# fixstars/cuda-bundle-adjustment

Measured on AMD Instinct MI355X. Metric: edges/sec (edge-iterations/s = E x LM iterations / wall, graph resident in HBM, every timed 10-iteration run from its own perturbed start) + 10-iter LM wall-clock (contract_wall: initialize()+optimize(10) after warm-up, C++ API) on KITTI-00-shaped graph; per-iter chi2 vs g2o-faithful oracle, higher is better.
Workload: dtype f64

## Files before the change

cuda-bundle-adjustment_amd/csrc/ba_device.hpp:

```cpp
#pragma once

#include "ba_kernels.hpp"

#include <type_traits>

namespace cubahip
{


#ifdef CUBA_HIP_TRACE
static __device__ unsigned long long cuba_trace_buf[3][8192 * 8];
#define TRACE_DECL unsigned long long tr_[8] = { 0, 0, 0, 0, 0, 0, 0, 0 }; int trn_ = 0; \
	{ unsigned long long t0_; asm volatile("s_memrealtime %0\n\ts_waitcnt lgkmcnt(0)" : "=s"(t0_)); tr_[7] = t0_; }
#define TRACE_MARK() do { asm volatile("s_waitcnt vmcnt(0) lgkmcnt(0)" ::: "memory"); tr_[trn_++] = wall_clock64(); } while (0)
#define TRACE_FLUSH(kid, wave) do { if ((threadIdx.x & 63) == 0 && (wave) < 8192) for (int t_ = 0; t_ < 8; t_++) cuba_trace_buf[kid][(wave) * 8 + t_] = tr_[t_]; } while (0)
#else
#define TRACE_DECL
#define TRACE_MARK() do { } while (0)
#define TRACE_FLUSH(kid, wave) do { } while (0)
#endif

__device__ __forceinline__ void atomic_max_nonneg(unsigned long long* p, Scalar v)
{
	if (v > 0) atomicMax(p, (unsigned long long)__double_as_longlong((double)v));
// ... 109 lines not shown
	int i = threadIdx.x;
	for (; i + 3072 < n; i += 4096)
	{
		const Scalar a = parts[i], b = parts[i + 1024], c = parts[i + 2048], d = parts[i + 3072];
		v0 += a; v1 += b; v2 += c; v3 += d;
	}
	for (; i < n; i += 1024) v0 += parts[i];
	return (v0 + v1) + (v2 + v3);
}

__device__ __forceinline__ Scalar block_sum_1024(Scalar v, Scalar* sh16)
{
	v = wave_sum(v);
	if ((threadIdx.x & 63) == 0) sh16[threadIdx.x >> 6] = v;
	__syncthreads();
	Scalar t = threadIdx.x < 16 ? sh16[threadIdx.x] : Scalar(0);
	if (threadIdx.x < 64) t = wave_sum(t);
	return t;
}

__device__ __forceinline__ void store_slot_group(Scalar* out, Scalar total)
{
	if (threadIdx.x < NSLOT) out[threadIdx.x] = threadIdx.x == 0 ? total : Scalar(0);
}

static __global__ __launch_bounds__(1024) void reduce_parts_kernel(const Scalar* __restrict__ parts, int n, Scalar* out)
{
	__shared__ Scalar sh[16];
	store_slot_group(out, block_sum_1024(parts_thread_sum(parts, n), sh));
}

static void launch_reduce_parts(const Scalar* parts, int n, Scalar* out, hipStream_t s)
{
	hipLaunchKernelGGL(reduce_parts_kernel, dim3(1), dim3(1024), 0, s, parts, n, out);
}

struct LaneEdge
{
	int ip, il;
	bool stereo;
	Scalar wr;
	EdgeLin lin;
};

__device__ __forceinline__ void load_pose(const DeviceGraph& g, int ip, Scalar q[4], Scalar t[3], Scalar cam[5])
{
#pragma unroll
	for (int i = 0; i < 4; i++) q[i] = g.q[4 * (size_t)ip + i];
#pragma unroll
	for (int i = 0; i < 3; i++) t[i] = g.t[3 * (size_t)ip + i];
#pragma unroll
	for (int i = 0; i < 5; i++) cam[i] = g.cam[5 * (size_t)ip + i];
}

__device__ __forceinline__ void linearize_edge(const DeviceGraph& g, int e, LaneEdge& out)
{
	const int pe = g.e_pose[e];
	out.stereo = (pe & STEREO_BIT) != 0;
	out.ip = pe & ~STEREO_BIT;
	out.il = g.e_lm[e];
	Scalar q[4], t[3], cam[5], Xw[3], meas[3], Xc[3];
	load_pose(g, out.ip, q, t, cam);
#pragma unroll
	for (int i = 0; i < 3; i++) Xw[i] = g.Xw[3 * (size_t)out.il + i];
	meas[0] = g.e_mu[e]; meas[1] = g.e_mv[e]; meas[2] = g.e_mr[e];
	const Scalar w = g.e_w[e];
	const Scalar s = edge_residual(q, t, cam, Xw, meas, out.stereo, out.lin.r, Xc);
	const int kind = out.stereo ? g.rk[1].kind : g.rk[0].kind;
	const Scalar delta = out.stereo ? g.rk[1].delta : g.rk[0].delta;
	out.wr = w * robust_weight(kind, delta, w * s);
	const Rot3 R = quat_to_rot(q[0], q[1], q[2], q[3]);
	edge_jacobians(Xc, R, cam, out.stereo, out.lin);
}

__device__ __forceinline__ void publish_report(const DeviceSystem& sys)
{
	sys.host_flags[0] = *sys.fail; sys.host_flags[1] = *sys.iters; sys.host_flags[2] = *sys.done;
	__threadfence_system();
	asm volatile("s_waitcnt vmcnt(0) lgkmcnt(0)" ::: "memory");
	const int t = ++(*sys.ticket);
	__hip_atomic_store(&sys.host_flags[3], t, __ATOMIC_RELAXED, __HIP_MEMORY_SCOPE_SYSTEM);
}

}
```

cuda-bundle-adjustment_amd/csrc/ba_edge.hip:

```cpp

#include "ba_device.hpp"

namespace cubahip
{

__device__ __forceinline__ void residual_chi2_body(const DeviceGraph& g, Scalar* parts, Scalar* per_edge, int bid, int nb)
{
	Scalar acc = 0;
	for (int e = g.e_begin + bid * 256 + threadIdx.x; e < g.e_end; e += nb * 256)
	{
		const int pe = g.e_pose[e];
		const bool stereo = (pe & STEREO_BIT) != 0;
		const int ip = pe & ~STEREO_BIT;
		const int il = g.e_lm[e];
		Scalar q[4], t[3], cam[5], Xw[3], meas[3], r[3], Xc[3];
		load_pose(g, ip, q, t, cam);
#pragma unroll
		for (int i = 0; i < 3; i++) Xw[i] = g.Xw[3 * (size_t)il + i];
		meas[0] = g.e_mu[e]; meas[1] = g.e_mv[e]; meas[2] = g.e_mr[e];
		const Scalar ee = g.e_w[e] * edge_residual(q, t, cam, Xw, meas, stereo, r, Xc);
		const int kind = stereo ? g.rk[1].kind : g.rk[0].kind;
		const Scalar delta = stereo ? g.rk[1].delta : g.rk[0].delta;
		acc += robust_rho(kind, delta, ee);
		if (per_edge) per_edge[e] = ee;
// ... 517 lines not shown
	{
		Scalar xl[3] = { 0, 0, 0 }, sc = 0;
		if (lmFree)
		{
			Scalar cs[3];
#pragma unroll
			for (int k = 0; k < 3; k++) cs[k] = red[0][k] + red[1][k] + red[2][k] + red[3][k];
			sc = finish_landmark_x(sys, il, cs, lambda, xl);
#pragma unroll
			for (int k = 0; k < 3; k++) g.Xw[3 * (size_t)il + k] = go.Xw[3 * (size_t)il + k] + xl[k];
		}
		scParts[blockIdx.x] = sc;
#pragma unroll
		for (int k = 0; k < 3; k++) xsh[k] = xl[k];
	}
	__syncthreads();
	Scalar Xn[3];
#pragma unroll
	for (int k = 0; k < 3; k++) Xn[k] = go.Xw[3 * (size_t)il + k] + xsh[k];
	Scalar rho = 0;
	for (int e = e0 + threadIdx.x; e < e1; e += 256)
	{
		const int pe = g.e_pose[e];
		const bool stereo = (pe & STEREO_BIT) != 0;
		const int ip = pe & ~STEREO_BIT;
		Scalar q[4], t[3], cam[5], meas[3], xp[6];
		load_pose(go, ip, q, t, cam);
		meas[0] = g.e_mu[e]; meas[1] = g.e_mv[e]; meas[2] = g.e_mr[e];
		const bool poseFree = ip < g.Pf;
#pragma unroll
		for (int r = 0; r < 6; r++) xp[r] = poseFree ? sys.xp[6 * (size_t)ip + r] : Scalar(0);
		rho += updated_edge_rho(g, q, t, cam, xp, poseFree, Xn, meas, g.e_w[e], stereo);
	}
	rho = wave_sum(rho);
	if ((threadIdx.x & 63) == 0) rsh[threadIdx.x >> 6] = rho;
	__syncthreads();
	if (threadIdx.x == 0) chiParts[blockIdx.x] = (rsh[0] + rsh[1]) + (rsh[2] + rsh[3]);
}

size_t trial_tail_parts(const DeviceGraph& g, const DeviceStructure& st, int priorParts)
{
	const size_t a = (size_t)(st.nWaves + LIN_BLOCK / WAVE - 1) / (LIN_BLOCK / WAVE) + st.nBig;
	const size_t nA = (a + 63) / 64 * 64;
	return nA + (a + priorParts + 63) / 64 * 64 + 4 * 256 + 64;
}

void launch_trial_tail_fused(const DeviceGraph& g, const DeviceStructure& st, const DeviceSystem& sys, Scalar lambda, const Scalar* old, hipStream_t s,
	const LmDevice* decide, const DevicePriors* pr, const DeviceRelPoses* rp)
{
	const int nLm = (st.nWaves + LIN_BLOCK / WAVE - 1) / (LIN_BLOCK / WAVE);
	const int nA = nLm + st.nBig;
	const int nRp = relpose_chi2_parts(rp);
	const int nPr = prior_chi2_parts(pr) + nRp;
	Scalar* scParts = sys.parts;
	Scalar* chiParts = sys.parts + (size_t)(nA + 63) / 64 * 64;
	Scalar* scaleParts = chiParts + (size_t)(nA + nPr + 63) / 64 * 64;
	const int poseBlocks = (g.Pf + LIN_BLOCK - 1) / LIN_BLOCK;
	const int nScale = g.Pf > 0 ? min((g.Pf * 6 + 255) / 256, 256) : 0;
	if (nLm + poseBlocks + nScale > 0)
		hipLaunchKernelGGL(trial_tail_kernel, dim3(nLm + poseBlocks + nScale), dim3(LIN_BLOCK), 0, s, g, st, sys, lambda, old, scParts, chiParts, nLm, poseBlocks, scaleParts, nScale);
	if (st.nBig > 0) hipLaunchKernelGGL(big_trial_tail_kernel, dim3(st.nBig), dim3(256), 0, s, g, st, sys, lambda, old, scParts + nLm, chiParts + nLm);
	if (nPr > nRp) launch_prior_chi2(g, *pr, chiParts + nA, s);
	if (nRp > 0) launch_relpose_chi2(g, *rp, chiParts + nA + (nPr - nRp), s);
	hipLaunchKernelGGL(reduce_report_kernel, dim3(1), dim3(1024), 0, s, sys, scParts, nA, sys.slots + NSLOT, chiParts, nA + nPr, sys.slots, scaleParts, 4 * nScale, sys.slots + 3 * NSLOT,
		decide ? decide->state : (double*)nullptr, decide ? decide->lam : (Scalar*)nullptr, decide ? decide->ring : (double*)nullptr);
}

void batch_fill_tail(const DeviceGraph& g, const DeviceStructure& st, const DeviceSystem& sys, const Scalar* old, const LmDevice& lm, Scalar* state, size_t stateCount, BatchTrial& t)
{
	const int nLm = (st.nWaves + LIN_BLOCK / WAVE - 1) / (LIN_BLOCK / WAVE);
	const int nA = nLm + st.nBig;
	t.scParts = sys.parts;
	t.chiParts = sys.parts + (size_t)(nA + 63) / 64 * 64;
	t.scaleParts = t.chiParts + (size_t)(nA + 63) / 64 * 64;
	t.poseBlocks = (g.Pf + LIN_BLOCK - 1) / LIN_BLOCK;
	t.nScale = g.Pf > 0 ? min((g.Pf * 6 + 255) / 256, 256) : 0;
	t.nLm = nLm; t.nA = nA; t.old = old;
	t.tailGrid = (unsigned)(nLm + t.poseBlocks + t.nScale);
	t.lmState = lm.state; t.lmLam = lm.lam; t.lmRing = lm.ring; t.reportOn = 1;
	t.state = state; t.stateCount = stateCount;
	t.restoreGrid = (unsigned)std::min<size_t>(512, (stateCount + 255) / 256);
}

__global__ void lm_decide_failed_kernel(DeviceSystem sys, double* lmState, Scalar* lmLam, double* lmRing)
{
	if (threadIdx.x != 0) return;
	lm_decide(lmState, lmLam, lmRing, 0, 0.0, 0.0, 0.0);
	__threadfence_system();
	if (sys.host_flags) publish_report(sys);
}

void launch_lm_decide_failed(const DeviceSystem& sys, const LmDevice& lm, hipStream_t s)
{
	hipLaunchKernelGGL(lm_decide_failed_kernel, dim3(1), dim3(64), 0, s, sys, lm.state, lm.lam, lm.ring);
}

__global__ __launch_bounds__(256) void restore_if_rejected_batch_kernel(const BatchEntry* __restrict__ tab)
{
	const BatchTrial& t = tab[blockIdx.y].t;
	if (blockIdx.x >= t.restoreGrid || t.lmState[5] != 0.0) return;
	const size_t stride = (size_t)t.restoreGrid * 256;
	const Scalar* __restrict__ backup = t.backupDst;
	Scalar* __restrict__ state = t.state;
	for (size_t i = (size_t)blockIdx.x * 256 + threadIdx.x; i < t.stateCount; i += stride) state[i] = backup[i];
}

__global__ __launch_bounds__(256) void restore_if_rejected_kernel(Scalar* __restrict__ state, const Scalar* __restrict__ backup, size_t count, const double* lmState)
{
	if (lmState[5] != 0.0) return;
	const size_t stride = (size_t)gridDim.x * 256;
	for (size_t i = (size_t)blockIdx.x * 256 + threadIdx.x; i < count; i += stride) state[i] = backup[i];
}

void launch_restore_if_rejected(Scalar* state, const Scalar* backup, size_t count, const LmDevice& lm, hipStream_t s)
{
	const unsigned grid = (unsigned)std::min<size_t>(512, (count + 255) / 256);
	if (grid) hipLaunchKernelGGL(restore_if_rejected_kernel, dim3(grid), dim3(256), 0, s, state, backup, count, lm.state);
}

void launch_batch_tail(const BatchEntry* tab, int n, unsigned tailGridMax, unsigned restoreGridMax, hipStream_t s)
{
	if (tailGridMax) hipLaunchKernelGGL(trial_tail_batch_kernel, dim3(tailGridMax, n), dim3(LIN_BLOCK), 0, s, tab);
	hipLaunchKernelGGL(reduce_report_batch_kernel, dim3(n), dim3(1024), 0, s, tab);
	if (restoreGridMax) hipLaunchKernelGGL(restore_if_rejected_batch_kernel, dim3(restoreGridMax, n), dim3(256), 0, s, tab);
}

}
```

cuda-bundle-adjustment_amd/csrc/ba_kernels.hpp:

```cpp
#pragma once

#include <hip/hip_runtime.h>
#include <cstdint>
#include <vector>

#include "ba_math.hpp"

namespace cubahip
{

constexpr int PCG_SETUP_POSES = 64;
constexpr int NSLOT = 16;
constexpr int WAVE = 64;
constexpr int LIN_BLOCK = 256;
constexpr int STEREO_BIT = 0x40000000;

struct DeviceGraph
{
	int Pt = 0, Pf = 0, Lt = 0, Lf = 0, E = 0;
	int e_begin = 0, e_end = 0;
	Scalar *q = nullptr, *t = nullptr, *cam = nullptr, *Xw = nullptr;
	int *e_pose = nullptr, *e_lm = nullptr;
	Scalar *e_mu = nullptr, *e_mv = nullptr, *e_mr = nullptr, *e_w = nullptr;
	int* lm_ptr = nullptr;
	RobustKernel rk[2] = { { 0, 0 }, { 0, 0 } };
};

constexpr int BP_HEAVY = 64;

struct DeviceStructure
{
	int nWaves = 0;
	int* wave_lm = nullptr;
	int nBig = 0;
	int* big_lm = nullptr;
	int nblk = 0;
	int *hsc_rowptr = nullptr, *hsc_colind = nullptr;
	int *adj_ptr = nullptr, *adj_blk = nullptr, *adj_col = nullptr;
	int2* ell = nullptr;
	int ell_m = 0, ell_over = 0;
	int* hsc_blkrow = nullptr;
	int nOd = 0;
	int nDiagProd = 0;
	int* od_blocks = nullptr;
	int inv_rows8 = 1;
	int nHeavy = 0;
	int *prod_ea = nullptr, *prod_eb = nullptr;
	const int *prod_beg = nullptr, *prod_end = nullptr, *pe_beg = nullptr, *pe_end = nullptr;
	int* prod_lm = nullptr;
	int* pe_edge = nullptr;
	int nCb = 0;
	int *cb_I = nullptr, *cb_J = nullptr, *cb_ptr = nullptr, *cb_blk = nullptr;
	Scalar *cb_wi = nullptr, *cb_wj = nullptr;
	Scalar* e_rec = nullptr;
	int mixed = 0;
};

int spmv_rows_for(int Pf);

struct DeviceSystem
{
	Scalar* hsc = nullptr;
	Scalar* bsc = nullptr;
	Scalar* bp = nullptr;
	Scalar* lm_sys = nullptr;
	Scalar* lm_inv = nullptr;
	Scalar* xp = nullptr;
	Scalar* xl = nullptr;
	Scalar* parts = nullptr;
	Scalar* slots = nullptr;
	unsigned long long* maxdiag = nullptr;
	int* fail = nullptr;
	Scalar *minv = nullptr, *r = nullptr, *z = nullptr, *p0 = nullptr, *p1 = nullptr, *ap = nullptr;
	Scalar *rz = nullptr, *pq = nullptr;
	int rzStride = 0, pqStride = 0;
	int nrz0 = 0, nrz = 0, npq = 0;
	int* done = nullptr;
	int* iters = nullptr;
	int* host_flags = nullptr;
	int* ticket = nullptr;
	int* kbase = nullptr;
	int agg = 0;
	int nc = 0;
	Scalar inv_agg = 0;
	int cl = 1;
	Scalar* acinv = nullptr;
	float* acinv32 = nullptr;
	Scalar* gj_pivots = nullptr;
	Scalar* rc = nullptr;
	Scalar* hrow = nullptr;
	int spmv_rows = 2;
	Scalar* qpart = nullptr;
	Scalar* r2 = nullptr;
	const Scalar* lam_dev = nullptr;
	int upper = 0;
	Scalar* tq = nullptr;
	int* lowpos = nullptr;
};

struct DevicePriors
{
	int n = 0;
	int nPoses = 0;
	const int* pose_ptr = nullptr;
	const int* pose_id = nullptr;
	const int* pose = nullptr;
	const Scalar *qbar = nullptr, *tbar = nullptr;
	const Scalar* info = nullptr;
	Scalar* chi = nullptr;
};
void launch_prior_linearize(const DeviceGraph& g, const DeviceStructure& st, const DeviceSystem& sys, const DevicePriors& pr, int mode, hipStream_t s);
void launch_prior_chi2(const DeviceGraph& g, const DevicePriors& pr, Scalar* parts, hipStream_t s);
int prior_chi2_parts(const DevicePriors* pr);

constexpr int REL_REC = 90;
struct DeviceRelPoses
{
	int n = 0;
	int nActive = 0;
	int nBlocks = 0;
	int nPoses = 0;
	const int *pose_i = nullptr, *pose_j = nullptr;
	const int* blk_ptr = nullptr;
	const int* blk_id = nullptr;
	const int* pose_ptr = nullptr;
	const int* pose_id = nullptr;
	const int* pose_item = nullptr;
	const Scalar *q = nullptr, *t = nullptr;
	const Scalar* info = nullptr;
	Scalar* rec = nullptr;
	Scalar* chi = nullptr;
};
void launch_relpose_linearize(const DeviceGraph& g, const DeviceStructure& st, const DeviceSystem& sys, const DeviceRelPoses& rp, int mode, hipStream_t s);
void launch_relpose_chi2(const DeviceGraph& g, const DeviceRelPoses& rp, Scalar* parts, hipStream_t s);
int relpose_chi2_parts(const DeviceRelPoses* rp);

void launch_residual_chi2(const DeviceGraph& g, Scalar* parts, Scalar* slots, Scalar* per_edge, hipStream_t st, const DevicePriors* pr = nullptr,
	const DeviceRelPoses* rp = nullptr);

struct BlockPassRange { int begin, end, heavy; };
void launch_linearize_dm(const DeviceGraph& g, const DeviceStructure& st, const DeviceSystem& sys, int mode, Scalar lambda, hipStream_t s,
	const Scalar* backupSrc = nullptr, Scalar* backupDst = nullptr, size_t backupCount = 0, const BlockPassRange* range = nullptr);
void launch_block_pass(const DeviceGraph& g, const DeviceStructure& st, const DeviceSystem& sys, const BlockPassRange& range, hipStream_t s);

void launch_pose_maxdiag(const DeviceGraph& g, const DeviceStructure& st, const DeviceSystem& sys, hipStream_t s);

void launch_back_substitute(const DeviceGraph& g, const DeviceStructure& st, const DeviceSystem& sys, Scalar lambda, hipStream_t s);

void launch_pose_scale(const DeviceGraph& g, const DeviceSystem& sys, Scalar lambda, Scalar* slots, hipStream_t s);
struct LmDevice;
void launch_trial_tail_fused(const DeviceGraph& g, const DeviceStructure& st, const DeviceSystem& sys, Scalar lambda, const Scalar* old, hipStream_t s,
	const LmDevice* decide = nullptr, const DevicePriors* pr = nullptr, const DeviceRelPoses* rp = nullptr);
size_t trial_tail_parts(const DeviceGraph& g, const DeviceStructure& st, int priorParts = 0);
constexpr int LM_REC = 8, LM_RING = 64;
struct LmDevice { double* state = nullptr; Scalar* lam = nullptr; double* ring = nullptr; };
void launch_lm_decide_failed(const DeviceSystem& sys, const LmDevice& lm, hipStream_t s);
void launch_restore_if_rejected(Scalar* state, const Scalar* backup, size_t count, const LmDevice& lm, hipStream_t s);
void launch_landmark_scale(const DeviceGraph& g, const DeviceSystem& sys, Scalar lambda, Scalar* slots, hipStream_t s);

void launch_update_state(const DeviceGraph& g, const DeviceSystem& sys, hipStream_t s);

void launch_pcg_setup(const DeviceGraph& g, const DeviceStructure& st, const DeviceSystem& sys, Scalar lambda, hipStream_t s);
void launch_pcg_spmv(const DeviceGraph& g, const DeviceStructure& st, const DeviceSystem& sys, int k, int maxIter, Scalar tol2, hipStream_t s);
void launch_pcg_update(const DeviceGraph& g, const DeviceStructure& st, const DeviceSystem& sys, int k, int maxIter, Scalar tol2, hipStream_t s);
Scalar* launch_coarse_setup(const DeviceGraph& g, const DeviceStructure& st, const DeviceSystem& sys, Scalar* work0, Scalar* work1, hipStream_t s, hipEvent_t assembled = nullptr);
Scalar* launch_dense_inverse(Scalar* work0, Scalar* work1, int n, Scalar* pivots, hipStream_t s);
void launch_coarse_finish(const Scalar* swept, Scalar* dst, int n, hipStream_t s);
struct GjJob { Scalar* buf[2]; Scalar* piv[2]; int n, tiles; };
void launch_coarse_assemble(const DeviceGraph& g, const DeviceStructure& st, const DeviceSystem& sys, Scalar* work0, hipStream_t s);
void launch_dense_inverse_batch(const GjJob* jobs, int m, int nMax, hipStream_t s);
void launch_pcg2_fused(const DeviceGraph& g, const DeviceSystem& sys, int k, int kOut, int maxIter, Scalar tol2, int doUpdate, hipStream_t s);
int spmv_upper_grid(int Pf);
int pcg_rows_max_aggregate();
int pcg_rows_entries_per_thread(const DeviceSystem& sys);
void launch_build_lowpos(const DeviceGraph& g, const DeviceStructure& st, int* lowpos, hipStream_t s);
void launch_pcg_upper_iteration(const DeviceGraph& g, const DeviceStructure& st, const DeviceSystem& sys, int k, int maxIter, Scalar tol2, hipStream_t s, int which = 7);
void launch_pcg_advance(const DeviceSystem& sys, int n, hipStream_t s, Scalar tol2 = Scalar(-1));
void launch_coarse_to_fp32(const Scalar* swept, float* dst, int n, hipStream_t s);
void launch_pcg_iteration(const DeviceGraph& g, const DeviceStructure& st, const DeviceSystem& sys, int k, int maxIter, Scalar tol2, hipStream_t s);

struct LmDevice;
struct BatchTrial
{
	unsigned lmGroups = 0, lmGrid = 0; const Scalar* backupSrc = nullptr; Scalar* backupDst = nullptr; size_t backupCount = 0;
	int poseGroups = 0; unsigned schurGrid = 0;
	int nSetup = 0; size_t expandTotal = 0; unsigned nExpand = 0; const Scalar* copySrc = nullptr; Scalar* copyDst = nullptr; size_t copyPairs = 0; unsigned setupGrid = 0;
	int fusedOn = 0;
	const Scalar* old = nullptr; Scalar *scParts = nullptr, *chiParts = nullptr, *scaleParts = nullptr; int nLm = 0, poseBlocks = 0, nScale = 0; unsigned tailGrid = 0; int nA = 0;
	double* lmState = nullptr; Scalar* lmLam = nullptr; double* lmRing = nullptr; int reportOn = 0;
	Scalar* state = nullptr; size_t stateCount = 0; unsigned restoreGrid = 0;
};
struct BatchEntry
{
	DeviceGraph g; DeviceStructure st; DeviceSystem sys;
	int maxIter = 0;
	int gridSpmv = 0;
	BatchTrial t;
};
void batch_fill_linearize(const DeviceGraph& g, const DeviceStructure& st, const Scalar* backupSrc, Scalar* backupDst, size_t backupCount, BatchTrial& t);
void launch_batch_linearize(const BatchEntry* tab, int n, unsigned lmGridMax, unsigned schurGridMax, bool mixed, hipStream_t s);
void batch_fill_setup(const DeviceGraph& g, const DeviceStructure& st, const DeviceSystem& sys, const Scalar* copySrc, Scalar* copyDst, size_t copyCount, BatchTrial& t);
void launch_batch_setup(const BatchEntry* tab, int n, unsigned gridMax, hipStream_t s);
void launch_batch_first_precond(const BatchEntry* tab, int n, const DeviceSystem& sys0, int ncMax, size_t ldsMax, Scalar tol2, hipStream_t s);
void batch_fill_tail(const DeviceGraph& g, const DeviceStructure& st, const DeviceSystem& sys, const Scalar* old, const LmDevice& lm, Scalar* state, size_t stateCount, BatchTrial& t);
void launch_batch_tail(const BatchEntry* tab, int n, unsigned tailGridMax, unsigned restoreGridMax, hipStream_t s);
int batch_kernel_class(const DeviceGraph& g, const DeviceSystem& sys);
size_t batch_pcg2_lds_bytes(const DeviceSystem& sys);
void launch_pcg_batch_iteration(const BatchEntry* tab, int n, const DeviceGraph& g0, const DeviceSystem& sys0, int gridSpmvMax, int ncMax, size_t ldsMax, int k, Scalar tol2, hipStream_t s);
void launch_pcg_batch_advance(const BatchEntry* tab, int n, int iters, hipStream_t s, Scalar tol2);

hipError_t graph_add_pcg_chunk(hipGraph_t graph, const DeviceGraph& g, const DeviceStructure& st, const DeviceSystem& sys, int chunk, int maxIter, Scalar tol2, int report);

void launch_hsc_expand(const DeviceGraph& g, const DeviceStructure& st, const DeviceSystem& sys, hipStream_t s);
void launch_pcg_setup_expand(const DeviceGraph& g, const DeviceStructure& st, const DeviceSystem& sys, Scalar lambda, hipStream_t s,
	const Scalar* copySrc = nullptr, Scalar* copyDst = nullptr, size_t copyCount = 0);

constexpr int SC_T = 32;
constexpr int SC_TP = 5;
constexpr int SC_TT = SC_T * SC_T;

struct SparseCholPlan
{
	int Pf = 0, T = 0, nTiles = 0, nLevels = 0, slack = 0;
	std::vector<int> posOfSeg, segOfPos;
	std::vector<int> colPtr;
	std::vector<int> rowIdx, colOfTile;
	std::vector<int> gPtr;
	std::vector<int> gather;
	std::vector<int> wgRec;
	std::vector<int> lvlPtr, lvlTiles;
	std::vector<int> lvlColPtr, lvlCols;
	std::vector<int> blkTile;
	long long entries = 0;
	size_t tileBytes() const { return sizeof(Scalar) * (size_t)SC_TT * ((size_t)2 * nTiles + 1); }
	double secondsEstimate() const;
};
bool sparse_chol_plan(int Pf, const int* rowptr, const int* colind, int slack, size_t maxTiles, SparseCholPlan& out);

struct SparseChol
{
	Scalar* tiles = nullptr;
	Scalar* tilesT = nullptr;
	Scalar* y = nullptr;
	Scalar* rinv = nullptr;
	const int *colPtr = nullptr, *rowIdx = nullptr, *colOfTile = nullptr, *gPtr = nullptr, *gather = nullptr;
	const int *wgRec = nullptr, *lvlCols = nullptr, *blkTile = nullptr, *posOfSeg = nullptr;
	int* fail = nullptr;
	int T = 0, Pf = 0, nTiles = 0;
};
void launch_sparse_chol_fill(const DeviceStructure& st, const DeviceSystem& sys, const SparseChol& d, hipStream_t s);
void launch_sparse_chol_solve(const SparseChol& d, const SparseCholPlan& plan, Scalar* x, hipStream_t s);
void launch_sparse_chol_factor(const SparseChol& d, const SparseCholPlan& plan, hipStream_t s);

struct SelInvPlan
{
	int nLevels = 0;
	std::vector<int> stepPtr;
	std::vector<int> offRec;
	std::vector<int> colStepPtr, cols;
	std::vector<int> gather;
// ... 58 lines not shown
```

cuda-bundle-adjustment_amd/csrc/ba_lm.hip:

```cpp
#include "ba_solver.hpp"

using namespace cubahip;

void cuba_hip_solver::graphWorker()
{
	(void)hipSetDevice(device);
	std::unique_lock<std::mutex> lk(gb.m);
	for (;;)
	{
		gb.cv.wait(lk, [&] { return gb.stop || !gb.jobs.empty() || !gb.trash.empty(); });
		if (gb.stop) return;
		if (gb.jobs.empty())
		{
			std::vector<hipGraphExec_t> t; t.swap(gb.trash);
			gb.busy = true;
			lk.unlock();
			for (hipGraphExec_t e : t) (void)hipGraphExecDestroy(e);
			lk.lock();
			gb.busy = false;
			gb.cv.notify_all();
			continue;
		}
		GraphJob j = gb.jobs.front(); gb.jobs.pop_front();
		gb.busy = true;
		lk.unlock();
		const auto t0 = Clock::now();
		hipGraph_t graph = nullptr; hipGraphExec_t exec = nullptr;
		bool ok = hipGraphCreate(&graph, 0) == hipSuccess && graph_add_pcg_chunk(graph, j.g, j.st, j.sys, j.chunk, j.maxIter, j.tol2, 1) == hipSuccess &&
			hipGraphInstantiate(&exec, graph, nullptr, nullptr, 0) == hipSuccess;
		if (graph) (void)hipGraphDestroy(graph);
		if (!ok) (void)hipGetLastError();
		const double dt = std::chrono::duration<double>(Clock::now() - t0).count();
		lk.lock();
		gb.busy = false;
		if (ok && j.gen == gb.gen) { gb.ready[std::make_pair(j.chunk, j.acinv)] = exec; gb.builds++; gb.seconds.store(gb.seconds.load() + dt); }
		else if (exec) (void)hipGraphExecDestroy(exec);
		gb.cv.notify_all();
	}
}

hipGraphExec_t cuba_hip_solver::pcgGraphIfReady(int chunk, int maxIter, Scalar tol2)
{
	if (pcgGraphTol2 != tol2 || pcgGraphMaxIter != maxIter) { dropPcgGraph(); pcgGraphTol2 = tol2; pcgGraphMaxIter = maxIter; }
	const auto key = std::make_pair(chunk, (const Scalar*)sys.acinv);
	auto it = pcgGraphs.find(key);
	if (it != pcgGraphs.end()) return it->second;
	std::lock_guard<std::mutex> lk(gb.m);
	for (auto& kv : gb.ready) pcgGraphs[kv.first] = kv.second;
	gb.ready.clear();
	it = pcgGraphs.find(key);
	if (it != pcgGraphs.end()) return it->second;
	if (!gb.requested.count(key))
	{
		gb.requested[key] = 1;
		gb.jobs.push_back(GraphJob{ chunk, (const Scalar*)sys.acinv, g, st, sys, maxIter, tol2, gb.gen });
		if (!gb.th.joinable()) gb.th = std::thread([this] { graphWorker(); });
		gb.cv.notify_all();
	}
	return nullptr;
}

void cuba_hip_solver::dropPcgGraph()
{
	{
		std::lock_guard<std::mutex> lk(gb.m);
		gb.gen++;
		gb.jobs.clear(); gb.requested.clear();
		const bool offload = gb.th.joinable() && !gb.stop;
		for (auto& kv : gb.ready) { if (offload) gb.trash.push_back(kv.second); else (void)hipGraphExecDestroy(kv.second); }
		gb.ready.clear();
		for (auto& kv : pcgGraphs) { if (offload) gb.trash.push_back(kv.second); else (void)hipGraphExecDestroy(kv.second); }
		if (offload && !gb.trash.empty()) gb.cv.notify_all();
	}
	pcgGraphs.clear();
	batchRequests.clear();
	graphsOrderedFor = nullptr;
}

void cuba_hip_solver::ensureOverlapObjects()
{
	if (gjStream) return;
	int prioLow = 0, prioHigh = 0;
	HIP_TRY(hipDeviceGetStreamPriorityRange(&prioLow, &prioHigh));
	HIP_TRY(hipStreamCreateWithPriority(&gjStream, hipStreamNonBlocking, prioLow));
	HIP_TRY(hipEventCreateWithFlags(&evSetup, hipEventDisableTiming));
	HIP_TRY(hipEventCreateWithFlags(&evAssembled, hipEventDisableTiming));
	HIP_TRY(hipEventCreateWithFlags(&evInverse, hipEventDisableTiming));
	HIP_TRY(hipEventCreateWithFlags(&evFirstInv, hipEventDisableTiming));
	HIP_TRY(hipEventRecord(evFirstInv, gjStream));
}

void cuba_hip_solver::waitReport()
{
	volatile int* flags = (volatile int*)((char*)h_pinned + 1024);
	{
		const auto t0 = Clock::now();
		for (long spins = 0; flags[3] != expectedTicket; spins++)
			if ((spins & 0xfff) == 0xfff && std::chrono::duration<double>(Clock::now() - t0).count() > 2.0) break;
		if (flags[3] == expectedTicket)
		{
			std::atomic_thread_fence(std::memory_order_acquire);
			return;
		}
	}
	sync();
	std::atomic_thread_fence(std::memory_order_acquire);
	expectedTicket = flags[3];
}

void cuba_hip_solver::downloadAsDouble(const Scalar* dsrc, double* hdst, size_t n)
{
	if (!n) return;
	if (sizeof(Scalar) == sizeof(double))
	{
		HIP_TRY(hipMemcpyAsync(hdst, dsrc, n * sizeof(double), hipMemcpyDeviceToHost, stream));
		sync();
		return;
	}
	std::vector<Scalar> tmp(n);
	HIP_TRY(hipMemcpyAsync(tmp.data(), dsrc, n * sizeof(Scalar), hipMemcpyDeviceToHost, stream));
	sync();
	for (size_t i = 0; i < n; i++) hdst[i] = (double)tmp[i];
}

void cuba_hip_solver::uploadFromDouble(Scalar* ddst, const double* hsrc, size_t n)
{
	if (!n) return;
	std::vector<Scalar> tmp(hsrc, hsrc + n);
	HIP_TRY(hipMemcpyAsync(ddst, tmp.data(), n * sizeof(Scalar), hipMemcpyHostToDevice, stream));
	sync();
}

double cuba_hip_solver::computeErrors()
{
	need();
	StageTimer tm(this, 2);
	launch_residual_chi2(g, d_parts.data(), slotsDev, nullptr, stream, priors(), relPoses());
	return readSlots(0);
}

void cuba_hip_solver::linearize(int mode, double lam, bool withBackup)
{
	waitAssembled();
	const bool parts = mode == 1 && !redParts.empty();
	launch_linearize_dm(g, st, sys, mode, lam, stream, withBackup ? d_state.data() : nullptr, d_backup.data(), d_state.size(), parts ? &redParts[0].od : nullptr);
	if (parts && !partsByCaller)
		for (size_t c = 1; c < redParts.size(); c++) launch_block_pass(g, st, sys, redParts[c].od, stream);
	if (priors()) launch_prior_linearize(g, st, sys, pri, mode, stream);
	if (relPoses()) launch_relpose_linearize(g, st, sys, rel, mode, stream);
}

void cuba_hip_solver::schurPart(int part, size_t ranges[4])
{
	need();
	if (part < 0 || part >= schurParts()) throw ArgError{ "cuba_hip_schur_part: no such part" };
	if (part == 0)
	{
		StageTimer tm(this, 4);
		zeroReduced();
		partsByCaller = true;
		try { linearize(1, lambda, false); } catch (...) { partsByCaller = false; throw; }
		partsByCaller = false;
	}
	else
	{
		StageTimer tm(this, 4);
		launch_block_pass(g, st, sys, redParts[part].od, stream);
	}
	const size_t nblk = (size_t)st.nblk;
	ranges[0] = redParts.empty() ? 0 : 36 * redParts[part].blkBegin;
	ranges[1] = redParts.empty() ? 36 * nblk : 36 * (redParts[part].blkEnd - redParts[part].blkBegin);
	ranges[2] = part == 0 ? 36 * nblk : 0;
	ranges[3] = part == 0 ? d_red.size() - 36 * nblk : 0;
}

void cuba_hip_solver::assemble()
{
	need();
	StageTimer tm(this, 3);
	zeroReduced(true);
	d_maxdiag.zero(stream);
	linearize(0, 0.0);
}

void cuba_hip_solver::maxDiagonalParts(double* posePart, double* lmPart)
{
	need();
// ... 67 lines not shown
	return ok2;
}

int cuba_hip_solver::pcgBudget(int maxIter) const
{
	const int it = directAfter > 0 ? directAfter : std::min(384, std::max(128, Pf / 4));
	return std::min(maxIter, std::max(4, it / 4 * 4));
}

bool cuba_hip_solver::ensureDirectPlan()
{
	if (directPlanValid) return !directRefused;
	const auto t0 = Clock::now();
	ensureHostPattern();
	if (!sparse_chol_plan(Pf, h_rowptr.data(), h_colind.data(), directSlack, (size_t)std::max(1, directMaxTiles), directPlan))
	{
		directPlanValid = true; directRefused = true;
		char buf[200];
		std::snprintf(buf, sizeof buf, "exact reduced solve unavailable: the factor of the %d-pose reduced matrix needs more than direct_max_tiles = %d tiles", Pf, directMaxTiles);
		lastError = buf;
		return false;
	}
	const SparseCholPlan& p = directPlan;
	{
		size_t freeB = 0, totalB = 0;
		const size_t have = sizeof(Scalar) * (d_scTiles.size() + d_scTilesT.size());
		if (hipMemGetInfo(&freeB, &totalB) == hipSuccess && p.tileBytes() > have && p.tileBytes() - have > freeB)
		{
			directPlanValid = true; directRefused = true;
			char buf[200];
			std::snprintf(buf, sizeof buf, "exact reduced solve unavailable: the factor of the %d-pose reduced matrix needs %.1f MB, %.1f MB of device memory are free",
				Pf, p.tileBytes() / 1e6, freeB / 1e6);
			lastError = buf;
			return false;
		}
		(void)hipGetLastError();
	}
	std::vector<int> ints;
	auto put = [&](const std::vector<int>& v) { const size_t o = ints.size(); ints.insert(ints.end(), v.begin(), v.end()); while (ints.size() % 4) ints.push_back(0); return o; };
	const size_t oColPtr = put(p.colPtr), oRowIdx = put(p.rowIdx), oColOf = put(p.colOfTile), oGPtr = put(p.gPtr), oGather = put(p.gather),
		oWgRec = put(p.wgRec), oLvlCols = put(p.lvlCols), oBlkTile = put(p.blkTile), oPos = put(p.posOfSeg);
	d_scInts.upload(ints, stream);
	d_scTiles.resize((size_t)SC_TT * ((size_t)p.nTiles + 1)); d_scTilesT.resize((size_t)SC_TT * std::max(1, p.nTiles));
	d_scY.resize((size_t)SC_T * p.T); d_scRinv.resize((size_t)SC_T * p.T); d_scFail.resize(1);
	sync();
	SparseChol& d = directDev;
	d.tiles = d_scTiles.data(); d.tilesT = d_scTilesT.data(); d.y = d_scY.data(); d.rinv = d_scRinv.data(); d.fail = d_scFail.data();
	const int* base = d_scInts.data();
	d.colPtr = base + oColPtr; d.rowIdx = base + oRowIdx; d.colOfTile = base + oColOf; d.gPtr = base + oGPtr; d.gather = base + oGather;
	d.wgRec = base + oWgRec; d.lvlCols = base + oLvlCols; d.blkTile = base + oBlkTile; d.posOfSeg = base + oPos;
	d.T = p.T; d.Pf = Pf; d.nTiles = p.nTiles;
	directPlanValid = true;
	directPlanBuilds++;
	directPlanSeconds = std::chrono::duration<double>(Clock::now() - t0).count();
	if (std::getenv("CUBA_HIP_DEBUG"))
		std::fprintf(stderr, "[cuba_hip] exact reduced solve, symbolic phase: %d poses -> %d tile columns, %d tiles (%.1f MB), %d levels, %lld tile products, slack %d, %.2f ms\n",
			Pf, p.T, p.nTiles, p.tileBytes() / 1e6, p.nLevels, p.entries, p.slack, 1e3 * directPlanSeconds);
	return true;
}

bool cuba_hip_solver::solveDirect()
{
	if (!ensureDirectPlan()) return false;
	const auto t0 = Clock::now();
	launch_sparse_chol_fill(st, sys, directDev, stream);
	launch_sparse_chol_solve(directDev, directPlan, sys.xp, stream);
	int* hflag = (int*)hostStage();
	HIP_TRY(hipMemcpyAsync(hflag, directDev.fail, sizeof(int), hipMemcpyDeviceToHost, stream));
	sync();
	directSeconds = std::chrono::duration<double>(Clock::now() - t0).count();
	cntDirect++;
	directSticky = true;
	coarseValid = false;
	if (std::getenv("CUBA_HIP_DEBUG"))
		std::fprintf(stderr, "[cuba_hip] exact reduced solve: %d unknowns, %.3f ms, lambda %.3e%s\n", 6 * Pf, 1e3 * directSeconds, lambda, *hflag ? " -- NON-POSITIVE PIVOT" : "");
	if (*hflag)
	{
		cntDirectFailed++;
		lastError = "exact reduced solve: non-positive pivot (the damped reduced matrix is not positive definite)";
		return false;
	}
	return true;
}

bool cuba_hip_solver::solveBegin(SolveCtx& sc)
{
	lastSolveBrokeDown = false;
	need();
	if (Pf == 0) { sc.result = true; return true; }
	const int maxIter = sc.maxIter = maxIterAlloc;
	const Scalar tol2 = sc.tol2 = pcgTol * pcgTol;
	if (failDirty) { d_fail.zero(stream); failDirty = false; }
	const bool twoLevel = sc.twoLevel = sys.agg > 0;
	const bool direct = sc.direct = directUsable();
	if (direct && (directSticky || directAlways))
	{
		launch_pcg_setup(g, st, sys, lambda, stream);
		failDirty = true;
		coarseValid = false;
		if (pcgHistory.size() >= 65536) pcgHistory.erase(pcgHistory.begin(), pcgHistory.begin() + 32768);
		pcgHistory.push_back(0);
		sc.result = solveDirect();
		return true;
	}
	sc.budget = direct && !acceptUnconverged ? pcgBudget(maxIter) : maxIter;
	const size_t invCount = (size_t)36 * sys.cl * sys.cl * sys.nc * sys.nc;
	bool takeInverse = false;
	if (twoLevel && coarseValid && pendingInv >= 0)
	{
		HIP_TRY(hipStreamWaitEvent(stream, evInverse, 0));
		takeInverse = true; pendingInv = -1;
	}
	const bool deferred = sc.deferLaunch && twoLevel && coarseValid;
	{
		const bool f32 = fp32Inverse();
		const Scalar* cpSrc = !takeInverse ? nullptr : f32 ? reinterpret_cast<const Scalar*>(d_coarse32[1].data()) : d_coarse[0].data();
		Scalar* cpDst = f32 ? reinterpret_cast<Scalar*>(d_coarse32[0].data()) : d_coarse[2].data();
		const size_t cpCount = f32 ? inv32Count() / 2 : invCount;
		if (deferred) { sc.deferred = true; sc.copySrc = cpSrc; sc.copyDst = cpDst; sc.copyCount = cpCount; }
		else launch_pcg_setup_expand(g, st, sys, lambda, stream, cpSrc, cpDst, cpCount);
	}
	if (twoLevel)
	{
		const int gjSteps = (6 * sys.cl * sys.nc + 31) / 32, first = gjSteps & 1;
		{
			ensureOverlapObjects();
			const size_t invBytes = sizeof(Scalar) * (size_t)36 * sys.cl * sys.cl * sys.nc * sys.nc;
			if (!coarseValid && heuristics && firstInvValid)
			{
				HIP_TRY(hipStreamWaitEvent(stream, evFirstInv, 0));
				if (fp32Inverse()) HIP_TRY(hipMemcpyAsync(d_coarse32[0].data(), d_firstInv32.data(), inv32Count() * sizeof(float), hipMemcpyDeviceToDevice, stream));
				else HIP_TRY(hipMemcpyAsync(d_coarse[2].data(), d_firstInv.data(), invBytes, hipMemcpyDeviceToDevice, stream));
				pendingInv = -1;
				coarseValid = true; sideAge = overlapPeriod(); firstInvPending = true;
			}
			else if (!coarseValid)
			{
				drainInversion();
				(void)launch_coarse_setup(g, st, sys, d_coarse[first].data(), d_coarse[1 - first].data(), stream);
				if (fp32Inverse()) launch_coarse_to_fp32(d_coarse[0].data(), d_coarse32[0].data(), 6 * sys.cl * sys.nc, stream);
				else launch_coarse_finish(d_coarse[0].data(), d_coarse[2].data(), 6 * sys.cl * sys.nc, stream);
				coarseValid = true; cntCoarseRefresh++; cntCoarseInline++; sideAge = 0;
				if (heuristics)
				{
					if (fp32Inverse()) d_firstInv32.resize(inv32Count()); else d_firstInv.resize(invCount);
					sideAge = overlapPeriod(); firstInvPending = true;
				}
			}
			sys.acinv = d_coarse[2].data();
			const bool regular = ++sideAge >= overlapPeriod();
			if (regular) sideAge = 0;
			if (regular)
			{
				if (!deferred) HIP_TRY(hipEventRecord(evSetup, stream));
				if (sc.deferCoarse)
				{
					sc.deferCoarse->push_back(CoarseJob{ this, first, firstInvPending, !deferred });
					if (firstInvPending) { firstInvPending = false; firstInvValid = true; }
				}
				else
				{
					HIP_TRY(hipStreamWaitEvent(gjStream, evSetup, 0));
					(void)launch_coarse_setup(g, st, sys, d_coarse[first].data(), d_coarse[1 - first].data(), gjStream, evAssembled);
					if (fp32Inverse()) launch_coarse_to_fp32(d_coarse[0].data(), d_coarse32[1].data(), 6 * sys.cl * sys.nc, gjStream);
					else launch_coarse_finish(d_coarse[0].data(), d_coarse[0].data(), 6 * sys.cl * sys.nc, gjStream);
					if (firstInvPending)
					{
						if (fp32Inverse()) HIP_TRY(hipMemcpyAsync(d_firstInv32.data(), d_coarse32[1].data(), inv32Count() * sizeof(float), hipMemcpyDeviceToDevice, gjStream));
						else HIP_TRY(hipMemcpyAsync(d_firstInv.data(), d_coarse[0].data(), invBytes, hipMemcpyDeviceToDevice, gjStream));
						HIP_TRY(hipEventRecord(evFirstInv, gjStream));
						firstInvPending = false; firstInvValid = true;
					}
					HIP_TRY(hipEventRecord(evInverse, gjStream));
				}
				pendingInv = 0;
				assemblePending = true; cntCoarseRefresh++;
			}
		}
		if (!deferred) launch_pcg2_fused(g, sys, 0, 0, maxIter, tol2, 0, stream);
	}
	const bool graphs = sc.graphs = useGraph && !sc.batched && g_liveHandles.load(std::memory_order_relaxed) <= 1;
	if (useGraph && !graphs && (!pcgGraphs.empty() || graphsOrderedFor)) dropPcgGraph();
	if (graphs && pcgGraphs.empty() && graphsOrderedFor != (const void*)sys.acinv)
	{
		for (int c = 64; c >= 4; c /= 2) (void)pcgGraphIfReady(c, maxIter, tol2);
		graphsOrderedFor = (const void*)sys.acinv;
	}
	sc.hInts = (volatile int*)((char*)h_pinned + 1024);
	sc.tSolve0 = Clock::now();
	int predicted = 32;
	if (runIters.size() >= 2)
	{
		const double a = runIters[runIters.size() - 2], b = runIters.back();
		const double lin = b + std::max(0.0, b - a), geo = b * std::min(1.35, std::max(1.0, b / std::max(1.0, a)));
		predicted = (int)std::max(lin, geo) + 1;
	}
	else if (runIters.size() == 1) predicted = (int)(1.35 * runIters[0]) + 2;
	else if (firstSolveIters > 0) predicted = firstSolveIters + 1;
	{
		const size_t k = runIters.size();
		if (heuristics && k < prevRunIters.size() && std::equal(runIters.begin(), runIters.end(), prevRunIters.begin())) predicted = prevRunIters[k];
	}
	sc.predicted = predicted;
	return false;
}

bool cuba_hip_solver::solveBrokeDown(SolveCtx& sc)
{
	lastSolveBrokeDown = true; lastFailCode = sc.hInts[0];
	cntPcgIters += sc.hInts[1]; coarseValid = false; firstInvValid = false; firstInvPending = false; failDirty = true;
	if (sc.direct && lastFailCode != 1 && !(lastFailCode == 2 && fp32Inverse() && sc.twoLevel))
	{
		if (pcgHistory.size() >= 65536) pcgHistory.erase(pcgHistory.begin(), pcgHistory.begin() + 32768);
		pcgHistory.push_back(-sc.hInts[1]);
		d_fail.zero(stream); failDirty = false;
		return solveDirect();
	}
	return false;
}

bool cuba_hip_solver::solveReducedOnce()
{
	StageTimer tm(this, 6);
	SolveCtx sc;
	if (solveBegin(sc)) return sc.result;
	const int maxIter = sc.maxIter; const Scalar tol2 = sc.tol2; const bool graphs = sc.graphs; const int predicted = sc.predicted;
	bool converged = false;
	int k0 = 0, looks = 0, eagerIters = 0;
	int target = (predicted + 3) / 4 * 4;
	while (k0 < sc.budget && !converged)
	{
		int todo = std::max(4, std::min(target, sc.budget) - k0);
		while (todo > 0)
		{
			int c = graphs ? 256 : todo;
			for (; graphs && c > 4 && c > todo; c >>= 1) {}
			if (graphs && todo > c && todo % 4 == 0 && todo <= 128 && pcgGraphMaxIter == maxIter && pcgGraphTol2 == tol2)
			{
				if ((pcgGraphs.count(std::make_pair(todo, (const Scalar*)sys.acinv)) || ++batchRequests[todo] >= 2) && pcgGraphIfReady(todo, maxIter, tol2)) c = todo;
			}
			hipGraphExec_t exec = graphs ? pcgGraphIfReady(c, maxIter, tol2) : nullptr;
			if (exec) { HIP_TRY(hipGraphLaunch(exec, stream)); noteReport(); }
			else
			{
				for (int k = 0; k < c; k++) enqueuePcgIteration(k, maxIter, tol2, stream);
				launch_pcg_advance(sys, c, stream, tol2); noteReport();
				if (graphs) { eagerIters += c; cntPcgPlain += c; }
			}
			k0 += c; todo -= c;
		}
		waitReport();
		if (sc.hInts[0] != 0) return solveBrokeDown(sc);
		if (sc.hInts[2] != 0 || sc.hInts[1] < std::min(k0, maxIter)) converged = true;
		target = k0 + ((looks == 0 && k0 <= 96) ? 4 : std::max(8, k0 / 8 / 4 * 4));
		looks++; cntPcgLooks++; cntHostLooks++;
	}
	sc.converged = converged; sc.k0 = k0; sc.looks = looks; sc.eagerIters = eagerIters;
	return solveEnd(sc);
}

bool cuba_hip_solver::solveEnd(SolveCtx& sc)
{
	const int maxIter = sc.maxIter; const bool direct = sc.direct; const bool converged = sc.converged;
	const int k0 = sc.k0, looks = sc.looks, eagerIters = sc.eagerIters, predicted = sc.predicted;
	const auto tSolve1 = Clock::now();
	if (std::getenv("CUBA_HIP_DEBUG"))
	{
		std::vector<Scalar> part((size_t)std::max(1, sys.nrz0));
		HIP_TRY(hipMemcpyAsync(part.data(), sys.rz, sizeof(Scalar) * part.size(), hipMemcpyDeviceToHost, stream));
		sync();
		double rz0 = 0; for (Scalar v : part) rz0 += (double)v;
		std::fprintf(stderr, "[cuba_hip] PCG: %d iterations, %d enqueued (%d as plain launches), %d host looks (prediction %d), lambda %.3e, r0.z0 %.6e, solve %.3f ms, graphs built so far %lld\n",
			sc.hInts[1], k0, eagerIters, looks, predicted, lambda, rz0, 1e3 * std::chrono::duration<double>(tSolve1 - sc.tSolve0).count(), (long long)gb.builds.load());
	}
	const int itersDone = sc.itersDone >= 0 ? sc.itersDone : sc.hInts[1];
	cntPcgIters += itersDone; cntPcgEnqueued += k0;
	if (runIters.empty()) firstSolveIters = itersDone;
	runIters.push_back(itersDone);
	if (pcgHistory.size() >= 65536) pcgHistory.erase(pcgHistory.begin(), pcgHistory.begin() + 32768);
	pcgHistory.push_back(converged ? itersDone : -itersDone);
	if (!converged)
	{
		cntPcgUnconverged++;
		coarseValid = false;
		if (direct && !acceptUnconverged) return solveDirect();
		char buf[160];
		std::snprintf(buf, sizeof buf, "PCG stopped at max_iter = %d without reaching pcg_tol = %g", maxIter, pcgTol);
		lastError = buf;
		return acceptUnconverged;
	}
	return true;
}

void cuba_hip_solver::backSubstitute()
{
	need();
	StageTimer tm(this, 4);
	launch_back_substitute(g, st, sys, lambda, stream);
}

bool cuba_hip_solver::solve()
{
	schur();
	if (!solveReduced()) return false;
	backSubstitute();
	return true;
}

void cuba_hip_solver::update()
{
	need();
	StageTimer tm(this, 7);
	launch_update_state(g, sys, stream);
}

double cuba_hip_solver::computeScale(double lam)
{
	need();
	double a = 0, b = 0;
	scaleParts(lam, &a, &b);
	return a + b;
}

void cuba_hip_solver::lmRunBegin(LmRun& r, int niter, double* chi2Out)
{
	const double tau = 1e-5;
	if (!h_lmRing)
	{
		HIP_TRY(hipHostMalloc((void**)&h_lmRing, sizeof(double) * LM_RING * LM_REC, hipHostMallocMapped | hipHostMallocCoherent));
		HIP_TRY(hipHostGetDevicePointer((void**)&lmRingDev, h_lmRing, 0));
	}
	coarseValid = false;
	startRunHistory();
	r = LmRun();
	r.niter = niter; r.chi2Out = chi2Out; r.stop = niter <= 0;
	r.F = computeErrors();
	r.lam = tau * maxDiagonal();
	{
		double* st8 = reinterpret_cast<double*>(hostStage());
		st8[0] = r.F; st8[1] = r.lam; st8[2] = 2.0; st8[3] = 0.0; st8[4] = 0.0; st8[5] = 1.0; st8[6] = 0.0; st8[7] = (double)LmRun::maxq;
		r.tagBase = 65536.0 * (double)(++lmRunNonce); st8[8] = r.tagBase;
		Scalar* l1 = reinterpret_cast<Scalar*>(st8 + 12);
		l1[0] = (Scalar)r.lam;
		HIP_TRY(hipMemcpyAsync(d_lmState.data(), st8, sizeof(double) * 9, hipMemcpyHostToDevice, stream));
		HIP_TRY(hipMemcpyAsync(d_lamS.data(), l1, sizeof(Scalar), hipMemcpyHostToDevice, stream));
	}
	r.lm.state = d_lmState.data(); r.lm.lam = d_lamS.data(); r.lm.ring = lmRingDev;
}

void cuba_hip_solver::lmAbsorb(LmRun& r, int upto)
{
	std::atomic_thread_fence(std::memory_order_acquire);
	for (; r.seen < upto && !r.stop; r.seen++)
	{
		const volatile double* rec = h_lmRing + (size_t)(r.seen % LM_RING) * LM_REC;
		const double tag = r.tagBase + (double)(r.seen + 1);
		if (rec[7] != tag)
		{
			cntLateRecords++;
			sync();
			std::atomic_thread_fence(std::memory_order_acquire);
			if (rec[7] != tag) throw StateError{ "the device's decision record of an LM trial never arrived" };
		}
		const bool acc = rec[5] != 0.0;
		const double rho = rec[2];
		r.lam = rec[3]; r.F = rec[4];
		if (acc) r.rejRun = 0; else r.rejRun++;
		const bool iterationEnds = acc || r.rejRun == LmRun::maxq || !(rho < 0);
		if (!iterationEnds) continue;
		if (r.chi2Out) r.chi2Out[r.done] = r.F;
		r.done++;
		if (r.done == r.niter || r.rejRun == LmRun::maxq || rho <= 0 || !std::isfinite(r.lam)) r.stop = true;
		r.rejRun = 0;
	}
}

bool cuba_hip_solver::lmBeforeTrial(LmRun& r)
{
	if (r.stop) return false;
	if (r.enq > r.seen)
	{
		const bool safe = r.done + 1 < r.niter && r.rejRun + 1 < LmRun::maxq;
		if (!safe) { waitReport(); cntHostLooks++; lmAbsorb(r, r.enq); if (r.stop) return false; }
	}
	cntTrials++;
	lambda = -1.0;
	return true;
}

bool cuba_hip_solver::lmAfterSolveHost(LmRun& r)
{
	lmAbsorb(r, r.enq);
	if (r.stop) { cntTrials--; return false; }
	return true;
}

bool cuba_hip_solver::lmAfterSolve(LmRun& r, bool ok)
{
	if (!lmAfterSolveHost(r)) return false;
	if (ok) launch_trial_tail_fused(g, st, sys, (Scalar)-1, d_backup.data(), stream, &r.lm, priors(), relPoses());
	else launch_lm_decide_failed(sys, r.lm, stream);
	noteReport();
	launch_restore_if_rejected(d_state.data(), d_backup.data(), d_state.size(), r.lm, stream);
	r.enq++;
	(void)hipStreamQuery(stream);
	return true;
}

int cuba_hip_solver::lmRunEnd(LmRun& r)
{
	if (r.seen < r.enq) { waitReport(); cntHostLooks++; lmAbsorb(r, r.enq); }
	lambda = r.lam;
	return r.done;
}

int cuba_hip_solver::optimizeDeviceDecision(int niter, double* chi2Out)
{
	LmRun r;
	lmRunBegin(r, niter, chi2Out);
	while (lmBeforeTrial(r))
	{
		schur(true);
		const bool ok = solveReduced();
		if (!lmAfterSolve(r, ok)) break;
	}
	return lmRunEnd(r);
}

bool cuba_hip_solver::fullyBatchable() const
{
	return batchable() && st.nBig == 0 && st.nDiagProd == 0 && st.nOd > 0 && st.nWaves > 0 && redParts.empty() && h_priorPose.empty() && h_relI.empty();
}

bool cuba_hip_solver::batchable() const
{
	return !profile && partHi < 0 && Pf > 0 && Lf > 0 && E > 0 && trial_tail_parts(g, st, extraChiParts()) <= d_parts.size() && batch_kernel_class(g, sys) >= 0;
}

void cuba_hip_solver::launchCoarseJobs(std::vector<CoarseJob>& jobs, hipEvent_t common)
{
	if (jobs.empty()) return;
	ensureOverlapObjects();
	hipStream_t side = gjStream;
	const int m = (int)jobs.size();
	if (!h_gjTab) { HIP_TRY(hipHostMalloc((void**)&h_gjTab, sizeof(GjJob) * CUBA_HIP_BATCH_MAX, hipHostMallocDefault)); HIP_TRY(hipEventCreateWithFlags(&evGjTab, hipEventDisableTiming)); HIP_TRY(hipEventRecord(evGjTab, side)); }
	d_gjTab.resize(sizeof(GjJob) * CUBA_HIP_BATCH_MAX);
	HIP_TRY(hipEventSynchronize(evGjTab));
	int nMax = 0;
	for (int a = 0; a < m; a++)
	{
		cuba_hip_solver* h = jobs[a].h;
		const int Nc = 6 * h->sys.cl * h->sys.nc;
		HIP_TRY(hipStreamWaitEvent(side, jobs[a].ownEvent || !common ? h->evSetup : common, 0));
		launch_coarse_assemble(h->g, h->st, h->sys, h->d_coarse[jobs[a].first].data(), side);
		GjJob& j = h_gjTab[a];
		j.buf[0] = h->d_coarse[jobs[a].first].data(); j.buf[1] = h->d_coarse[1 - jobs[a].first].data();
		j.piv[0] = h->sys.gj_pivots; j.piv[1] = h->sys.gj_pivots + 32 * 32;
		j.n = Nc; j.tiles = (Nc + 31) / 32;
		nMax = std::max(nMax, Nc);
	}
	for (int a = 0; a < m; a++) HIP_TRY(hipEventRecord(jobs[a].h->evAssembled, side));
	HIP_TRY(hipMemcpyAsync(d_gjTab.data(), h_gjTab, sizeof(GjJob) * m, hipMemcpyHostToDevice, side));
	HIP_TRY(hipEventRecord(evGjTab, side));
	launch_dense_inverse_batch(reinterpret_cast<const GjJob*>(d_gjTab.data()), m, nMax, side);
	for (int a = 0; a < m; a++)
	{
		cuba_hip_solver* h = jobs[a].h;
		const int Nc = 6 * h->sys.cl * h->sys.nc;
		const size_t invBytes = sizeof(Scalar) * (size_t)Nc * Nc;
		if (h->fp32Inverse()) launch_coarse_to_fp32(h->d_coarse[0].data(), h->d_coarse32[1].data(), Nc, side);
		else launch_coarse_finish(h->d_coarse[0].data(), h->d_coarse[0].data(), Nc, side);
		if (jobs[a].firstInvCopy)
		{
			if (h->fp32Inverse()) HIP_TRY(hipMemcpyAsync(h->d_firstInv32.data(), h->d_coarse32[1].data(), h->inv32Count() * sizeof(float), hipMemcpyDeviceToDevice, side));
			else HIP_TRY(hipMemcpyAsync(h->d_firstInv.data(), h->d_coarse[0].data(), invBytes, hipMemcpyDeviceToDevice, side));
			HIP_TRY(hipEventRecord(h->evFirstInv, side));
		}
		HIP_TRY(hipEventRecord(h->evInverse, side));
	}
	jobs.clear();
}

static int cuba_hip_optimize_batch_full(cuba_hip_solver** hs, int n, int niter, double* chi2, int* nDone)
{
	cuba_hip_solver* lead = hs[0];
	hipStream_t bs = lead->stream;
	struct StreamGuard
	{
		cuba_hip_solver** hs; int n; std::vector<hipStream_t> own;
		StreamGuard(cuba_hip_solver** h, int m, hipStream_t s) : hs(h), n(m), own((size_t)m)
		{
			for (int i = 0; i < n; i++) { own[i] = hs[i]->stream; (void)hipStreamSynchronize(own[i]); hs[i]->stream = s; }
		}
		~StreamGuard() { if (n > 0) (void)hipStreamSynchronize(hs[0]->stream); for (int i = 0; i < n; i++) hs[i]->stream = own[i]; }
	} streamGuard(hs, n, bs);
	std::vector<cuba_hip_solver::LmRun> runs((size_t)n);
	std::vector<cuba_hip_solver::SolveCtx> ctx((size_t)n);
	lead->ensureOverlapObjects();
	std::vector<cuba_hip_solver::CoarseJob> coarseJobs;
	if (lead->h_batchTab && lead->batchTabEntries < 3 * CUBA_HIP_BATCH_MAX) { (void)hipHostFree(lead->h_batchTab); lead->h_batchTab = nullptr; }
	if (!lead->h_batchTab) { HIP_TRY(hipHostMalloc((void**)&lead->h_batchTab, sizeof(BatchEntry) * CUBA_HIP_BATCH_MAX * 3, hipHostMallocDefault)); lead->batchTabEntries = 3 * CUBA_HIP_BATCH_MAX; }
	lead->d_batchTab.resize(sizeof(BatchEntry) * CUBA_HIP_BATCH_MAX * 3);
// ... 404 lines not shown
```

cuda-bundle-adjustment_amd/csrc/ba_pcg.hip:

```cpp

#include "ba_device.hpp"

namespace cubahip
{

template <bool ROWCOPY>
__device__ __forceinline__ void pcg_setup_body(const DeviceGraph& g, const DeviceStructure& st, const DeviceSystem& sys, Scalar lambda, int bid, int nb)
{
	const int i = threadIdx.x < PCG_SETUP_POSES ? bid * PCG_SETUP_POSES + (int)threadIdx.x : g.Pf;
	lambda = launch_lambda(sys, lambda);
	Scalar rz = 0;
	if (i < g.Pf)
	{
		Scalar* blk = sys.hsc + 36 * (size_t)st.hsc_rowptr[i];
		Scalar A[36], Ai[36];
#pragma unroll
		for (int c = 0; c < 6; c++)
#pragma unroll
			for (int r = 0; r <= c; r++)
			{
				Scalar v = blk[c * 6 + r];
				if (r == c) v += lambda;
				A[c * 6 + r] = v;
				A[r * 6 + c] = v;
			}
#pragma unroll
		for (int k = 0; k < 36; k++) blk[k] = A[k];
		if (ROWCOPY && !sys.upper)
		{
			const int pos = (st.adj_ptr[i + 1] - st.adj_ptr[i]) - (st.hsc_rowptr[i + 1] - st.hsc_rowptr[i]);
			if (pos < 20 * st.ell_m)
			{
				Scalar* dst = sys.hrow + 36 * ((size_t)i * st.ell_m * 20 + pos);
#pragma unroll
				for (int k = 0; k < 36; k++) dst[k] = A[k];
			}
		}
		if (!spd6_inverse(A, Ai)) *sys.fail = 1;
#pragma unroll
		for (int k = 0; k < 36; k++) sys.minv[36 * (size_t)i + k] = Ai[k];
		Scalar rr[6];
#pragma unroll
		for (int k = 0; k < 6; k++) rr[k] = sys.bsc[6 * (size_t)i + k];
#pragma unroll
		for (int r = 0; r < 6; r++)
		{
			Scalar z = 0;
#pragma unroll
			for (int c = 0; c < 6; c++) z += Ai[c * 6 + r] * rr[c];
			sys.r[6 * (size_t)i + r] = rr[r];
			sys.z[6 * (size_t)i + r] = z;
			sys.xp[6 * (size_t)i + r] = 0;
			sys.p0[6 * (size_t)i + r] = 0;
			sys.p1[6 * (size_t)i + r] = 0;
			rz += rr[r] * z;
		}
	}
	rz = wave_sum(rz);
	if (sys.agg == 0)
	{
		if (threadIdx.x == 0)
		{
			const Scalar s2 = rz;
			sys.rz[bid] = s2;
			sys.rz[sys.rzStride + bid] = s2;
		}
		for (int t = nb + bid * 256 + threadIdx.x; t < sys.nrz; t += nb * 256) sys.rz[sys.rzStride + t] = 0;
	}
	if (bid == 0 && threadIdx.x == 0) { *sys.iters = 0; *sys.done = 0; *sys.kbase = 0; }
}

__global__ __launch_bounds__(256) void pcg_setup_kernel(DeviceGraph g, DeviceStructure st, DeviceSystem sys, Scalar lambda)
{
	pcg_setup_body<false>(g, st, sys, lambda, blockIdx.x, gridDim.x);
}

void launch_pcg_setup(const DeviceGraph& g, const DeviceStructure& st, const DeviceSystem& sys, Scalar lambda, hipStream_t s)
{
	if (g.Pf > 0) hipLaunchKernelGGL(pcg_setup_kernel, dim3((g.Pf + PCG_SETUP_POSES - 1) / PCG_SETUP_POSES), dim3(256), 0, s, g, st, sys, lambda);
}

__device__ __forceinline__ bool pcg_active(const DeviceSystem& sys, int k, int maxIter, Scalar tol2, int lane, Scalar& rzk)
{
	if (*sys.done) return false;
	rzk = wave_sum(load_parts(rz_slot(sys, k), rz_count(sys, k), lane));
	const Scalar rz0 = wave_sum(load_parts(sys.rz, sys.nrz0, lane));
	const bool on = k < maxIter && *sys.fail == 0 && rzk > tol2 * rz0 && rzk == rzk;
	if (!on && blockIdx.x == 0 && threadIdx.x == 0) { *sys.done = 1; if (!(rzk == rzk)) *sys.fail = 3; }
	return on;
}

__device__ __forceinline__ void spmv_entry(const DeviceStructure& st, const DeviceSystem& sys, const Scalar* pold, int a, int rr,
	Scalar& accz, Scalar& accp)
{
	const int bi = st.adj_blk[a];
	const int j = st.adj_col[a];
	const Scalar* B = sys.hsc + 36 * (size_t)(bi & 0x7fffffff);
	const int sr = bi < 0 ? 6 : 1, sc = bi < 0 ? 1 : 6;
	Scalar av[6], zv[6], pv[6];
#pragma unroll
	for (int c = 0; c < 6; c++)
	{
		av[c] = B[rr * sr + c * sc];
		zv[c] = sys.z[6 * (size_t)j + c];
		pv[c] = pold[6 * (size_t)j + c];
	}
#pragma unroll
	for (int c = 0; c < 6; c++) { accz += av[c] * zv[c]; accp += av[c] * pv[c]; }
}

typedef Scalar Scalar2 __attribute__((ext_vector_type(2)));

template <bool FUSED>
__device__ __forceinline__ void hsc_expand_body(const DeviceStructure& st, const DeviceSystem& sys, size_t total, size_t bid)
{
	const size_t t = bid * 256 + threadIdx.x;
	if (t >= total) return;
	const size_t slot = t / 36;
	const int e = (int)(t - 36 * slot);
	const int2 en = st.ell[slot];
	if (en.y < 0) return;
	const int rr = e / 6, c = e - 6 * rr;
	const Scalar* B = sys.hsc + 36 * (size_t)(en.x & 0x7fffffff);
	if (FUSED && en.y == (int)(slot / ((size_t)st.ell_m * 20))) return;
	sys.hrow[t] = B[en.x < 0 ? rr * 6 + c : c * 6 + rr];
}

__global__ __launch_bounds__(256) void hsc_expand_kernel(DeviceStructure st, DeviceSystem sys, size_t total)
{
	hsc_expand_body<false>(st, sys, total, blockIdx.x);
}

__global__ __launch_bounds__(256) void pcg_setup_expand_kernel(DeviceGraph g, DeviceStructure st, DeviceSystem sys, Scalar lambda, int nSetup, size_t total,
	unsigned nExpand, const Scalar2* __restrict__ copySrc, Scalar2* __restrict__ copyDst, size_t copyPairs)
{
	if ((int)blockIdx.x < nSetup) pcg_setup_body<true>(g, st, sys, lambda, blockIdx.x, nSetup);
	else if (blockIdx.x < nSetup + nExpand) hsc_expand_body<true>(st, sys, total, blockIdx.x - nSetup);
	else
	{
		const size_t stride = (size_t)(gridDim.x - nSetup - nExpand) * 256;
		for (size_t i = (size_t)(blockIdx.x - nSetup - nExpand) * 256 + threadIdx.x; i < copyPairs; i += stride) copyDst[i] = copySrc[i];
	}
}

__global__ __launch_bounds__(256) void pcg_setup_expand_batch_kernel(const BatchEntry* __restrict__ tab)
{
	const BatchEntry& e = tab[blockIdx.y];
	const BatchTrial& t = e.t;
	if (blockIdx.x >= t.setupGrid) return;
	if ((int)blockIdx.x < t.nSetup) pcg_setup_body<true>(e.g, e.st, e.sys, Scalar(-1), blockIdx.x, t.nSetup);
	else if (blockIdx.x < t.nSetup + t.nExpand) hsc_expand_body<true>(e.st, e.sys, t.expandTotal, blockIdx.x - t.nSetup);
	else
	{
		const Scalar2* __restrict__ src = reinterpret_cast<const Scalar2*>(t.copySrc);
		Scalar2* __restrict__ dst = reinterpret_cast<Scalar2*>(t.copyDst);
		const size_t stride = (size_t)(t.setupGrid - t.nSetup - t.nExpand) * 256;
		for (size_t i = (size_t)(blockIdx.x - t.nSetup - t.nExpand) * 256 + threadIdx.x; i < t.copyPairs; i += stride) dst[i] = src[i];
	}
}

void launch_hsc_expand(const DeviceGraph& g, const DeviceStructure& st, const DeviceSystem& sys, hipStream_t s)
{
	const size_t total = (size_t)g.Pf * st.ell_m * 20 * 36;
	if (total) hipLaunchKernelGGL(hsc_expand_kernel, dim3((unsigned)((total + 255) / 256)), dim3(256), 0, s, st, sys, total);
}

void launch_pcg_setup_expand(const DeviceGraph& g, const DeviceStructure& st, const DeviceSystem& sys, Scalar lambda, hipStream_t s,
	const Scalar* copySrc, Scalar* copyDst, size_t copyCount)
{
	if (g.Pf <= 0) return;
	const size_t total = sys.upper ? 0 : (size_t)g.Pf * st.ell_m * 20 * 36;
// ... 5 lines not shown
		reinterpret_cast<const Scalar2*>(copySrc), reinterpret_cast<Scalar2*>(copyDst), pairs);
}

void batch_fill_setup(const DeviceGraph& g, const DeviceStructure& st, const DeviceSystem& sys, const Scalar* copySrc, Scalar* copyDst, size_t copyCount, BatchTrial& t)
{
	t.expandTotal = sys.upper ? 0 : (size_t)g.Pf * st.ell_m * 20 * 36;
	t.nSetup = (g.Pf + PCG_SETUP_POSES - 1) / PCG_SETUP_POSES;
	t.nExpand = (unsigned)((t.expandTotal + 255) / 256);
	t.copyPairs = copySrc ? copyCount / 2 : 0;
	const unsigned nCopy = t.copyPairs ? (unsigned)std::min<size_t>(1024, (t.copyPairs + 255) / 256) : 0;
	t.copySrc = copySrc; t.copyDst = copyDst;
	t.setupGrid = t.nSetup + t.nExpand + nCopy;
}

void launch_batch_setup(const BatchEntry* tab, int n, unsigned gridMax, hipStream_t s)
{
	if (gridMax) hipLaunchKernelGGL(pcg_setup_expand_batch_kernel, dim3(gridMax, n), dim3(256), 0, s, tab);
}

template <int N>
__device__ __forceinline__ void spmv_batch(const DeviceSystem& sys, const Scalar* pold, const int2 (&e)[3], const Scalar* Arow, int rr, Scalar& accz, Scalar& accp)
{
	Scalar2 av[N][3], zv[N][3], pv[N][3];
#pragma unroll
	for (int n = 0; n < N; n++)
	{
		const size_t j = e[n].y >= 0 ? e[n].y : 0;
		const Scalar2* A2 = reinterpret_cast<const Scalar2*>(Arow + (size_t)n * (20 * 36) + 6 * rr);
		const Scalar2* z2 = reinterpret_cast<const Scalar2*>(sys.z + 6 * j);
		const Scalar2* p2 = reinterpret_cast<const Scalar2*>(pold + 6 * j);
		const bool on = e[n].y >= 0;
#pragma unroll
		for (int c = 0; c < 3; c++) { av[n][c] = on ? A2[c] : Scalar2{ 0, 0 }; zv[n][c] = z2[c]; pv[n][c] = p2[c]; }
	}
#pragma unroll
	for (int n = 0; n < N; n++)
	{
#pragma unroll
		for (int c = 0; c < 3; c++)
		{
			const Scalar a0 = av[n][c].x, a1 = av[n][c].y;
			accz += a0 * zv[n][c].x; accp += a0 * pv[n][c].x;
			accz += a1 * zv[n][c].y; accp += a1 * pv[n][c].y;
		}
	}
}

template <int ROWS>
__device__ __forceinline__ void pcg_spmv_body(const DeviceGraph& g, const DeviceStructure& st, const DeviceSystem& sys, int k, int maxIter, Scalar tol2)
{
	const int lane = threadIdx.x & 63, wv = threadIdx.x >> 6;
	const int half = wv & 1, lr = wv >> 1;
	const Scalar* pold = (k & 1) ? sys.p1 : sys.p0;
	Scalar* pnew = (k & 1) ? sys.p0 : sys.p1;
	const int row = blockIdx.x * ROWS + lr;
	TRACE_DECL
	TRACE_MARK();
	const int kb_v = vector_load_flag(sys.kbase);
	const int failed_v = vector_load_flag(sys.fail) | vector_load_flag(sys.done);
	const Scalar s_k = load_parts(rz_slot(sys, k), sys.nrz, lane);
	const Scalar s_0 = load_parts(sys.rz, sys.nrz0, lane);
	const Scalar s_m = load_parts(rz_slot(sys, k - 1), sys.nrz, lane);

	const bool rowOn = row < g.Pf;
	const int slot = half * 10 + lane / 6, rr = lane % 6;
	int2 e[3];
	int a0 = 0, a1 = 0;
#pragma unroll
	for (int m = 0; m < 3; m++)
		e[m] = (rowOn && lane < 60 && m < st.ell_m) ? st.ell[((size_t)row * st.ell_m + m) * 20 + slot] : int2{ 0, -1 };
	if (rowOn && st.ell_over && lane < 60) { a0 = st.adj_ptr[row] + 20 * st.ell_m + slot; a1 = st.adj_ptr[row + 1]; }
	Scalar accz = 0, accp = 0, zi = 0, pi_old = 0;
	if (rowOn && half == 0 && lane < 6)
	{
		zi = sys.z[6 * (size_t)row + lane];
		pi_old = pold[6 * (size_t)row + lane];
	}
	TRACE_MARK();
	k += __builtin_amdgcn_readfirstlane(kb_v);
	const int failed = __builtin_amdgcn_readfirstlane(failed_v);
	const Scalar rzk = to_uniform(wave_sum(s_k)), rz0 = to_uniform(wave_sum(s_0)), rzm = to_uniform(wave_sum(s_m));
	if (!(k < maxIter && failed == 0 && rzk > tol2 * rz0 && rzk == rzk))
	{
		if (blockIdx.x == 0 && threadIdx.x == 0) { *sys.done = 1; if (!(rzk == rzk)) *sys.fail = 3; }
		return;
	}
	const Scalar beta = k > 0 ? rzk / rzm : Scalar(0);
	if (rowOn)
	{
		int cnt = 0;
#pragma unroll
		for (int m = 0; m < 3; m++) cnt += __any(e[m].y >= 0) ? 1 : 0;
		const Scalar* Arow = sys.hrow + 36 * ((size_t)row * st.ell_m * 20 + slot);
		if (cnt == 3) spmv_batch<3>(sys, pold, e, Arow, rr, accz, accp);
		else if (cnt == 2) spmv_batch<2>(sys, pold, e, Arow, rr, accz, accp);
		else if (cnt == 1) spmv_batch<1>(sys, pold, e, Arow, rr, accz, accp);
		for (int a = a0; a < a1; a += 20) spmv_entry(st, sys, pold, a, rr, accz, accp);
	}
	TRACE_MARK();
	accz += __shfl_down(accz, 30); accp += __shfl_down(accp, 30);
	Scalar tz = accz, tp = accp;
	tz += __shfl_down(accz, 6);  tp += __shfl_down(accp, 6);
	tz += __shfl_down(accz, 12); tp += __shfl_down(accp, 12);
	tz += __shfl_down(accz, 18); tp += __shfl_down(accp, 18);
	tz += __shfl_down(accz, 24); tp += __shfl_down(accp, 24);
	__shared__ Scalar other[ROWS][12];
	__shared__ Scalar qrow[ROWS][6];
	__shared__ Scalar part[ROWS];
	if (half == 1 && lane < 6) { other[lr][lane] = tz; other[lr][6 + lane] = tp; }
	__syncthreads();
	TRACE_MARK();
	Scalar dot = 0;
	if (half == 0)
	{
		Scalar q = 0;
		if (row < g.Pf && lane < 6)
		{
			tz += other[lr][lane]; tp += other[lr][6 + lane];
			const Scalar pi = zi + beta * pi_old;
			q = tz + beta * tp;
			pnew[6 * (size_t)row + lane] = pi;
			sys.ap[6 * (size_t)row + lane] = q;
			dot = pi * q;
		}
		if (lane < 6) qrow[lr][lane] = q;
		dot = wave_sum(dot);
		if (lane == 0) part[lr] = dot;
	}
	__syncthreads();
	if (threadIdx.x < 6 * sys.cl)
	{
		const int a = threadIdx.x / 6, c = threadIdx.x - 6 * a;
		Scalar s2 = 0;
#pragma unroll
		for (int w = 0; w < ROWS; w++)
			s2 += (a == 0 ? Scalar(1) : agg_weight(blockIdx.x * ROWS + w, sys.agg, g.Pf)) * qrow[w][c];
		if (sys.qpart && sys.agg > 0)
		{
			const int per = sys.agg / ROWS, J = blockIdx.x / per, m = blockIdx.x - J * per;
			sys.qpart[(size_t)m * (6 * sys.cl * sys.nc) + 6 * sys.cl * J + threadIdx.x] = s2;
		}
	}
	if (threadIdx.x == 64)
	{
		Scalar s2 = 0;
#pragma unroll
		for (int w = 0; w < ROWS; w++) s2 += part[w];
		pq_slot(sys, k)[blockIdx.x] = s2;
	}
	TRACE_MARK();
	TRACE_FLUSH(0, blockIdx.x * 2 * ROWS + wv);
}

template <int ROWS, int MIN_WAVES>
__global__ __launch_bounds__(128 * ROWS, MIN_WAVES) void pcg_spmv_kernel(DeviceGraph g, DeviceStructure st, DeviceSystem sys, int k, int maxIter, Scalar tol2)
{
	pcg_spmv_body<ROWS>(g, st, sys, k, maxIter, tol2);
}

template <int ROWS, int MIN_WAVES>
__global__ __launch_bounds__(128 * ROWS, MIN_WAVES) void pcg_spmv_batch_kernel(const BatchEntry* __restrict__ tab, int k, Scalar tol2)
{
	const BatchEntry& e = tab[blockIdx.y];
	if ((int)blockIdx.x >= e.gridSpmv) return;
	pcg_spmv_body<ROWS>(e.g, e.st, e.sys, k, e.maxIter, tol2);
}

__device__ __forceinline__ void spmv_level(const DeviceSystem& sys, const Scalar* pold, int2 e, const Scalar* Arow, int r2,
	Scalar& az0, Scalar& ap0, Scalar& az1, Scalar& ap1)
{
	Scalar2 a0v[3], a1v[3], zv[3], pv[3];
	const size_t j = e.y >= 0 ? e.y : 0;
	const Scalar2* A2 = reinterpret_cast<const Scalar2*>(Arow + 12 * r2);
	const Scalar2* z2 = reinterpret_cast<const Scalar2*>(sys.z + 6 * j);
	const Scalar2* p2 = reinterpret_cast<const Scalar2*>(pold + 6 * j);
	const bool on = e.y >= 0;
#pragma unroll
	for (int c = 0; c < 3; c++)
	{
		a0v[c] = on ? A2[c] : Scalar2{ 0, 0 }; a1v[c] = on ? A2[3 + c] : Scalar2{ 0, 0 };
		zv[c] = z2[c]; pv[c] = p2[c];
	}
#pragma unroll
	for (int c = 0; c < 3; c++)
	{
		az0 += a0v[c].x * zv[c].x; ap0 += a0v[c].x * pv[c].x;
		az0 += a0v[c].y * zv[c].y; ap0 += a0v[c].y * pv[c].y;
		az1 += a1v[c].x * zv[c].x; ap1 += a1v[c].x * pv[c].x;
		az1 += a1v[c].y * zv[c].y; ap1 += a1v[c].y * pv[c].y;
	}
}

template <int ROWS>
__global__ __launch_bounds__(64 * ROWS, 5) void pcg_spmv_row_kernel(DeviceGraph g, DeviceStructure st, DeviceSystem sys, int k, int maxIter, Scalar tol2)
{
	const int lane = threadIdx.x & 63, lr = threadIdx.x >> 6;
	const Scalar* pold = (k & 1) ? sys.p1 : sys.p0;
	Scalar* pnew = (k & 1) ? sys.p0 : sys.p1;
	const int row = blockIdx.x * ROWS + lr;
	const int kb_v = vector_load_flag(sys.kbase);
	const int failed_v = vector_load_flag(sys.fail) | vector_load_flag(sys.done);
	const Scalar s_k = load_parts(rz_slot(sys, k), sys.nrz, lane);
	const Scalar s_0 = load_parts(sys.rz, sys.nrz0, lane);
	const Scalar s_m = load_parts(rz_slot(sys, k - 1), sys.nrz, lane);
	const bool rowOn = row < g.Pf;
	const int slot = lane / 3, r2 = lane - 3 * slot;
	int2 e[3];
	int a0 = 0, a1 = 0;
#pragma unroll
	for (int m = 0; m < 3; m++)
		e[m] = (rowOn && lane < 60 && m < st.ell_m) ? st.ell[((size_t)row * st.ell_m + m) * 20 + slot] : int2{ 0, -1 };
	if (rowOn && st.ell_over && lane < 60) { a0 = st.adj_ptr[row] + 20 * st.ell_m + slot; a1 = st.adj_ptr[row + 1]; }
	Scalar zi = 0, pi_old = 0;
	if (rowOn && lane < 6)
	{
		zi = sys.z[6 * (size_t)row + lane];
		pi_old = pold[6 * (size_t)row + lane];
	}
	k += __builtin_amdgcn_readfirstlane(kb_v);
	const int failed = __builtin_amdgcn_readfirstlane(failed_v);
	const Scalar rzk = to_uniform(wave_sum(s_k)), rz0 = to_uniform(wave_sum(s_0)), rzm = to_uniform(wave_sum(s_m));
	if (!(k < maxIter && failed == 0 && rzk > tol2 * rz0 && rzk == rzk))
	{
		if (blockIdx.x == 0 && threadIdx.x == 0) { *sys.done = 1; if (!(rzk == rzk)) *sys.fail = 3; }
		return;
	}
	const Scalar beta = k > 0 ? rzk / rzm : Scalar(0);
	Scalar az0 = 0, ap0 = 0, az1 = 0, ap1 = 0;
	if (rowOn)
	{
		int cnt = 0;
#pragma unroll
		for (int m = 0; m < 3; m++) cnt += __any(e[m].y >= 0) ? 1 : 0;
		const Scalar* Arow = sys.hrow + 36 * ((size_t)row * st.ell_m * 20 + slot);
		if (cnt >= 1) spmv_level(sys, pold, e[0], Arow, r2, az0, ap0, az1, ap1);
		if (cnt >= 2) spmv_level(sys, pold, e[1], Arow + 20 * 36, r2, az0, ap0, az1, ap1);
		if (cnt == 3) spmv_level(sys, pold, e[2], Arow + 2 * (20 * 36), r2, az0, ap0, az1, ap1);
		for (int a = a0; a < a1; a += 20)
		{
			const int bi = st.adj_blk[a];
			const size_t j = st.adj_col[a];
			const Scalar* B = sys.hsc + 36 * (size_t)(bi & 0x7fffffff);
			const int sr = bi < 0 ? 6 : 1, sc = bi < 0 ? 1 : 6;
#pragma unroll
			for (int c = 0; c < 6; c++)
			{
				const Scalar zc = sys.z[6 * j + c], pc = pold[6 * j + c];
				const Scalar b0 = B[(2 * r2) * sr + c * sc], b1 = B[(2 * r2 + 1) * sr + c * sc];
				az0 += b0 * zc; ap0 += b0 * pc; az1 += b1 * zc; ap1 += b1 * pc;
			}
		}
	}
	az0 += __shfl_down(az0, 30); ap0 += __shfl_down(ap0, 30); az1 += __shfl_down(az1, 30); ap1 += __shfl_down(ap1, 30);
	az0 += __shfl_down(az0, 15); ap0 += __shfl_down(ap0, 15); az1 += __shfl_down(az1, 15); ap1 += __shfl_down(ap1, 15);
	Scalar t0 = az0, u0 = ap0, t1 = az1, u1 = ap1;
#pragma unroll
	for (int d = 3; d <= 12; d += 3) { t0 += __shfl_down(az0, d); u0 += __shfl_down(ap0, d); t1 += __shfl_down(az1, d); u1 += __shfl_down(ap1, d); }
	const Scalar tzA = __shfl(t0, lane >> 1), tzB = __shfl(t1, lane >> 1), tpA = __shfl(u0, lane >> 1), tpB = __shfl(u1, lane >> 1);
	const Scalar tz = (lane & 1) ? tzB : tzA, tp = (lane & 1) ? tpB : tpA;
	__shared__ Scalar qrow[ROWS][6];
	__shared__ Scalar part[ROWS];
	Scalar q = 0, dot = 0;
	if (rowOn && lane < 6)
	{
		const Scalar pi = zi + beta * pi_old;
		q = tz + beta * tp;
		pnew[6 * (size_t)row + lane] = pi;
		sys.ap[6 * (size_t)row + lane] = q;
		dot = pi * q;
	}
	if (lane < 6) qrow[lr][lane] = q;
	dot = wave_sum(dot);
	if (lane == 0) part[lr] = dot;
	__syncthreads();
	if (threadIdx.x < 6 * sys.cl)
	{
		const int a = threadIdx.x / 6, c = threadIdx.x - 6 * a;
		Scalar s2 = 0;
#pragma unroll
		for (int w = 0; w < ROWS; w++)
			s2 += (a == 0 ? Scalar(1) : agg_weight(blockIdx.x * ROWS + w, sys.agg, g.Pf)) * qrow[w][c];
		if (sys.qpart && sys.agg > 0)
		{
			const int per = sys.agg / ROWS, J = blockIdx.x / per, m = blockIdx.x - J * per;
			sys.qpart[(size_t)m * (6 * sys.cl * sys.nc) + 6 * sys.cl * J + threadIdx.x] = s2;
		}
	}
	if (threadIdx.x == 64)
	{
		Scalar s2 = 0;
#pragma unroll
		for (int w = 0; w < ROWS; w++) s2 += part[w];
		pq_slot(sys, k)[blockIdx.x] = s2;
	}
}

__global__ __launch_bounds__(256) void pcg_update_kernel(DeviceGraph g, DeviceStructure st, DeviceSystem sys, int k, int maxIter, Scalar tol2)
{
	const int lane = threadIdx.x & 63, wv = threadIdx.x >> 6;
	k += *sys.kbase;
	Scalar rzk;
	if (!pcg_active(sys, k, maxIter, tol2, lane, rzk)) return;
	const Scalar pqk = wave_sum(load_parts(pq_slot(sys, k), sys.npq, lane));
	if (!(pqk > 0))
	{
		if (blockIdx.x == 0 && threadIdx.x == 0) *sys.fail = 2;
		return;
// ... 120 lines not shown
	if (doUpdate)
	{
		for (int u = t + PCG2_T; u < sys.nrz; u += PCG2_T) a_k += rz_slot(sys, k)[u];
		for (int u = t + PCG2_T; u < sys.nrz0; u += PCG2_T) a_0 += sys.rz[u];
		if (!PRE) for (int u = t + 2 * PCG2_T; u < sys.npq; u += PCG2_T) a_q += pq_slot(sys, k)[u];
	}
	if (t < ownN) { rown[t] = pre_r; qown[t] = pre_q; }
	for (int w = t + PCG2_T; w < ownN; w += PCG2_T)
	{
		rown[w] = rin[own0 + w];
		qown[w] = doUpdate && !PRE ? sys.ap[own0 + w] : Scalar(0);
	}
	if (doUpdate)
	{
		for (int pj = t; 2 * pj < Nc; pj += PCG2_T)
		{
			Scalar2 s1, s2 = { 0, 0 };
			if (pj == t)
			{
				s1 = sr;
#pragma unroll
				for (int m = 0; m < QV; m++) s2 += qv[m];
			}
			else s1 = *reinterpret_cast<const Scalar2*>(rcin + 2 * pj);
			for (int m0 = pj == t ? QV : 0; !PRE && m0 < per; m0 += QV)
			{
				Scalar2 qx[QV];
				const Scalar* src = sys.qpart + (size_t)m0 * Nc + 2 * pj;
#pragma unroll
				for (int m = 0; m < QV; m++) qx[m] = m0 + m < per ? *reinterpret_cast<const Scalar2*>(src + (size_t)m * Nc) : Scalar2{ 0, 0 };
#pragma unroll
				for (int m = 0; m < QV; m++) s2 += qx[m];
			}
			*reinterpret_cast<Scalar2*>(sR + 2 * pj) = s1;
			*reinterpret_cast<Scalar2*>(sQ + 2 * pj) = s2;
		}
		if (t < NcP - Nc) { sR[Nc + t] = 0; sQ[Nc + t] = 0; }
	}
	else
	{
		for (int jc = t; jc < Nc; jc += PCG2_T)
		{
			const int Jj = jc / CD, rem = jc - CD * Jj;
			const int a = rem / 6, c = rem - 6 * a;
			const int i0 = Jj * sys.agg, i1 = min(g.Pf, i0 + sys.agg);
			Scalar s1 = 0;
			for (int i = i0; i < i1; i += 8)
			{
				Scalar rv[8];
#pragma unroll
				for (int m = 0; m < 8; m++) rv[m] = i + m < i1 ? rin[6 * (size_t)(i + m) + c] : Scalar(0);
#pragma unroll
				for (int m = 0; m < 8; m++) s1 += (a == 0 ? Scalar(1) : agg_weight_local(Jj, i + m - i0, sys, g.Pf)) * rv[m];
			}
			sR[jc] = s1; sQ[jc] = 0;
		}
		if (t < NcP - Nc) { sR[Nc + t] = 0; sQ[Nc + t] = 0; }
	}
	AV ainv2[AR][AC2 > 0 ? AC2 : 1];
	if (AC2 > 0 && Nc > 64 * W * AC)
	{
#pragma unroll
		for (int a = 0; a < AR; a++)
		{
			const PT* Arow = acinv + (size_t)(CD * I + min(wv + 8 * a, CD - 1)) * ld;
#pragma unroll
			for (int m = 0; m < AC2; m++) ainv2[a][m] = *reinterpret_cast<const AV*>(Arow + min(W * lane + 64 * W * (AC + m), ld - W));
		}
	}
	TRACE_MARK();
	a_k = wave_sum(a_k); a_0 = wave_sum(a_0); a_q = wave_sum(a_q);
	if (lane == 0) { wsum[wv] = a_k; wsum[8 + wv] = a_0; wsum[16 + wv] = a_q; }
	__syncthreads();
	Scalar alpha = 0;
	const int kabs = k + __builtin_amdgcn_readfirstlane(kb_v);
	const int failed = __builtin_amdgcn_readfirstlane(failed_v);
	if (doUpdate)
	{
		Scalar rzk = 0, rz0 = 0, pqk = 0;
#pragma unroll
		for (int w = 0; w < PCG2_T / 64; w++) { rzk += wsum[w]; rz0 += wsum[8 + w]; pqk += wsum[16 + w]; }
		if (!(kabs < maxIter && failed == 0 && rzk > tol2 * rz0 && rzk == rzk))
		{
			if (blockIdx.x == 0 && threadIdx.x == 0) { *sys.done = 1; if (!(rzk == rzk)) *sys.fail = 3; }
			return;
		}
		if (!PRE)
		{
			if (!(pqk > 0))
			{
				if (blockIdx.x == 0 && threadIdx.x == 0) *sys.fail = 2;
				return;
			}
			alpha = rzk / pqk;
		}
	}
	TRACE_MARK();
	const int ow = t;
	for (int w = ow; w < ownN; w += PCG2_T)
	{
		const Scalar r = rown[w] - alpha * qown[w];
		rown[w] = r;
		if (doUpdate && !PRE)
		{
			rout[own0 + w] = r;
			sys.xp[own0 + w] = (w == ow ? pre_x : sys.xp[own0 + w]) + alpha * (w == ow ? pre_p : p[own0 + w]);
		}
	}
#pragma unroll
	for (int a = 0; a < AR; a++)
	{
		const int row = wv + 8 * a;
		Scalar acc = 0;
#pragma unroll
		for (int m = 0; m < AC; m++)
		{
			const int j = W * lane + 64 * W * m;
			if (j < Nc)
			{
#pragma unroll
				for (int i = 0; i < W; i++) acc += (Scalar)ainv[a][m][i] * (PRE ? sR[j + i] : sR[j + i] - alpha * sQ[j + i]);
			}
		}
		if (AC2 > 0 && Nc > 64 * W * AC)
		{
#pragma unroll
			for (int m = 0; m < AC2; m++)
			{
				const int j = W * lane + 64 * W * (AC + m);
				if (j < Nc)
				{
#pragma unroll
					for (int i = 0; i < W; i++) acc += (Scalar)ainv2[a][m][i] * (PRE ? sR[j + i] : sR[j + i] - alpha * sQ[j + i]);
				}
			}
		}
		if (row < CD)
			for (int j = lane + 64 * W * (AC + AC2); j < Nc; j += 64) acc += (Scalar)acinv[(size_t)(CD * I + row) * ld + j] * (PRE ? sR[j] : sR[j] - alpha * sQ[j]);
		acc = wave_sum(acc);
		if (lane == 0 && row < CD) yc[row] = acc;
	}
	__syncthreads();
	TRACE_MARK();
	Scalar dot = 0;
	for (int w = ow; w < ownN; w += PCG2_T)
	{
		const int il = w / 6, comp = w - 6 * il;
		Scalar z = yc[comp];
		if (CL == 2) z += agg_weight_local(I, il, sys, g.Pf) * yc[6 + comp];
#pragma unroll
		for (int c = 0; c < 6; c++)
			z += (w == ow ? pre_m[c] : sys.minv[36 * ((size_t)I * sys.agg + il) + c * 6 + comp]) * rown[6 * il + c];
		sys.z[(size_t)own0 + w] = z;
		dot += rown[w] * z;
	}
	dot = wave_sum(dot);
	if (lane == 0) wsum[24 + wv] = dot;
	if (!PRE && t < 8 * CD)
	{
		const int u = t % CD, h = t / CD, a = u / 6, c = u - 6 * a;
		Scalar s3 = 0;
		for (int il = h; 6 * il + c < ownN; il += 8)
			s3 += (a == 0 ? Scalar(1) : agg_weight_local(I, il, sys, g.Pf)) * rown[6 * il + c];
		part[t] = s3;
	}
	__syncthreads();
	if (!PRE && t >= 64 && t < 64 + CD)
// ... 67 lines not shown
	v += dpp_shift<0x118, 0xf>(v);
	v += dpp_shift<0x142, 0xa>(v);
	union { Scalar s; int w[sizeof(Scalar) / 4]; } u, lo, hi;
	u.s = v;
#pragma unroll
	for (int i = 0; i < (int)(sizeof(Scalar) / 4); i++) { lo.w[i] = __builtin_amdgcn_readlane(u.w[i], 31); hi.w[i] = __builtin_amdgcn_readlane(u.w[i], 63); }
	return upperHalf ? hi.s : lo.s;
}

template <int NS>
__device__ __forceinline__ void upper_steps(const DeviceStructure& st, const DeviceSystem& sys, const Scalar* pold, int s0, int b0, int b1, int grp, int c,
	Scalar beta, const Scalar (&pi)[6], Scalar (&acc)[6], Scalar& dotT)
{
	int bb[NS], j[NS], lp[NS]; bool on[NS];
	Scalar2 v[NS][3]; Scalar zj[NS], pjo[NS];
#pragma unroll
	for (int s = 0; s < NS; s++)
	{
		const int b = s0 + 5 * s + grp;
		on[s] = grp < 5 && b < b1;
		bb[s] = on[s] ? b : b0;
	}
#pragma unroll
	for (int s = 0; s < NS; s++) { j[s] = st.hsc_colind[bb[s]]; lp[s] = sys.lowpos[bb[s]]; }
#pragma unroll
	for (int s = 0; s < NS; s++)
	{
		const Scalar2* B2 = reinterpret_cast<const Scalar2*>(sys.hsc + (36 * (size_t)bb[s] + 6 * c));
		v[s][0] = B2[0]; v[s][1] = B2[1]; v[s][2] = B2[2];
	}
#pragma unroll
	for (int s = 0; s < NS; s++) { zj[s] = sys.z[6 * (size_t)j[s] + c]; pjo[s] = pold[6 * (size_t)j[s] + c]; }
#pragma unroll
	for (int s = 0; s < NS; s++)
	{
		const Scalar pj = on[s] ? zj[s] + beta * pjo[s] : Scalar(0);
		const Scalar Bc[6] = { v[s][0].x, v[s][0].y, v[s][1].x, v[s][1].y, v[s][2].x, v[s][2].y };
		Scalar t = 0;
#pragma unroll
		for (int r = 0; r < 6; r++) { acc[r] += Bc[r] * pj; t += Bc[r] * pi[r]; }
		if (on[s] && bb[s] != b0)
		{
			sys.tq[6 * (size_t)lp[s] + c] = t;
			dotT += pj * t;
		}
	}
}

constexpr int UPPER_WAVES = 4;
constexpr int UPPER_ROWS = 2 * UPPER_WAVES;
__global__ __launch_bounds__(64 * UPPER_WAVES, 4) void pcg_spmv_upper_kernel(DeviceGraph g, DeviceStructure st, DeviceSystem sys, int k, int maxIter, Scalar tol2)
{
	const int lane = threadIdx.x & 63, wv = threadIdx.x >> 6;
	const bool hi = lane >= 32;
	const int hl = lane & 31;
	const Scalar* pold = (k & 1) ? sys.p1 : sys.p0;
	Scalar* pnew = (k & 1) ? sys.p0 : sys.p1;
	const int lr = 2 * wv + (hi ? 1 : 0);
	const int row = blockIdx.x * UPPER_ROWS + lr;
	const int kb_v = vector_load_flag(sys.kbase);
	const int failed_v = vector_load_flag(sys.fail) | vector_load_flag(sys.done);
	const Scalar s_k = load_parts(rz_slot(sys, k), sys.nrz, lane);
	const Scalar s_0 = load_parts(sys.rz, sys.nrz0, lane);
	const Scalar s_m = load_parts(rz_slot(sys, k - 1), sys.nrz, lane);
	const bool rowOn = row < g.Pf;
	const int grp = hl / 6, c = hl - 6 * grp;
	TRACE_DECL
	TRACE_MARK();
	int b0 = 0, b1 = 0;
	if (rowOn) { b0 = st.hsc_rowptr[row]; b1 = st.hsc_rowptr[row + 1]; }
	Scalar zi[6], pio[6];
#pragma unroll
	for (int r = 0; r < 6; r++)
	{
		zi[r] = rowOn ? sys.z[6 * (size_t)row + r] : Scalar(0);
		pio[r] = rowOn ? pold[6 * (size_t)row + r] : Scalar(0);
	}
	TRACE_MARK();
	k += __builtin_amdgcn_readfirstlane(kb_v);
	const int failed = __builtin_amdgcn_readfirstlane(failed_v);
	const Scalar rzk = to_uniform(wave_sum(s_k)), rz0 = to_uniform(wave_sum(s_0)), rzm = to_uniform(wave_sum(s_m));
	if (!(k < maxIter && failed == 0 && rzk > tol2 * rz0 && rzk == rzk))
	{
		if (blockIdx.x == 0 && threadIdx.x == 0) { *sys.done = 1; if (!(rzk == rzk)) *sys.fail = 3; }
		return;
	}
	const Scalar beta = k > 0 ? rzk / rzm : Scalar(0);
	Scalar pi[6];
#pragma unroll
	for (int r = 0; r < 6; r++) pi[r] = zi[r] + beta * pio[r];
	Scalar acc[6] = { 0, 0, 0, 0, 0, 0 };
	Scalar dotT = 0;
	const int nb = b1 - b0;
	const int nbMax = max(__builtin_amdgcn_readlane(nb, 0), __builtin_amdgcn_readlane(nb, 32));
	int done = 0;
	for (; done + 10 < nbMax; done += 20) upper_steps<4>(st, sys, pold, b0 + done, b0, b1, grp, c, beta, pi, acc, dotT);
	if (done + 5 < nbMax) upper_steps<2>(st, sys, pold, b0 + done, b0, b1, grp, c, beta, pi, acc, dotT);
	else if (done < nbMax) upper_steps<1>(st, sys, pold, b0 + done, b0, b1, grp, c, beta, pi, acc, dotT);
	TRACE_MARK();
	Scalar qv[6];
#pragma unroll
	for (int r = 0; r < 6; r++) qv[r] = half_wave_sum(acc[r], hi);
	Scalar dot = half_wave_sum(dotT, hi);
#pragma unroll
	for (int r = 0; r < 6; r++) dot += pi[r] * qv[r];
	if (rowOn && hl < 6)
	{
		Scalar q = qv[0], pr = pi[0];
#pragma unroll
		for (int r = 1; r < 6; r++) { q = hl == r ? qv[r] : q; pr = hl == r ? pi[r] : pr; }
		pnew[6 * (size_t)row + hl] = pr;
		sys.ap[6 * (size_t)row + hl] = q;
	}
	__shared__ Scalar part[UPPER_ROWS];
	if (hl == 0) part[lr] = rowOn ? dot : Scalar(0);
	__syncthreads();
	if (threadIdx.x == 0)
	{
		Scalar s2 = 0;
#pragma unroll
		for (int w = 0; w < UPPER_ROWS; w++) s2 += part[w];
		pq_slot(sys, k)[blockIdx.x] = s2;
	}
	TRACE_MARK();
	TRACE_FLUSH(0, blockIdx.x * UPPER_WAVES + wv);
}

constexpr int ROWS_T = 512;
constexpr int ROWS_MAX_AGG = 8 * ROWS_T / 6;
template <int EPT>
__global__ __launch_bounds__(ROWS_T) void pcg_rows_kernel(DeviceGraph g, DeviceStructure st, DeviceSystem sys, int k, int maxIter, Scalar tol2)
{
	extern __shared__ __align__(16) unsigned char rows_lds[];
	Scalar* rown = reinterpret_cast<Scalar*>(rows_lds);
	Scalar* part = rown + 6 * sys.agg;
	Scalar* wsum = part + 96;
	const int t = threadIdx.x, lane = t & 63, wv = t >> 6, I = blockIdx.x;
	const int CD = 6 * sys.cl, Nc = CD * sys.nc;
	const Scalar* p = (k & 1) ? sys.p0 : sys.p1;
	const Scalar* rin = (k & 1) ? sys.r2 : sys.r;
	Scalar* rout = (k & 1) ? sys.r : sys.r2;
	Scalar* rcout = sys.rc + ((k & 1) ? 0 : Nc);
	TRACE_DECL
	TRACE_MARK();
	const int kb_v = vector_load_flag(sys.kbase);
	const int failed_v = vector_load_flag(sys.fail) | vector_load_flag(sys.done);
	Scalar a_k = 0, a_0 = 0, a_q = 0;
	for (int u = t; u < sys.nrz; u += ROWS_T) a_k += rz_slot(sys, k)[u];
	for (int u = t; u < sys.nrz0; u += ROWS_T) a_0 += sys.rz[u];
	{
		const Scalar* pq = pq_slot(sys, k);
		int u = t;
		Scalar q0 = 0, q1 = 0, q2 = 0, q3 = 0;
		for (; u + 3 * ROWS_T < sys.npq; u += 4 * ROWS_T) { const Scalar x0 = pq[u], x1 = pq[u + ROWS_T], x2 = pq[u + 2 * ROWS_T], x3 = pq[u + 3 * ROWS_T]; q0 += x0; q1 += x1; q2 += x2; q3 += x3; }
		for (; u < sys.npq; u += ROWS_T) q0 += pq[u];
		a_q = (q0 + q1) + (q2 + q3);
	}
	const int own0 = 6 * I * sys.agg;
	const int ownN = min(6 * g.Pf, own0 + 6 * sys.agg) - own0;
	Scalar qrow[EPT], rrow[EPT], prow[EPT], xrow[EPT];
#pragma unroll
	for (int e = 0; e < EPT; e++) { qrow[e] = 0; rrow[e] = 0; prow[e] = 0; xrow[e] = 0; }
#pragma unroll
	for (int e = 0; e < EPT; e++)
	{
		const int w = t + e * ROWS_T;
		if (w >= ownN) break;
		const size_t gi = (size_t)own0 + w;
		const int pose = (int)(gi / 6), comp = (int)(gi - 6 * (size_t)pose);
		const int a0 = st.adj_ptr[pose];
		const int nlow = (st.adj_ptr[pose + 1] - a0) - (st.hsc_rowptr[pose + 1] - st.hsc_rowptr[pose]);
		Scalar q = sys.ap[gi];
		rrow[e] = rin[gi]; prow[e] = p[gi]; xrow[e] = sys.xp[gi];
		const Scalar* tin = sys.tq + 6 * (size_t)(a0 - st.hsc_rowptr[pose]) + comp;
		for (int a = 0; a < nlow; a += 16)
		{
			Scalar tv[16];
#pragma unroll
			for (int m = 0; m < 16; m++) tv[m] = tin[6 * (size_t)min(a + m, nlow - 1)];
#pragma unroll
			for (int m = 0; m < 16; m++) q += a + m < nlow ? tv[m] : Scalar(0);
		}
		qrow[e] = q;
	}
	TRACE_MARK();
	a_k = wave_sum(a_k); a_0 = wave_sum(a_0); a_q = wave_sum(a_q);
	if (lane == 0) { wsum[wv] = a_k; wsum[8 + wv] = a_0; wsum[16 + wv] = a_q; }
	__syncthreads();
	TRACE_MARK();
	const int kabs = k + __builtin_amdgcn_readfirstlane(kb_v);
	const int failed = __builtin_amdgcn_readfirstlane(failed_v);
	Scalar rzk = 0, rz0 = 0, pqk = 0;
#pragma unroll
	for (int w = 0; w < ROWS_T / 64; w++) { rzk += wsum[w]; rz0 += wsum[8 + w]; pqk += wsum[16 + w]; }
	if (!(kabs < maxIter && failed == 0 && rzk > tol2 * rz0 && rzk == rzk))
	{
		if (blockIdx.x == 0 && threadIdx.x == 0) { *sys.done = 1; if (!(rzk == rzk)) *sys.fail = 3; }
		return;
	}
	if (!(pqk > 0))
	{
		if (blockIdx.x == 0 && threadIdx.x == 0) *sys.fail = 2;
		return;
	}
	const Scalar alpha = rzk / pqk;
#pragma unroll
	for (int e = 0; e < EPT; e++)
	{
		const int w = t + e * ROWS_T;
		if (w >= ownN) break;
		const Scalar r = rrow[e] - alpha * qrow[e];
		rown[w] = r;
		rout[own0 + w] = r;
		sys.xp[own0 + w] = xrow[e] + alpha * prow[e];
	}
	__syncthreads();
	if (t < 8 * CD)
	{
		const int u = t % CD, h = t / CD, a = u / 6, c = u - 6 * a;
		Scalar s3 = 0;
		for (int il = h; 6 * il + c < ownN; il += 8)
			s3 += (a == 0 ? Scalar(1) : agg_weight_local(I, il, sys, g.Pf)) * rown[6 * il + c];
		part[t] = s3;
	}
	__syncthreads();
	if (t < CD)
	{
		Scalar s3 = 0;
#pragma unroll
		for (int h = 0; h < 8; h++) s3 += part[CD * h + t];
		rcout[CD * I + t] = s3;
	}
	TRACE_MARK();
	TRACE_FLUSH(2, blockIdx.x * (ROWS_T / 64) + wv);
}

typedef void (*PcgRowsKernel)(DeviceGraph, DeviceStructure, DeviceSystem, int, int, Scalar);
int pcg_rows_entries_per_thread(const DeviceSystem& sys)
{
	const int entries = 6 * sys.agg;
	return entries <= 2 * ROWS_T ? 2 : entries <= 4 * ROWS_T ? 4 : 8;
}
static PcgRowsKernel pcg_rows_kernel_for(const DeviceSystem& sys)
{
	const int ept = pcg_rows_entries_per_thread(sys);
	return ept == 2 ? pcg_rows_kernel<2> : ept == 4 ? pcg_rows_kernel<4> : pcg_rows_kernel<8>;
}
int pcg_rows_max_aggregate() { return ROWS_MAX_AGG; }

__global__ __launch_bounds__(256) void build_lowpos_kernel(DeviceStructure st, int Pf, int* __restrict__ lowpos)
{
	const int row = blockIdx.x * 256 + threadIdx.x;
	if (row >= Pf) return;
	const int a0 = st.adj_ptr[row];
	const int nlow = (st.adj_ptr[row + 1] - a0) - (st.hsc_rowptr[row + 1] - st.hsc_rowptr[row]);
	const int base = a0 - st.hsc_rowptr[row];
	for (int a = 0; a < nlow; a++) lowpos[st.adj_blk[a0 + a] & 0x7fffffff] = base + a;
}

void launch_build_lowpos(const DeviceGraph& g, const DeviceStructure& st, int* lowpos, hipStream_t s)
{
	if (g.Pf > 0) hipLaunchKernelGGL(build_lowpos_kernel, dim3((g.Pf + 255) / 256), dim3(256), 0, s, st, g.Pf, lowpos);
}

static void* spmv_upper_kernel_for(const DeviceSystem&) { return (void*)pcg_spmv_upper_kernel; }
int spmv_upper_grid(int Pf) { return (Pf + UPPER_ROWS - 1) / UPPER_ROWS; }
static size_t rows_lds_bytes(const DeviceSystem& sys) { return sizeof(Scalar) * (6 * (size_t)sys.agg + 96 + 24); }

void launch_pcg_upper_iteration(const DeviceGraph& g, const DeviceStructure& st, const DeviceSystem& sys, int k, int maxIter, Scalar tol2, hipStream_t s, int which)
{
	typedef void (*K3)(DeviceGraph, DeviceStructure, DeviceSystem, int, int, Scalar);
	if (which & 1) hipLaunchKernelGGL((K3)spmv_upper_kernel_for(sys), dim3(spmv_upper_grid(g.Pf)), dim3(64 * UPPER_WAVES), 0, s, g, st, sys, k, maxIter, tol2);
	if (which & 2) hipLaunchKernelGGL(pcg_rows_kernel_for(sys), dim3(sys.nc), dim3(ROWS_T), rows_lds_bytes(sys), s, g, st, sys, k, maxIter, tol2);
	if (which & 4)
		hipLaunchKernelGGL((void (*)(DeviceGraph, DeviceSystem, int, int, int, Scalar, int))pcg2_kernel_for(sys, true), dim3(sys.nc), dim3(PCG2_T), pcg2_lds_bytes(sys), s,
			g, sys, k, k + 1, maxIter, tol2, 1);
}

static bool spmv_wants_occupancy(const DeviceGraph& g) { return 2 * (long long)g.Pf > 3 * 1024; }
int spmv_rows_for(int Pf)
{
	return 2 * (long long)Pf > 3 * 1024 ? 4 : 2;
}
static bool spmv_row_per_wave(const DeviceSystem& sys) { return sys.spmv_rows >= 4; }
static void* spmv_kernel_for(const DeviceGraph&, const DeviceSystem& sys)
{
	return sys.spmv_rows == 4 ? (void*)pcg_spmv_row_kernel<4> : (void*)pcg_spmv_kernel<2, 1>;
}
static dim3 spmv_block_for(const DeviceSystem& sys) { return dim3((spmv_row_per_wave(sys) ? 64 : 128) * sys.spmv_rows); }

void launch_pcg_spmv(const DeviceGraph& g, const DeviceStructure& st, const DeviceSystem& sys, int k, int maxIter, Scalar tol2, hipStream_t s)
{
	const dim3 grid((g.Pf + sys.spmv_rows - 1) / sys.spmv_rows);
	hipLaunchKernelGGL((void (*)(DeviceGraph, DeviceStructure, DeviceSystem, int, int, Scalar))spmv_kernel_for(g, sys), grid, spmv_block_for(sys), 0, s, g, st, sys, k, maxIter, tol2);
}

void launch_pcg_update(const DeviceGraph& g, const DeviceStructure& st, const DeviceSystem& sys, int k, int maxIter, Scalar tol2, hipStream_t s)
{
	hipLaunchKernelGGL(pcg_update_kernel, dim3((g.Pf + 39) / 40), dim3(256), 0, s, g, st, sys, k, maxIter, tol2);
}

__device__ __forceinline__ void pcg_advance_body(const DeviceSystem& sys, int n, int report, Scalar tol2)
{
	if (tol2 >= 0 && n > 0)
	{
		const int lane = threadIdx.x;
		const Scalar rzk = wave_sum(load_parts(rz_slot(sys, 0), sys.nrz, lane)), rz0 = wave_sum(load_parts(sys.rz, sys.nrz0, lane));
		if (lane == 0 && *sys.done == 0 && *sys.fail == 0 && !(rzk > tol2 * rz0))
		{
			*sys.done = 1;
			if (!(rzk == rzk)) *sys.fail = 3;
		}
	}
	if (threadIdx.x != 0) return;
	*sys.kbase += n;
	if (report && sys.host_flags) publish_report(sys);
}

__global__ __launch_bounds__(64) void pcg_advance_kernel(DeviceSystem sys, int n, int report, Scalar tol2) { pcg_advance_body(sys, n, report, tol2); }

__global__ __launch_bounds__(64) void pcg_advance_batch_kernel(const BatchEntry* __restrict__ tab, int n, int report, Scalar tol2)
{
	if (tab[blockIdx.x].gridSpmv == 0) return;
	pcg_advance_body(tab[blockIdx.x].sys, n, report, tol2);
}

__global__ void collect_eval_kernel(const Scalar* slots, Scalar* out)
{
	if (threadIdx.x == 0) { out[0] = slots[0]; out[1] = slots[NSLOT]; out[2] = slots[3 * NSLOT]; }
}

void launch_collect_eval(const DeviceSystem& sys, Scalar* out3, hipStream_t s)
{
	hipLaunchKernelGGL(collect_eval_kernel, dim3(1), dim3(64), 0, s, sys.slots, out3);
}

void launch_pcg_report(const DeviceSystem& sys, hipStream_t s)
{
	hipLaunchKernelGGL(pcg_advance_kernel, dim3(1), dim3(64), 0, s, sys, 0, 1, Scalar(-1));
}

void launch_pcg_advance(const DeviceSystem& sys, int n, hipStream_t s, Scalar tol2)
{
	hipLaunchKernelGGL(pcg_advance_kernel, dim3(1), dim3(64), 0, s, sys, n, 1, tol2);
}

template <int CL, int AC, int AC2, int W>
static void* pcg2_batch_fn() { return (void*)pcg2_fused_batch_kernel<CL, AC, AC2, W>; }
static void* pcg2_batch_kernel_for(const DeviceSystem& sys)
{
	const int Nc = 6 * sys.cl * sys.nc;
	if (sys.acinv32 && sizeof(Scalar) == 8)
	{
		if (sys.cl == 2) return Nc <= 768 ? pcg2_batch_fn<2, 3, 0, 4>() : Nc <= 1536 ? pcg2_batch_fn<2, 6, 0, 4>() : pcg2_batch_fn<2, 6, 3, 4>();
		return Nc <= 768 ? pcg2_batch_fn<1, 3, 0, 4>() : Nc <= 1536 ? pcg2_batch_fn<1, 6, 0, 4>() : pcg2_batch_fn<1, 6, 3, 4>();
	}
	const bool small = Nc <= 768;
	if (sys.cl == 2) return small ? pcg2_batch_fn<2, 6, 0, 2>() : pcg2_batch_fn<2, 12, 6, 2>();
	return small ? pcg2_batch_fn<1, 6, 0, 2>() : pcg2_batch_fn<1, 12, 6, 2>();
}

int batch_kernel_class(const DeviceGraph& g, const DeviceSystem& sys)
{
	if (sys.agg <= 0 || sys.upper || sys.spmv_rows != 2) return -1;
	const int Nc = 6 * sys.cl * sys.nc;
	const int cls = (sys.acinv32 && sizeof(Scalar) == 8) ? (Nc <= 768 ? 0 : Nc <= 1536 ? 1 : 2) : (Nc <= 768 ? 3 : 4);
	return (cls * 2 + (sys.cl == 2 ? 1 : 0)) * 2 + (spmv_wants_occupancy(g) ? 1 : 0);
}

size_t batch_pcg2_lds_bytes(const DeviceSystem& sys) { return pcg2_lds_bytes(sys); }

void launch_pcg_batch_iteration(const BatchEntry* tab, int n, const DeviceGraph& g0, const DeviceSystem& sys0, int gridSpmvMax, int ncMax, size_t ldsMax, int k, Scalar tol2, hipStream_t s)
{
	void* spmv = 2LL * gridSpmvMax * n * 2 > 3 * 1024 || spmv_wants_occupancy(g0) ? (void*)pcg_spmv_batch_kernel<2, 4> : (void*)pcg_spmv_batch_kernel<2, 1>;
	hipLaunchKernelGGL((void (*)(const BatchEntry*, int, Scalar))spmv, dim3(gridSpmvMax, n), dim3(256), 0, s, tab, k, tol2);
	hipLaunchKernelGGL((void (*)(const BatchEntry*, int, int, Scalar, int))pcg2_batch_kernel_for(sys0), dim3(ncMax, n), dim3(PCG2_T), ldsMax, s, tab, k, k + 1, tol2, 1);
}

void launch_batch_first_precond(const BatchEntry* tab, int n, const DeviceSystem& sys0, int ncMax, size_t ldsMax, Scalar tol2, hipStream_t s)
{
	hipLaunchKernelGGL((void (*)(const BatchEntry*, int, int, Scalar, int))pcg2_batch_kernel_for(sys0), dim3(ncMax, n), dim3(PCG2_T), ldsMax, s, tab, 0, 0, tol2, 0);
}

void launch_pcg_batch_advance(const BatchEntry* tab, int n, int iters, hipStream_t s, Scalar tol2)
{
	hipLaunchKernelGGL(pcg_advance_batch_kernel, dim3(n), dim3(64), 0, s, tab, iters, 1, tol2);
}

void launch_pcg_iteration(const DeviceGraph& g, const DeviceStructure& st, const DeviceSystem& sys, int k, int maxIter, Scalar tol2, hipStream_t s)
{
	launch_pcg_spmv(g, st, sys, k, maxIter, tol2, s);
	launch_pcg_update(g, st, sys, k, maxIter, tol2, s);
}

template <typename... Args>
static hipError_t add_kernel_node(hipGraph_t graph, hipGraphNode_t& last, void* fn, dim3 grid, dim3 block, unsigned lds, Args... args)
{
	void* ptrs[] = { (void*)&args... };
	hipKernelNodeParams p = {};
	p.func = fn; p.gridDim = grid; p.blockDim = block; p.sharedMemBytes = lds; p.kernelParams = ptrs; p.extra = nullptr;
	hipGraphNode_t node = nullptr;
	const hipError_t e = hipGraphAddKernelNode(&node, graph, last ? &last : nullptr, last ? 1 : 0, &p);
	last = node;
	return e;
}

hipError_t graph_add_pcg_chunk(hipGraph_t graph, const DeviceGraph& g, const DeviceStructure& st, const DeviceSystem& sys, int chunk, int maxIter, Scalar tol2, int report)
{
	hipGraphNode_t last = nullptr;
	hipError_t e = hipSuccess;
	for (int k = 0; k < chunk && e == hipSuccess; k++)
	{
		if (sys.upper && sys.agg > 0)
		{
			e = add_kernel_node(graph, last, spmv_upper_kernel_for(sys), dim3(spmv_upper_grid(g.Pf)), dim3(64 * UPPER_WAVES), 0, g, st, sys, k, maxIter, tol2);
			if (e == hipSuccess) e = add_kernel_node(graph, last, (void*)pcg_rows_kernel_for(sys), dim3(sys.nc), dim3(ROWS_T), (unsigned)rows_lds_bytes(sys), g, st, sys, k, maxIter, tol2);
			if (e == hipSuccess) e = add_kernel_node(graph, last, pcg2_kernel_for(sys, true), dim3(sys.nc), dim3(PCG2_T), (unsigned)pcg2_lds_bytes(sys), g, sys, k, k + 1, maxIter, tol2, 1);
			continue;
		}
		e = add_kernel_node(graph, last, spmv_kernel_for(g, sys), dim3((g.Pf + sys.spmv_rows - 1) / sys.spmv_rows), spmv_block_for(sys), 0, g, st, sys, k, maxIter, tol2);
		if (e != hipSuccess) break;
		if (sys.agg > 0)
		{
			e = add_kernel_node(graph, last, pcg2_kernel_for(sys), dim3(sys.nc), dim3(PCG2_T),
				(unsigned)pcg2_lds_bytes(sys), g, sys, k, k + 1, maxIter, tol2, 1);
		}
		else e = add_kernel_node(graph, last, (void*)pcg_update_kernel, dim3((g.Pf + 39) / 40), dim3(256), 0, g, st, sys, k, maxIter, tol2);
	}
	if (e == hipSuccess) e = add_kernel_node(graph, last, (void*)pcg_advance_kernel, dim3(1), dim3(64), 0, sys, chunk, report, tol2);
	return e;
}


}


#ifdef CUBA_HIP_TRACE
extern "C" int cuba_hip_debug_read_trace(unsigned long long* out)
{
	return (int)hipMemcpyFromSymbol(out, HIP_SYMBOL(cubahip::cuba_trace_buf), sizeof(unsigned long long) * 3 * 8192 * 8);
}
#endif
```

cuda-bundle-adjustment_amd/csrc/ba_setup.hip:

```cpp
#include "ba_solver.hpp"

using namespace cubahip;

void cuba_hip_solver::finishValues()
{
	if (!valuesPending) return;
	valuesPending = false;
	HIP_TRY(hipStreamWaitEvent(stream, evValues, 0));
	topo::launch_gather_edges(d_perm.data(), d_rawEp.data(), d_rawEl.data(), d_rawDim.data(), d_rawMeas.data(), d_rawOmega.data(), E,
		nullptr, nullptr, d_mu.data(), d_mv.data(), d_mr.data(), d_w.data(), stream);
	sortedValuesValid = true;
}

void cuba_hip_solver::setGraph(int Pt_, int Pf_, int Lt_, int Lf_, const double* q, const double* t, const double* cam, const double* Xw,
	int E_, const int32_t* ep, const int32_t* el, const uint8_t* edim, const double* meas, const double* omega, bool deferValues, int ownLo, int ownHi)
{
	const bool ranged = ownHi >= 0;
	if (ranged && (ownLo < 0 || ownHi > Lt_ || ownLo > ownHi)) throw ArgError{ "bad landmark range" };
	if (ranged) deferValues = false;
	if (valuesPending) { HIP_TRY(hipStreamSynchronize(upStream)); valuesPending = false; sortedValuesValid = false; }
	deferredUpload = false;
	if (Pt_ < 0 || Lt_ < 0 || E_ < 0 || Pf_ < 0 || Pf_ > Pt_ || Lf_ < 0 || Lf_ > Lt_) throw ArgError{ "bad vertex counts" };
	if (Pt_ >= STEREO_BIT) throw ArgError{ "too many poses" };
	if (sizeof(Scalar) == 4 && Lt_ >= (1 << 23)) throw ArgError{ "fp32 build: at most 2^23 - 1 landmarks" };
// ... 95 lines not shown
		lap("set_graph: device sort + gather enqueued");
	}
	else
	{
	resetPoseOrder();
	if (!sameInput)
	{
	h_inEp.assign(ep, ep + E); h_inEl.assign(el, el + E); h_inDim.assign(edim, edim + E);
	h_lmptr.assign(Lt + 1, 0);
	for (int e = 0; e < E; e++) h_lmptr[el[e] + 1]++;
	for (int l = 0; l < Lt; l++) h_lmptr[l + 1] += h_lmptr[l];
	perm.assign(E, 0);
	{
		std::vector<int> cursor(h_lmptr.begin(), h_lmptr.end() - 1);
		for (int e = 0; e < E; e++) perm[cursor[el[e]]++] = e;
		std::vector<long long> byEdges(h_lmptr.begin(), h_lmptr.end());
		parallelRows(Lt, byEdges, [&](int l) {
			std::sort(perm.begin() + h_lmptr[l], perm.begin() + h_lmptr[l + 1],
				[&](int a, int b) { return ep[a] != ep[b] ? ep[a] < ep[b] : a < b; });
		});
	}
	}
	lap("set_graph: validate + sort edges");
	std::vector<int>& sPose = h_spose[sameInput ? topoSlot : topoSlot ^ 1];
	std::vector<int>& sLm = h_slm[sameInput ? topoSlot : topoSlot ^ 1];
	sPose.resize(E); sLm.resize(E);
	std::vector<Scalar>&mu = h_stage[0], &mv = h_stage[1], &mr = h_stage[2], &w = h_stage[3];
	mu.resize(E); mv.resize(E); mr.resize(E); w.resize(E);
	h_epose.resize(E);
	{
		parallelFor(E, [&](int i) {
			const int e = perm[i];
			if (!sameInput)
			{
				h_epose[i] = ep[e];
				sPose[i] = ep[e] | (edim[e] == 3 ? STEREO_BIT : 0);
				sLm[i] = el[e];
			}
			mu[i] = meas[3 * (size_t)e]; mv[i] = meas[3 * (size_t)e + 1];
			mr[i] = edim[e] == 3 ? meas[3 * (size_t)e + 2] : 0.0;
			w[i] = omega[e];
		});
	}
	sameTopology = sameCounts && hostTopoValid && (sameInput || (sPose == h_spose[topoSlot] && sLm == h_slm[topoSlot]));
	if (!sameInput) topoSlot ^= 1;
	lap("set_graph: gather sorted arrays");
	if (!sameInput || devTopology) { d_epose.upload(sPose, stream); d_elm.upload(sLm, stream); d_lmptr.upload(h_lmptr, stream); }
	d_mu.upload(mu, stream); d_mv.upload(mv, stream); d_mr.upload(mr, stream); d_w.upload(w, stream);
	cntValueBytes += (int64_t)E * 4 * (int64_t)sizeof(Scalar);
	devTopology = false; hostTopoValid = true;
	}
	const size_t nState = (size_t)7 * Pt + (size_t)3 * Lt;
	if (sizeof(Scalar) == sizeof(double) && !reorderActive)
	{
		d_state.resize(nState); d_cam.resize((size_t)5 * Pt);
		Scalar* ds = d_state.data();
		if (Pt)
		{
			HIP_TRY(hipMemcpyAsync(ds, q, sizeof(double) * 4 * (size_t)Pt, hipMemcpyHostToDevice, stream));
			HIP_TRY(hipMemcpyAsync(ds + 4 * (size_t)Pt, t, sizeof(double) * 3 * (size_t)Pt, hipMemcpyHostToDevice, stream));
			HIP_TRY(hipMemcpyAsync(d_cam.data(), cam, sizeof(double) * 5 * (size_t)Pt, hipMemcpyHostToDevice, stream));
		}
		if (Lt) HIP_TRY(hipMemcpyAsync(ds + 7 * (size_t)Pt, Xw, sizeof(double) * 3 * (size_t)Lt, hipMemcpyHostToDevice, stream));
	}
	else
	{
		if (!reorderActive) stageState();
		d_state.upload(state, stream);
		d_cam.upload(camv, stream);
	}
	if (!useDev && lmOrderActive) { lmOrderActive = false; }
	if (lmOrderActive) landmarkRowsInPlace(d_state.data() + 7 * (size_t)Pt, Lt, 3, true);
	d_backup.resize(nState);
	dropSnapshots();
	d_perEdge.resize(E);
	if (!h_pinned)
	{
		HIP_TRY(hipHostMalloc((void**)&h_pinned, 4096, hipHostMallocMapped | hipHostMallocCoherent));
		std::memset(h_pinned, 0, 4096);
		void* dev = nullptr;
		HIP_TRY(hipHostGetDevicePointer(&dev, h_pinned, 0));
		slotsDev = (Scalar*)dev; flagsDev = (int*)((char*)dev + 1024);
	}
	d_parts.resize(8192 + (size_t)E + 64); d_maxdiag.resize(64); d_fail.resize(1); d_iters.resize(1); d_kbase.resize(1); d_done.resize(1); d_ticket.resize(1);
	d_fail.zero(stream); d_iters.zero(stream); d_kbase.zero(stream); d_done.zero(stream); d_ticket.zero(stream);
	if (deferredUpload)
	{
		if (!upStream) { HIP_TRY(hipStreamCreateWithFlags(&upStream, hipStreamNonBlocking)); HIP_TRY(hipEventCreateWithFlags(&evValues, hipEventDisableTiming)); }
		HIP_TRY(hipEventRecord(evValues, stream)); HIP_TRY(hipStreamWaitEvent(upStream, evValues, 0));
		HIP_TRY(hipMemcpyAsync(d_rawMeas.data(), meas, sizeof(double) * 3 * (size_t)E, hipMemcpyHostToDevice, upStream));
		HIP_TRY(hipMemcpyAsync(d_rawOmega.data(), omega, sizeof(double) * (size_t)E, hipMemcpyHostToDevice, upStream));
		HIP_TRY(hipEventRecord(evValues, upStream));
		cntValueBytes += (int64_t)E * 32;
		deferredUpload = false;
	}
	sync(); expectedTicket = 0; ((volatile int*)((char*)h_pinned + 1024))[3] = 0;
	sync();

	lap("set_graph: alloc + upload + sync");
	g = DeviceGraph();
	g.Pt = Pt; g.Pf = Pf; g.Lt = Lt; g.Lf = Lf; g.E = E;
	g.q = d_state.data(); g.t = d_state.data() + 4 * (size_t)Pt; g.Xw = d_state.data() + 7 * (size_t)Pt;
	g.cam = d_cam.data();
	g.e_pose = d_epose.data(); g.e_lm = d_elm.data(); g.lm_ptr = d_lmptr.data();
	g.e_mu = d_mu.data(); g.e_mv = d_mv.data(); g.e_mr = d_mr.data(); g.e_w = d_w.data();
	g.rk[0] = rk[0]; g.rk[1] = rk[1];
	g.e_begin = 0; g.e_end = E;
	partLo = ranged ? ownLo : 0; partHi = ranged ? ownHi : -1;
	valuesPartial = ranged && useDev;
	if (sameTopology)
	{
		DeviceGraph a = gOld, b = g;
		a.rk[0] = a.rk[1] = b.rk[0] = b.rk[1] = RobustKernel();
		if (std::memcmp(&a, &b, sizeof(DeviceGraph)) != 0) dropPcgGraph();
		haveStructure = true;
	}
	coarseValid = false; startRunHistory();
	haveGraph = true;
	lambda = 0;
	for (double& v : prof) v = 0;
	cntPcgIters = cntTrials = cntCoarseRefresh = cntPcgLooks = cntPcgEnqueued = cntPcgUnconverged = 0;
	cntCoarseInline = cntFp32Fallbacks = 0;
	pcgHistory.clear();
	cntUploads++;
	prof[0] += std::chrono::duration<double>(Clock::now() - t0).count();
}

void cuba_hip_solver::buildStructure()
{
	if (!haveGraph) throw StateError{ "set_graph must be called first" };
	if (haveStructure) return;
	if (gjStream) { HIP_TRY(hipStreamSynchronize(gjStream)); pendingInv = -1; assemblePending = false; }
	if (devTopology && deviceSetup) { buildStructureDevice(); return; }
	localRanges = false;
	if (reorderActive) { std::vector<int> id(Pf); for (int i = 0; i < Pf; i++) id[i] = i; applyPoseOrder(id); }
	ensureHostTopology();
	const auto t0 = Clock::now();
	std::vector<int> nfree(Lf, 0);
	std::vector<long long> pairBase(Lf, 0);
	nmul = 0;
	long long npairs = 0;
	parallelFor(Lf, [&](int l) {
		int n = 0;
		for (int i = h_lmptr[l]; i < h_lmptr[l + 1]; i++) n += h_epose[i] < Pf;
		nfree[l] = n;
	});
	for (int l = 0; l < Lf; l++)
	{
		const int n = nfree[l];
		pairBase[l] = npairs;
		npairs += (long long)n * (n - 1) / 2;
		nmul += (long long)n * (n + 1) / 2;
	}
	if (npairs >= (1LL << 31)) throw ArgError{ "graph too dense: more than 2^31 Schur block products" };
	lap(nullptr);
	std::vector<int> peAllPtr(Pf + 1, 0);
	std::vector<int>& peAll = h_work[5];
	{
		const int T = (int)std::min<long long>(HostPool::instance().maxThreads(), E / 50000 + 1);
		std::vector<int> hist((size_t)T * Pf, 0);
		auto range = [&](int t) { return std::make_pair((int)((long long)E * t / T), (int)((long long)E * (t + 1) / T)); };
		HostPool::instance().run(T, [&](int t) {
			int* h = hist.data() + (size_t)t * Pf;
			for (int i = range(t).first; i < range(t).second; i++) if (h_epose[i] < Pf) h[h_epose[i]]++;
		});
		int run = 0;
		for (int ps = 0; ps < Pf; ps++)
		{
// ... 896 lines not shown
```

cuda-bundle-adjustment_amd/csrc/ba_solver.hip:

```cpp
#include "ba_solver.hpp"

using namespace cubahip;


namespace cubahip_host
{
std::atomic<int> g_liveHandles{ 0 };
}

namespace
{
std::string g_createError;

template <typename F>
int guarded(cuba_hip_solver* s, F&& f)
{
	if (!s) return CUBA_HIP_ERR_INVALID_ARGUMENT;
	try
	{
		if (hipSetDevice(s->device) != hipSuccess) { s->lastError = "hipSetDevice failed"; return CUBA_HIP_ERR_RUNTIME; }
		f();
		return CUBA_HIP_OK;
	}
	catch (const HipError& e)
// ... 41 lines not shown
	}
	std::free(p);
}

const char* cuba_hip_version(void) { return sizeof(Scalar) == 8 ? "cuba-hip 0.1 (gfx950, fp64)" : "cuba-hip 0.1 (gfx950, fp32)"; }
int cuba_hip_scalar_size(void) { return (int)sizeof(Scalar); }

int cuba_hip_create(int device, cuba_hip_solver** out)
{
	if (!out) return CUBA_HIP_ERR_INVALID_ARGUMENT;
	*out = nullptr;
	int n = 0;
	if (hipGetDeviceCount(&n) != hipSuccess || n <= 0) return CUBA_HIP_ERR_NO_DEVICE;
	if (device < 0 || device >= n) return CUBA_HIP_ERR_INVALID_ARGUMENT;
	if (hipSetDevice(device) != hipSuccess) return CUBA_HIP_ERR_RUNTIME;
	cuba_hip_solver* s = new (std::nothrow) cuba_hip_solver;
	if (!s) return CUBA_HIP_ERR_RUNTIME;
	s->device = device;
	if (hipStreamCreateWithFlags(&s->stream, hipStreamNonBlocking) != hipSuccess) { delete s; return CUBA_HIP_ERR_RUNTIME; }
	s->ownStream = true;
	g_liveHandles.fetch_add(1, std::memory_order_relaxed);
	*out = s;
	return CUBA_HIP_OK;
}

int cuba_hip_destroy(cuba_hip_solver* s)
{
	if (!s) return CUBA_HIP_ERR_INVALID_ARGUMENT;
	(void)hipSetDevice(s->device);
	(void)hipStreamSynchronize(s->stream);
	delete s;
	g_liveHandles.fetch_sub(1, std::memory_order_relaxed);
	return CUBA_HIP_OK;
}

const char* cuba_hip_last_error(const cuba_hip_solver* s) { return s ? s->lastError.c_str() : "null solver handle"; }

int cuba_hip_set_stream(cuba_hip_solver* s, void* hip_stream)
{
	return guarded(s, [&] {
		s->sync();
		if (s->ownStream && s->stream) { HIP_TRY(hipStreamDestroy(s->stream)); s->ownStream = false; }
		s->stream = (hipStream_t)hip_stream;
	});
}

int cuba_hip_set_option(cuba_hip_solver* s, const char* key, double value)
{
	return guarded(s, [&] {
		if (!key) throw ArgError{ "null key" };
		const std::string k(key);
		if (k == "pcg_tol") s->pcgTol = value;
		else if (k == "pcg_max_iter") { s->pcgMaxIter = (int)value; s->haveStructure = false; }
		else if (k == "heuristics") { s->heuristics = value != 0; s->firstInvValid = false; s->firstInvPending = false; }
		else if (k == "precond_fp32") { s->precondFp32 = value != 0; s->haveStructure = false; s->coarseValid = false; s->dropPcgGraph(); }
		else if (k == "pose_reorder") { s->poseReorder = value != 0; s->haveStructure = false; }
		else if (k == "device_setup") { s->deviceSetup = value != 0; s->haveStructure = false; }
		else if (k == "mixed_precision") s->mixedPrecision = value != 0 && sizeof(Scalar) == 8;
		else if (k == "pcg_accept_unconverged") s->acceptUnconverged = value != 0;
		else if (k == "direct_fallback") { s->directFallback = value != 0; s->directSticky = false; }
		else if (k == "direct_after") s->directAfter = (int)value;
		else if (k == "direct_max_tiles") { s->directMaxTiles = (int)value; s->directRefused = false; s->directPlanValid = false; }
		else if (k == "direct_slack") { s->directSlack = (int)value; s->directRefused = false; s->directPlanValid = false; }
		else if (k == "reduced_solver")
		{
			if (value != 0 && value != 1) throw ArgError{ "reduced_solver: 0 = block PCG with the exact solver as fallback, 1 = exact sparse Cholesky for every solve" };
			s->directAlways = value != 0;
		}
		else if (k == "pcg_aggregate") { s->pcgAggregate = (int)value; s->haveStructure = false; }
		else if (k == "coarse_linear") { s->coarseLinear = value != 0; s->haveStructure = false; }
		else if (k == "covariance_workspace_mb")
		{
			if (value < 0 || value > (double)(1 << 30)) throw ArgError{ "covariance_workspace_mb must lie in 0 .. 2^30 (0 = automatic)" };
			s->covWorkspaceMb = value;
		}
		else if (k == "landmark_reorder") s->lmReorder = value != 0;
		else if (k == "reduction_chunks")
		{
			if (value < 0 || value > 64) throw ArgError{ "reduction_chunks must lie in 0 .. 64" };
			s->redChunks = (int)value; s->haveStructure = false;
		}
		else if (k == "spmv_upper") { s->spmvUpper = (int)value; s->haveStructure = false; s->dropPcgGraph(); }
		else if (k == "pcg_graph") { s->useGraph = value != 0; s->dropPcgGraph(); }
		else if (k == "profile") s->profile = value != 0;
		else throw ArgError{ "unknown option: " + k };
	});
}


int cuba_hip_hint_unchanged(cuba_hip_solver* s, int same_edges, int same_values)
{
	return guarded(s, [&] { s->hintSameEdges = same_edges != 0; s->hintSameValues = same_edges != 0 && same_values != 0; });
}

int cuba_hip_set_graph(cuba_hip_solver* s, int Pt, int Pf, int Lt, int Lf, const double* q, const double* t, const double* cam,
	const double* Xw, int E, const int32_t* edge_pose, const int32_t* edge_landmark, const uint8_t* edge_dim,
	const double* meas, const double* omega)
{
	return guarded(s, [&] { s->setGraph(Pt, Pf, Lt, Lf, q, t, cam, Xw, E, edge_pose, edge_landmark, edge_dim, meas, omega); });
}

int cuba_hip_set_graph_begin(cuba_hip_solver* s, int Pt, int Pf, int Lt, int Lf, const double* q, const double* t, const double* cam,
	const double* Xw, int E, const int32_t* edge_pose, const int32_t* edge_landmark, const uint8_t* edge_dim,
	const double* meas, const double* omega)
{
	return guarded(s, [&] { s->setGraph(Pt, Pf, Lt, Lf, q, t, cam, Xw, E, edge_pose, edge_landmark, edge_dim, meas, omega, true); });
}

int cuba_hip_set_graph_partition(cuba_hip_solver* s, int Pt, int Pf, int Lt, int Lf,
	const double* q, const double* t, const double* cam, const double* Xw,
	int E, const int32_t* edge_pose, const int32_t* edge_landmark, const uint8_t* edge_dim,
	const double* meas, const double* omega, int landmark_begin, int landmark_end)
{
	return guarded(s, [&] {
		if (landmark_end < 0) throw ArgError{ "bad landmark range" };
		s->setGraph(Pt, Pf, Lt, Lf, q, t, cam, Xw, E, edge_pose, edge_landmark, edge_dim, meas, omega, false, landmark_begin, landmark_end);
	});
}

int cuba_hip_set_graph_end(cuba_hip_solver* s)
{
	return guarded(s, [&] {
		if (!s->haveGraph) throw StateError{ "set_graph_begin must be called first" };
		if (s->upStream) HIP_TRY(hipStreamSynchronize(s->upStream));
		s->finishValues();
	});
}

int cuba_hip_set_robust_kernel(cuba_hip_solver* s, int edge_type, int kind, double delta)
{
	return guarded(s, [&] {
		if (edge_type < 0 || edge_type > 1 || kind < 0 || kind > 2) throw ArgError{ "bad robust kernel" };
		s->rk[edge_type] = RobustKernel{ kind, (Scalar)delta };
	});
}

int cuba_hip_build_structure(cuba_hip_solver* s) { return guarded(s, [&] { s->buildStructure(); s->sync(); }); }

int cuba_hip_compute_errors(cuba_hip_solver* s, double* chi2)
{
	return guarded(s, [&] { if (!chi2) throw ArgError{ "null output" }; *chi2 = s->computeErrors(); });
}

int cuba_hip_build_system(cuba_hip_solver* s) { return guarded(s, [&] { s->need(); }); }

int cuba_hip_max_diagonal(cuba_hip_solver* s, double* v)
{
	return guarded(s, [&] { if (!v) throw ArgError{ "null output" }; *v = s->maxDiagonal(); });
}

int cuba_hip_set_lambda(cuba_hip_solver* s, double lambda) { return guarded(s, [&] { s->lambda = lambda; }); }
int cuba_hip_restore_diagonal(cuba_hip_solver* s) { return guarded(s, [&] { s->lambda = 0; }); }

int cuba_hip_schur(cuba_hip_solver* s) { return guarded(s, [&] { s->schur(); }); }

int cuba_hip_schur_parts(cuba_hip_solver* s, int* n_parts)
{
	return guarded(s, [&] { s->need(); if (n_parts) *n_parts = s->schurParts(); });
}

int cuba_hip_schur_part(cuba_hip_solver* s, int part, size_t ranges[4])
{
	return guarded(s, [&] { size_t r[4]; s->schurPart(part, r); if (ranges) std::copy(r, r + 4, ranges); });
}

int cuba_hip_solve_reduced(cuba_hip_solver* s, int* ok)
// ... 66 lines not shown
		if (niterations < 0) throw ArgError{ "negative iteration count" };
		const int b = cuba_hip_optimize_batch_impl(handles, n, niterations, chi2_per_iter, n_done);
		if (batched_solves) *batched_solves = b;
	});
}

int cuba_hip_get_solution(cuba_hip_solver* s, double* q, double* t, double* Xw)
{
	return guarded(s, [&] {
		if (!s->haveGraph) throw StateError{ "set_graph must be called first" };
		const Scalar* base = s->d_state.data();
		if (q) { s->downloadAsDouble(base, q, (size_t)4 * s->Pt); s->permutePoseArray(q, 4, false); }
		if (t) { s->downloadAsDouble(base + 4 * (size_t)s->Pt, t, (size_t)3 * s->Pt); s->permutePoseArray(t, 3, false); }
		if (Xw) s->downloadAsDouble(s->landmarkRowsForCaller(base + 7 * (size_t)s->Pt, s->Lt, 3), Xw, (size_t)3 * s->Lt);
	});
}

int cuba_hip_set_solution(cuba_hip_solver* s, const double* q, const double* t, const double* Xw)
{
	return guarded(s, [&] {
		if (!s->haveGraph) throw StateError{ "set_graph must be called first" };
		s->buildStructure();
		Scalar* base = s->d_state.data();
		if (q) { std::vector<double> v(q, q + (size_t)4 * s->Pt); s->permutePoseArray(v.data(), 4, true); s->uploadFromDouble(base, v.data(), v.size()); }
		if (t) { std::vector<double> v(t, t + (size_t)3 * s->Pt); s->permutePoseArray(v.data(), 3, true); s->uploadFromDouble(base + 4 * (size_t)s->Pt, v.data(), v.size()); }
		if (Xw)
		{
			s->uploadFromDouble(base + 7 * (size_t)s->Pt, Xw, (size_t)3 * s->Lt);
			if (s->lmOrderActive) s->landmarkRowsInPlace(base + 7 * (size_t)s->Pt, s->Lt, 3, true);
		}
	});
}

int cuba_hip_chi_squares(cuba_hip_solver* s, double* out)
{
	return guarded(s, [&] { if (!out && s->E) throw ArgError{ "null output" }; s->chiSquares(out); });
}

int cuba_hip_chi_squares_begin(cuba_hip_solver* s, double* out)
{
	return guarded(s, [&] { if (!out && s->E) throw ArgError{ "null output" }; s->chiSquares(out, false); });
}

int cuba_hip_chi_squares_end(cuba_hip_solver* s)
{
	return guarded(s, [&] { s->sync(); });
}

int cuba_hip_get_profile(cuba_hip_solver* s, double seconds[CUBA_HIP_PROFILE_ITEMS])
{
	return guarded(s, [&] { for (int i = 0; i < CUBA_HIP_PROFILE_ITEMS; i++) seconds[i] = s->prof[i]; });
}

int cuba_hip_get_counters(cuba_hip_solver* s, int64_t c[8])
{
	return guarded(s, [&] {
		c[0] = s->cntPcgIters; c[1] = s->cntTrials; c[2] = s->st.nblk; c[3] = s->nmul;
		c[4] = s->cntCoarseRefresh; c[5] = s->cntPcgLooks; c[6] = s->cntPcgEnqueued; c[7] = 6 * (int64_t)s->sys.cl * s->sys.nc;
	});
}

int cuba_hip_get_counter(cuba_hip_solver* s, const char* name, int64_t* value)
{
	return guarded(s, [&] {
		if (!name || !value) throw ArgError{ "null argument" };
		const std::string k(name);
		if (k == "pcg_iterations") *value = s->cntPcgIters;
		else if (k == "lm_trials") *value = s->cntTrials;
		else if (k == "coarse_refreshes") *value = s->cntCoarseRefresh;
		else if (k == "coarse_inline_inversions") *value = s->cntCoarseInline;
		else if (k == "pcg_host_looks") *value = s->cntPcgLooks;
		else if (k == "pcg_iterations_enqueued") *value = s->cntPcgEnqueued;
		else if (k == "pcg_unconverged_solves") *value = s->cntPcgUnconverged;
		else if (k == "pcg_graph_instantiations") *value = s->gb.builds.load();
		else if (k == "precond_fp32_fallbacks") *value = s->cntFp32Fallbacks;
		else if (k == "pcg_iterations_plain_launches") *value = s->cntPcgPlain;
		else if (k == "host_looks") *value = s->cntHostLooks;
		else if (k == "exact_solve_fallbacks") *value = s->cntDirect;
		else if (k == "exact_solve_failures") *value = s->cntDirectFailed;
		else if (k == "graph_uploads") *value = s->cntUploads;
		else if (k == "structure_builds") *value = s->cntStructureBuilds;
		else if (k == "value_bytes_uploaded") *value = s->cntValueBytes;
		else if (k == "late_decision_records") *value = s->cntLateRecords;
		else if (k == "covariance_ns") *value = (int64_t)(1e9 * s->covSeconds);
		else if (k == "covariance_pairs_ns") *value = (int64_t)(1e9 * s->covPairsSeconds);
		else if (k == "covariance_pairs_chunks") *value = s->covPairChunks;
		else throw ArgError{ "unknown counter: " + k };
	});
}

int cuba_hip_get_pcg_history(cuba_hip_solver* s, int32_t* iterations, int capacity, int* n_solves, int64_t* n_unconverged)
{
	return guarded(s, [&] {
		const int n = (int)s->pcgHistory.size();
		if (n_solves) *n_solves = n;
		if (n_unconverged) *n_unconverged = s->cntPcgUnconverged;
		if (iterations) for (int i = 0; i < std::min(n, capacity); i++) iterations[i] = s->pcgHistory[i];
	});
}

int cuba_hip_get_hsc_structure(cuba_hip_solver* s, int32_t* row_ptr, int32_t* col_ind, int* nblk)
{
	return guarded(s, [&] {
		s->need();
		s->ensureHostPattern();
		if (nblk) *nblk = (int)s->h_colind.size();
		if (!s->reorderActive)
		{
			if (row_ptr) std::memcpy(row_ptr, s->h_rowptr.data(), sizeof(int) * s->h_rowptr.size());
			if (col_ind) std::memcpy(col_ind, s->h_colind.data(), sizeof(int) * s->h_colind.size());
			return;
		}
		const auto blocks = s->callerBlocks();
		if (row_ptr)
		{
			for (int i = 0; i <= s->Pf; i++) row_ptr[i] = 0;
			for (const auto& b : blocks) row_ptr[(int)(b.key >> 32) + 1]++;
			for (int i = 0; i < s->Pf; i++) row_ptr[i + 1] += row_ptr[i];
		}
		if (col_ind) for (size_t k = 0; k < blocks.size(); k++) col_ind[k] = (int)(uint32_t)blocks[k].key;
	});
}

int cuba_hip_get_array(cuba_hip_solver* s, int which, double* out, size_t* count)
{
	return guarded(s, [&] {
		s->need();
		const Scalar* src = nullptr; size_t n = 0;
		switch (which)
		{
		case CUBA_HIP_ARRAY_BP: src = s->sys.bp; n = (size_t)6 * s->Pf; break;
		case CUBA_HIP_ARRAY_BSC: src = s->sys.bsc; n = (size_t)6 * s->Pf; break;
		case CUBA_HIP_ARRAY_XP: src = s->sys.xp; n = (size_t)6 * s->Pf; break;
		case CUBA_HIP_ARRAY_XL: src = s->sys.xl; n = (size_t)3 * s->Lf; break;
		case CUBA_HIP_ARRAY_LM_SYS: src = s->sys.lm_sys; n = (size_t)9 * s->Lf; break;
		case CUBA_HIP_ARRAY_HSC: src = s->sys.hsc; n = (size_t)36 * s->st.nblk; break;
		default: throw ArgError{ "unknown array id" };
		}
		if (count) *count = n;
		if (out && n)
		{
			if (which == CUBA_HIP_ARRAY_XL) src = s->landmarkRowsForCaller(src, s->Lf, 3);
			else if (which == CUBA_HIP_ARRAY_LM_SYS) src = s->landmarkRowsForCaller(src, s->Lf, 9);
			s->downloadAsDouble(src, out, n);
			if (s->reorderActive)
			{
				if (which == CUBA_HIP_ARRAY_BP || which == CUBA_HIP_ARRAY_BSC || which == CUBA_HIP_ARRAY_XP) s->permutePoseArray(out, 6, false);
				else if (which == CUBA_HIP_ARRAY_HSC)
				{
					const std::vector<double> v(out, out + n);
					const auto blocks = s->callerBlocks();
					for (size_t k = 0; k < blocks.size(); k++)
					{
						const double* src36 = v.data() + 36 * (size_t)blocks[k].src;
						double* dst = out + 36 * k;
						for (int c = 0; c < 6; c++)
							for (int r = 0; r < 6; r++) dst[c * 6 + r] = blocks[k].transposed ? src36[r * 6 + c] : src36[c * 6 + r];
					}
				}
			}
		}
	});
}

int cuba_hip_compute_covariance(cuba_hip_solver* s, double* pose_cov, double* landmark_cov, int* not_positive_definite)
{
// ... 474 lines not shown
```

cuda-bundle-adjustment_amd/csrc/ba_solver.hpp:

```cpp
#pragma once

#include <algorithm>
#include <chrono>
#include <cmath>
#include <cstdarg>
#include <cstdio>
#include <cstdlib>
#include <cstring>
#include <numeric>
#include <string>
#include <thread>
#include <atomic>
#include <functional>
#include <condition_variable>
#include <deque>
#include <map>
#include <mutex>
#include <vector>

#include "../../include/cuba_hip.h"
#include "ba_kernels.hpp"
#include "host_pool.hpp"
#include "ba_structure.hpp"

// ... 9 lines not shown
		hipError_t err__ = (expr);                                       \
		if (err__ != hipSuccess) throw HipError{ err__, #expr, __FILE__, __LINE__ }; \
	} while (0)

struct StateError { std::string msg; };
struct ArgError { std::string msg; };

template <typename T>
class DevBuf
{
public:
	DevBuf() = default;
	DevBuf(const DevBuf&) = delete;
	DevBuf& operator=(const DevBuf&) = delete;
	~DevBuf() { release(); }
	void release()
	{
		if (ptr_) (void)hipFree(ptr_);
		ptr_ = nullptr; size_ = cap_ = 0;
	}
	void resize(size_t n)
	{
		if (n > cap_)
		{
			release();
			if (n) HIP_TRY(hipMalloc((void**)&ptr_, n * sizeof(T)));
			static const int poison = std::getenv("CUBA_HIP_POISON") ? std::max(1, std::atoi(std::getenv("CUBA_HIP_POISON"))) : 0;
			static std::atomic<unsigned> poisonCount{ 0 };
			static const int pattern[4] = { 0x3f, 0x40, 0x3e, 0x41 };
			if (n && poison) { HIP_TRY(hipMemset(ptr_, poison >= 2 ? pattern[poisonCount++ & 3] : 0x7f, n * sizeof(T))); HIP_TRY(hipDeviceSynchronize()); }
			cap_ = n;
		}
		size_ = n;
	}
	void upload(const std::vector<T>& h, hipStream_t s)
	{
		resize(h.size());
		if (!h.empty()) HIP_TRY(hipMemcpyAsync(ptr_, h.data(), h.size() * sizeof(T), hipMemcpyHostToDevice, s));
	}
	void uploadRaw(const T* h, size_t n, hipStream_t s)
	{
		resize(n);
		if (n) HIP_TRY(hipMemcpyAsync(ptr_, h, n * sizeof(T), hipMemcpyHostToDevice, s));
	}
	void zero(hipStream_t s) { if (size_) HIP_TRY(hipMemsetAsync(ptr_, 0, size_ * sizeof(T), s)); }
	T* data() const { return ptr_; }
	size_t size() const { return size_; }
private:
	T* ptr_ = nullptr;
	size_t size_ = 0, cap_ = 0;
};

using Clock = std::chrono::steady_clock;

extern std::atomic<int> g_liveHandles;

constexpr int CUBA_HIP_BATCH_MAX = 64;

void upload_selinv_plan(const SelInvPlan& p, DevBuf<int>& ints, SelInv& view, hipStream_t s);

struct PairWork { DevBuf<Scalar> X; DevBuf<int> ints; };
int run_covariance_pairs(const SparseChol& d, const SparseCholPlan& plan, const DeviceGraph& g, const DeviceSystem& sys, const Scalar* W,
	const PairRequest& rq, size_t budgetBytes, PairWork& w, Scalar* out, hipStream_t s);

}
using namespace cubahip_host;

struct cuba_hip_solver;
int cuba_hip_optimize_batch_impl(cuba_hip_solver** hs, int n, int niter, double* chi2, int* nDone);

struct cuba_hip_solver
{
	int device = 0;
	hipStream_t stream = nullptr;
	bool ownStream = false;
	std::string lastError;

	double pcgTol = sizeof(Scalar) == 8 ? 1e-7 : 1e-4;
	int pcgMaxIter = 0;
	int coarseLinear = 1;
	int pcgAggregate = -1;
	int spmvUpper = -1;
	DevBuf<Scalar> d_tq; DevBuf<int> d_lowpos;
	bool deviceSetup = true;
	bool devTopology = false;
	bool hostTopoValid = false;
	static int bitsFor(long long n) { int b = 1; while ((1LL << b) < n + 1) b++; return b; }
	DevBuf<int> d_rawEp, d_rawEl, d_counters, d_tmpI0, d_tmpI1, d_adjRow, d_lowerPtr, d_chunk;
	DevBuf<uint8_t> d_rawDim;
	DevBuf<double> d_rawMeas, d_rawOmega, d_chiCaller;
	DevBuf<int> d_ownIds; DevBuf<double> d_ownVals;
	std::vector<int> h_ownIds; std::vector<double> h_ownVals;
	int64_t cntValueBytes = 0;
	bool valuesPartial = false;
	DevBuf<uint32_t> d_perm, d_k32a, d_k32b, d_v32a, d_v32b;
	DevBuf<uint64_t> d_k64a, d_k64b, d_v64a, d_v64b;
	DevBuf<unsigned char> d_topoTemp;
	DevBuf<long long> d_pairCount, d_freeCount, d_freeScan;
	bool poseReorder = true;
	bool reorderActive = false, reorderTried = false;
	std::vector<int> poseNewOfOld, poseOldOfNew;
	DevBuf<int> d_rawEpCaller, d_poseMap;
	bool lmReorder = true;
	bool lmOrderActive = false;
	DevBuf<int> d_lmMap, d_rawElCaller, d_lmFirst, d_lmLast;
	DevBuf<Scalar> d_rowTmp;
	bool landmarkOrderAllowed() const { return lmReorder && Lf > 1 && E > 0 && (partHi < 0 || (partLo <= 0 && partHi >= Lt)); }
	void switchLandmarkOrder(bool on);
	void computeLandmarkOrder();
	void resetLandmarkOrder();
	void landmarkRowsInPlace(Scalar* rows, int nrows, int width, bool toInternal);
	const Scalar* landmarkRowsForCaller(const Scalar* rows, int nrows, int width);
	bool mixedPrecision = false;
	bool profile = false;

	int Pt = 0, Pf = 0, Lt = 0, Lf = 0, E = 0;
	bool haveGraph = false, haveStructure = false;
	int partLo = 0, partHi = -1;
	struct RedPart { BlockPassRange od; size_t blkBegin, blkEnd; };
	int redChunks = 0;
	std::vector<RedPart> redParts;
	void cutReductionParts();
	int schurParts() const { return redParts.empty() ? 1 : (int)redParts.size(); }
	void schurPart(int part, size_t ranges[4]);
	bool partsByCaller = false;
	std::vector<int> perm;
	std::vector<int> h_lmptr, h_epose;
	RobustKernel rk[2] = { { 0, 0 }, { 0, 0 } };

	DevBuf<Scalar> d_state, d_backup, d_cam;
	std::map<int, DevBuf<Scalar>> d_snapshots;
	void dropSnapshots() { d_snapshots.clear(); }
	DevBuf<int> d_epose, d_elm, d_lmptr;
	DevBuf<Scalar> d_mu, d_mv, d_mr, d_w, d_perEdge;
	DevBuf<int> d_waveLm, d_bigLm, d_rowptr, d_colind, d_lmNfree, d_adjPtr, d_adjBlk, d_adjCol;
	DevBuf<int2> d_ell;
	DevBuf<long long> d_lmPairBase;
	DevBuf<Scalar> d_red;
	DevBuf<Scalar> d_parts, d_lmSys, d_lmInv, d_xp, d_xl, d_minv, d_r, d_z, d_p0, d_p1, d_ap, d_rz, d_pq;
	DevBuf<unsigned long long> d_maxdiag;
	DevBuf<int> d_fail, d_iters, d_kbase, d_done, d_ticket;
	DevBuf<Scalar> d_eval;
	DevBuf<Scalar> d_coarse[3], d_gjPivots, d_rc, d_r2, d_qpart, d_hrow;
	DevBuf<float> d_coarse32[2];
	DevBuf<Scalar> d_firstInv; DevBuf<float> d_firstInv32;
	bool firstInvValid = false, firstInvPending = false;
	bool heuristics = true;
	bool precondFp32 = sizeof(Scalar) == 8;
	bool fp32Inverse() const { return precondFp32 && sizeof(Scalar) == 8; }
	size_t inv32Count() const { const size_t n = (size_t)6 * sys.cl * sys.nc; return n * ((n + 3) & ~(size_t)3); }
	DevBuf<int> d_blkrow, d_odBlocks, d_prodPtr, d_prodEa, d_prodEb, d_prodLm, d_pePtr, d_peEdge;
	DevBuf<int> d_prodBeg, d_prodEnd, d_peBeg, d_peEnd;
	bool localRanges = false;
	DevBuf<Scalar> d_erec;
	DevBuf<int> d_cbI, d_cbJ, d_cbPtr, d_cbBlk;
	DevBuf<Scalar> d_cbWi, d_cbWj;
	std::vector<int> h_rowptr, h_colind;
	Scalar* h_pinned = nullptr;
	Scalar* slotsDev = nullptr;
	int* flagsDev = nullptr;
	Scalar* hostStage() const { return (Scalar*)((char*)h_pinned + 2048); }
	Scalar slot(int i) const { return ((const volatile Scalar*)h_pinned)[i]; }

	DeviceGraph g;
	DeviceStructure st;
	DeviceSystem sys;

	std::map<std::pair<int, const Scalar*>, hipGraphExec_t> pcgGraphs;
	bool useGraph = graphsByDefault();
	static bool graphsByDefault() { const char* e = std::getenv("CUBA_HIP_GRAPHS"); return e && e[0] == '1'; }
	hipStream_t captureStream = nullptr;
	hipStream_t capStream()
	{
		if (!captureStream) HIP_TRY(hipStreamCreateWithFlags(&captureStream, hipStreamNonBlocking));
		return captureStream;
	}

	struct GraphJob { int chunk; const Scalar* acinv; DeviceGraph g; DeviceStructure st; DeviceSystem sys; int maxIter; Scalar tol2; uint64_t gen; };
	struct GraphBuilder
	{
		std::thread th;
		std::mutex m;
		std::condition_variable cv;
		std::deque<GraphJob> jobs;
		std::map<std::pair<int, const Scalar*>, hipGraphExec_t> ready;
		std::map<std::pair<int, const Scalar*>, int> requested;
		std::vector<hipGraphExec_t> trash;
		uint64_t gen = 0;
		bool stop = false, busy = false;
		std::atomic<int64_t> builds{ 0 };
		std::atomic<double> seconds{ 0.0 };
	} gb;
	void graphWorker();
	hipGraphExec_t pcgGraphIfReady(int chunk, int maxIter, Scalar tol2);
	void dropPcgGraph();
	std::map<int, int> batchRequests;

	void enqueuePcgIteration(int k, int maxIter, Scalar tol2, hipStream_t s)
	{
		if (sys.agg > 0 && sys.upper) launch_pcg_upper_iteration(g, st, sys, k, maxIter, tol2, s);
		else if (sys.agg > 0)
		{
			launch_pcg_spmv(g, st, sys, k, maxIter, tol2, s);
			launch_pcg2_fused(g, sys, k, k + 1, maxIter, tol2, 1, s);
		}
		else launch_pcg_iteration(g, st, sys, k, maxIter, tol2, s);
	}

	Scalar pcgGraphTol2 = 0; int pcgGraphMaxIter = 0;
	const void* graphsOrderedFor = nullptr;

	bool coarseValid = false;
	int sideAge = 0;
	int overlapPeriod() const
	{
		const int Nc = 6 * sys.cl * sys.nc;
		return Nc <= 512 ? 1 : Nc <= 1024 ? 2 : 3;
	}
	hipStream_t gjStream = nullptr;
	hipEvent_t evSetup = nullptr, evAssembled = nullptr, evInverse = nullptr, evFirstInv = nullptr;
	int pendingInv = -1;
	bool assemblePending = false;
	void ensureOverlapObjects();
	void waitAssembled() { if (assemblePending) { HIP_TRY(hipStreamWaitEvent(stream, evAssembled, 0)); assemblePending = false; } }
	void drainInversion()
	{
		if (pendingInv >= 0) { HIP_TRY(hipStreamWaitEvent(stream, evInverse, 0)); pendingInv = -1; }
		assemblePending = false;
	}
	struct PatternEntry { uint64_t key; int ea, eb; };
	std::vector<PatternEntry> h_ent; std::vector<int> h_work[6];
	std::vector<double> h_chiSorted;
	std::vector<Scalar> h_stage[6];
	std::vector<int> h_inEp, h_inEl; std::vector<uint8_t> h_inDim;
	std::vector<int> h_spose[2], h_slm[2];
	int topoSlot = 0;
	std::vector<int> runIters;
	std::vector<int> prevRunIters;
	void startRunHistory() { if (!runIters.empty()) prevRunIters.swap(runIters); runIters.clear(); directSticky = false; }
	int firstSolveIters = 0;

	double lambda = 0;
	int maxIterAlloc = 0;
	long long nmul = 0;
	int64_t cntPcgIters = 0, cntTrials = 0, cntCoarseRefresh = 0, cntPcgLooks = 0, cntPcgEnqueued = 0, cntPcgUnconverged = 0;
	int64_t cntPcgPlain = 0;
	int64_t cntCoarseInline = 0;
	int64_t cntFp32Fallbacks = 0;
	int64_t cntUploads = 0;
	bool acceptUnconverged = false;
	std::vector<int> pcgHistory;
	double prof[CUBA_HIP_PROFILE_ITEMS] = { 0, 0, 0, 0, 0, 0, 0, 0 };

	~cuba_hip_solver()
	{
		{ std::lock_guard<std::mutex> lk(gb.m); gb.stop = true; gb.jobs.clear(); }
		gb.cv.notify_all();
		if (gb.th.joinable()) gb.th.join();
		for (hipGraphExec_t e : gb.trash) (void)hipGraphExecDestroy(e);
		gb.trash.clear();
		dropPcgGraph();
		if (gjStream) { (void)hipStreamSynchronize(gjStream); (void)hipStreamDestroy(gjStream); (void)hipEventDestroy(evSetup); (void)hipEventDestroy(evAssembled); (void)hipEventDestroy(evInverse); (void)hipEventDestroy(evFirstInv); }
		if (captureStream) (void)hipStreamDestroy(captureStream);
		if (upStream) { (void)hipStreamSynchronize(upStream); (void)hipStreamDestroy(upStream); (void)hipEventDestroy(evValues); }
		if (h_tileStage) (void)hipHostFree(h_tileStage);
		if (evTileInputs) (void)hipEventDestroy(evTileInputs);
		if (h_pinned) (void)hipHostFree(h_pinned);
		if (h_lmRing) (void)hipHostFree(h_lmRing);
		if (h_batchTab) (void)hipHostFree(h_batchTab);
		if (h_gjTab) { (void)hipHostFree(h_gjTab); (void)hipEventDestroy(evGjTab); }
		for (hipEvent_t e : batchEvents) (void)hipEventDestroy(e);
		if (ownStream && stream) (void)hipStreamDestroy(stream);
	}

	void sync() { HIP_TRY(hipStreamSynchronize(stream)); }

	bool failDirty = true;
	int expectedTicket = 0;
	bool hintSameEdges = false, hintSameValues = false;
	void noteReport() { expectedTicket++; }
	void waitReport();

	void downloadAsDouble(const Scalar* dsrc, double* hdst, size_t n);
	void uploadFromDouble(Scalar* ddst, const double* hsrc, size_t n);

	template <class F>
	static void parallelRows(int nrows, const std::vector<long long>& start, F&& fn)
	{
		const long long total = nrows > 0 ? start[nrows] - start[0] : 0;
		const int T = (int)std::min<long long>(HostPool::instance().maxThreads(), total / 50000 + 1);
		if (T <= 1) { for (int i = 0; i < nrows; i++) fn(i); return; }
		std::vector<int> cut(T + 1, 0);
		for (int t = 1; t < T; t++)
		{
			const long long target = start[0] + total * t / T;
			cut[t] = std::max(cut[t - 1], (int)(std::upper_bound(start.begin(), start.begin() + nrows + 1, target) - start.begin()) - 1);
		}
		cut[T] = nrows;
		HostPool::instance().run(T, [&](int t) { for (int i = cut[t]; i < cut[t + 1]; i++) fn(i); });
	}

	template <class F>
	static void parallelFor(int n, F&& fn)
	{
		const int T = (int)std::min<long long>(HostPool::instance().maxThreads(), n / 50000 + 1);
		if (T <= 1) { for (int i = 0; i < n; i++) fn(i); return; }
		HostPool::instance().run(T, [&](int t) {
			const int r0 = (int)((long long)n * t / T), r1 = (int)((long long)n * (t + 1) / T);
			for (int i = r0; i < r1; i++) fn(i);
		});
	}

	Clock::time_point lapT;
	void lap(const char* what)
	{
		static const bool on = std::getenv("CUBA_HIP_DEBUG") != nullptr;
		if (!on) return;
		const auto now = Clock::now();
		if (what) std::fprintf(stderr, "[cuba_hip] %-34s %7.2f ms\n", what, 1e3 * std::chrono::duration<double>(now - lapT).count());
		lapT = now;
	}

	struct StageTimer
	{
		cuba_hip_solver* s; int item; Clock::time_point t0;
		StageTimer(cuba_hip_solver* s_, int item_) : s(s_), item(item_)
		{
			if (s->profile) { s->sync(); t0 = Clock::now(); }
		}
		~StageTimer()
		{
			if (s->profile)
			{
				(void)hipStreamSynchronize(s->stream);
				s->prof[item] += std::chrono::duration<double>(Clock::now() - t0).count();
			}
		}
	};

	hipStream_t upStream = nullptr; hipEvent_t evValues = nullptr;
	bool valuesPending = false, deferredUpload = false;
	bool sortedValuesValid = false;
	int* h_tileStage = nullptr; size_t tileStageCap = 0; hipEvent_t evTileInputs = nullptr;
	void finishValues();
	void setGraph(int Pt_, int Pf_, int Lt_, int Lf_, const double* q, const double* t, const double* cam, const double* Xw,
		int E_, const int32_t* ep, const int32_t* el, const uint8_t* edim, const double* meas, const double* omega, bool deferValues = false,
		int ownLo = 0, int ownHi = -1);

	void buildStructure();

	struct CoarseCfg { int agg, cl, nc, spmvRows; };
	CoarseCfg coarseConfig() const;

	int rzStrideCfg = 1, pqStrideCfg = 1;
	void allocSystem(int nblk, const CoarseCfg& c);

	static bool rowGroupedBlocks(long long products) { return products > (1LL << 19); }
	std::vector<int> rowGroupedOrder(const int* blkRow, const int* blkCol, const int* cnt, int nblk) const;
	int diagProdBlocks = 0;
	int heavyBlocks = 0;
	void publishStructure(int nblk, int nWaves, int nBig, int nOd, int nCb, int ellM, int ellOver, const CoarseCfg& c);
// ... 111 lines not shown
	bool solveReduced();

	bool directFallback = true;
	bool directAlways = false;
	int directAfter = 0;
	int directMaxTiles = 1 << 20;
	int directSlack = -1;
	bool directSticky = false;
	bool directRefused = false;
	bool directPlanValid = false;
	double directSeconds = 0, directPlanSeconds = 0;
	SparseCholPlan directPlan;
	SparseChol directDev;
	DevBuf<Scalar> d_scTiles, d_scTilesT, d_scY, d_scRinv;
	DevBuf<int> d_scInts, d_scFail;
	int64_t cntDirect = 0, cntDirectFailed = 0;
	int64_t directPlanBuilds = 0;
	bool directUsable() const { return directFallback && !directRefused && Pf > 0; }
	int pcgBudget(int maxIter) const;
	bool ensureDirectPlan();
	bool solveDirect();

	SelInvPlan selPlan;
	int64_t selPlanFor = -1;
	SelInv selDev;
	DevBuf<int> d_selInts;
	DevBuf<Scalar> d_sigma, d_covW, d_covPose, d_covBlk, d_covLm;
	bool covBlocksValid = false;
	double covSeconds = 0;
	bool computeCovariance(double* poseCov, double* lmCov);
	void covarianceBlocks(double* out);
	double covWorkspaceMb = 0;
	double covPairsSeconds = 0;
	int covPairChunks = 0;
	PairWork covPairWork;
	DevBuf<Scalar> d_pairOut;
	bool computeCovariancePairs(int n, const int32_t* kindA, const int32_t* indexA, const int32_t* kindB, const int32_t* indexB, double* out);

	struct CoarseJob { cuba_hip_solver* h; int first; bool firstInvCopy; bool ownEvent; };
	void launchCoarseJobs(std::vector<CoarseJob>& jobs, hipEvent_t common = nullptr);
	GjJob* h_gjTab = nullptr; DevBuf<unsigned char> d_gjTab; hipEvent_t evGjTab = nullptr;
	struct SolveCtx
	{
		int maxIter = 0, budget = 0, predicted = 32, k0 = 0, looks = 0, eagerIters = 0;
		int itersDone = -1;
		Scalar tol2 = 0;
		bool twoLevel = false, direct = false, graphs = false, converged = false, result = false;
		bool batched = false;
		std::vector<CoarseJob>* deferCoarse = nullptr;
		bool deferLaunch = false;
		bool deferred = false;
		const Scalar* copySrc = nullptr; Scalar* copyDst = nullptr; size_t copyCount = 0;
		volatile int* hInts = nullptr;
		Clock::time_point tSolve0;
	};
	bool solveBegin(SolveCtx& sc);
	bool solveBrokeDown(SolveCtx& sc);
	bool solveEnd(SolveCtx& sc);
	bool solveReducedOnce();
	bool retryWithFp64Inverse(bool ok);

	void backSubstitute();

	bool solve();

	void update();

	double computeScale(double lam);

	void push() { need(); HIP_TRY(hipMemcpyAsync(d_backup.data(), d_state.data(), d_state.size() * sizeof(Scalar), hipMemcpyDeviceToDevice, stream)); }
	void pop() { need(); HIP_TRY(hipMemcpyAsync(d_state.data(), d_backup.data(), d_state.size() * sizeof(Scalar), hipMemcpyDeviceToDevice, stream)); }

	int optimize(int niter, double* chi2Out);
	int optimizeDeviceDecision(int niter, double* chi2Out);
	struct LmRun
	{
		static constexpr int maxq = 10;
		int niter = 0, enq = 0, seen = 0, done = 0, rejRun = 0;
		bool stop = false;
		double lam = 0, F = 0, tagBase = 0;
		double* chi2Out = nullptr;
		LmDevice lm;
	};
	void lmRunBegin(LmRun& r, int niter, double* chi2Out);
	void lmAbsorb(LmRun& r, int upto);
	bool lmBeforeTrial(LmRun& r);
	bool lmAfterSolveHost(LmRun& r);
	bool lmAfterSolve(LmRun& r, bool ok);
	bool fullyBatchable() const;
	int lmRunEnd(LmRun& r);
	bool batchable() const;
	std::vector<hipEvent_t> batchEvents;
	BatchEntry* h_batchTab = nullptr; int batchTabEntries = 0;
	DevBuf<unsigned char> d_batchTab;
	DevBuf<double> d_lmState; DevBuf<Scalar> d_lamS;
	double* h_lmRing = nullptr; double* lmRingDev = nullptr; uint64_t lmRunNonce = 0; int64_t cntLateRecords = 0;
	int64_t cntHostLooks = 0;

	void enqueueEvaluate(double lam, bool withScale);
	void readEvaluate(bool withScale, double* Fhat, double* scale);
	void evaluateTrial(double lam, bool withScale, double* Fhat, double* scale);


	void timeKernels(int reps, double* msOut);

	void chiSquares(double* out, bool wait = true);
};
```

Before: 818.0 million.

## Publish PCG convergence early from device and start LM on device

When PCG graphs are off, the first PCG kernel that detects convergence now publishes the host report immediately, so the host spin-wait can return before the rest of the enqueued batch drains. The advance kernel then skips its duplicate report, and the host waiter accepts tickets at or past the expected value. PCG batches are sized exactly, with a smaller prediction margin and finer continuation steps. LM start (initial chi2, max diagonal, lambda) is computed by a new device kernel, removing host round-trips. The trade-off is extra ticket and flag bookkeeping that could desynchronise the host and device.

```diff
diff --git a/cuda-bundle-adjustment_amd/csrc/ba_device.hpp b/cuda-bundle-adjustment_amd/csrc/ba_device.hpp
--- a/cuda-bundle-adjustment_amd/csrc/ba_device.hpp
+++ b/cuda-bundle-adjustment_amd/csrc/ba_device.hpp
@@ -215,4 +215,12 @@
 	__hip_atomic_store(&sys.host_flags[3], t, __ATOMIC_RELAXED, __HIP_MEMORY_SCOPE_SYSTEM);
 }
 
-}
+__device__ __forceinline__ void pcg_raise_done(const DeviceSystem& sys, Scalar rzk)
+{
+	const bool first = sys.early != nullptr && vector_load_flag(sys.done) == 0;
+	*sys.done = 1;
+	if (!(rzk == rzk)) *sys.fail = 3;
+	if (first && sys.host_flags) { *sys.early = 1; publish_report(sys); }
+}
+
+}
diff --git a/cuda-bundle-adjustment_amd/csrc/ba_edge.hip b/cuda-bundle-adjustment_amd/csrc/ba_edge.hip
--- a/cuda-bundle-adjustment_amd/csrc/ba_edge.hip
+++ b/cuda-bundle-adjustment_amd/csrc/ba_edge.hip
@@ -623,6 +623,26 @@
 	t.restoreGrid = (unsigned)std::min<size_t>(512, (stateCount + 255) / 256);
 }
 
+__global__ __launch_bounds__(64) void lm_start_kernel(const Scalar* slots, const unsigned long long* maxdiag, double* lmState, Scalar* lmLam, double tau, double maxq, double tagBase)
+{
+#pragma clang fp contract(off)
+	double v = __longlong_as_double((long long)maxdiag[threadIdx.x]);
+#pragma unroll
+	for (int o = 32; o > 0; o >>= 1) v = fmax(v, __shfl_xor(v, o));
+	if (threadIdx.x != 0) return;
+	double F = 0;
+	for (int i = 0; i < NSLOT; i++) F += (double)slots[i];
+	const double lam = tau * v;
+	lmState[0] = F; lmState[1] = lam; lmState[2] = 2.0; lmState[3] = 0.0; lmState[4] = 0.0; lmState[5] = 1.0; lmState[6] = 0.0; lmState[7] = maxq;
+	lmState[8] = tagBase;
+	lmLam[0] = (Scalar)lam;
+}
+
+void launch_lm_start(const DeviceSystem& sys, const Scalar* slots, const LmDevice& lm, double tau, int maxq, double tagBase, hipStream_t s)
+{
+	hipLaunchKernelGGL(lm_start_kernel, dim3(1), dim3(64), 0, s, slots, sys.maxdiag, lm.state, lm.lam, tau, (double)maxq, tagBase);
+}
+
 __global__ void lm_decide_failed_kernel(DeviceSystem sys, double* lmState, Scalar* lmLam, double* lmRing)
 {
 	if (threadIdx.x != 0) return;
diff --git a/cuda-bundle-adjustment_amd/csrc/ba_kernels.hpp b/cuda-bundle-adjustment_amd/csrc/ba_kernels.hpp
--- a/cuda-bundle-adjustment_amd/csrc/ba_kernels.hpp
+++ b/cuda-bundle-adjustment_amd/csrc/ba_kernels.hpp
@@ -80,6 +80,7 @@
 	int* host_flags = nullptr;
 	int* ticket = nullptr;
 	int* kbase = nullptr;
+	int* early = nullptr;
 	int agg = 0;
 	int nc = 0;
 	Scalar inv_agg = 0;
@@ -155,6 +156,7 @@
 constexpr int LM_REC = 8, LM_RING = 64;
 struct LmDevice { double* state = nullptr; Scalar* lam = nullptr; double* ring = nullptr; };
 void launch_lm_decide_failed(const DeviceSystem& sys, const LmDevice& lm, hipStream_t s);
+void launch_lm_start(const DeviceSystem& sys, const Scalar* slots, const LmDevice& lm, double tau, int maxq, double tagBase, hipStream_t s);
 void launch_restore_if_rejected(Scalar* state, const Scalar* backup, size_t count, const LmDevice& lm, hipStream_t s);
 void launch_landmark_scale(const DeviceGraph& g, const DeviceSystem& sys, Scalar lambda, Scalar* slots, hipStream_t s);
 
@@ -175,7 +177,7 @@
 int pcg_rows_entries_per_thread(const DeviceSystem& sys);
 void launch_build_lowpos(const DeviceGraph& g, const DeviceStructure& st, int* lowpos, hipStream_t s);
 void launch_pcg_upper_iteration(const DeviceGraph& g, const DeviceStructure& st, const DeviceSystem& sys, int k, int maxIter, Scalar tol2, hipStream_t s, int which = 7);
-void launch_pcg_advance(const DeviceSystem& sys, int n, hipStream_t s, Scalar tol2 = Scalar(-1));
+void launch_pcg_advance(const DeviceSystem& sys, int n, hipStream_t s, Scalar tol2, int kEnd);
 void launch_coarse_to_fp32(const Scalar* swept, float* dst, int n, hipStream_t s);
 void launch_pcg_iteration(const DeviceGraph& g, const DeviceStructure& st, const DeviceSystem& sys, int k, int maxIter, Scalar tol2, hipStream_t s);
 
diff --git a/cuda-bundle-adjustment_amd/csrc/ba_lm.hip b/cuda-bundle-adjustment_amd/csrc/ba_lm.hip
--- a/cuda-bundle-adjustment_amd/csrc/ba_lm.hip
+++ b/cuda-bundle-adjustment_amd/csrc/ba_lm.hip
@@ -95,14 +95,15 @@
 	volatile int* flags = (volatile int*)((char*)h_pinned + 1024);
 	{
 		const auto t0 = Clock::now();
-		for (long spins = 0; flags[3] != expectedTicket; spins++)
+		for (long spins = 0; flags[3] - expectedTicket < 0; spins++)
 			if ((spins & 0xfff) == 0xfff && std::chrono::duration<double>(Clock::now() - t0).count() > 2.0) break;
-		if (flags[3] == expectedTicket)
+		if (flags[3] - expectedTicket >= 0)
 		{
 			std::atomic_thread_fence(std::memory_order_acquire);
 			return;
 		}
 	}
+	cntReportTimeouts++;
 	sync();
 	std::atomic_thread_fence(std::memory_order_acquire);
 	expectedTicket = flags[3];
@@ -336,6 +337,9 @@
 	}
 	return true;
 }
+
+constexpr int PCG_PREDICT_MARGIN = 2;
+constexpr int PCG_CONT_FIRST = 3;
 
 bool cuba_hip_solver::solveBegin(SolveCtx& sc)
 {
@@ -442,15 +446,16 @@
 	}
 	sc.hInts = (volatile int*)((char*)h_pinned + 1024);
 	sc.tSolve0 = Clock::now();
+	const int margin = !useGraph && !sc.batched ? PCG_PREDICT_MARGIN : 1;
 	int predicted = 32;
 	if (runIters.size() >= 2)
 	{
 		const double a = runIters[runIters.size() - 2], b = runIters.back();
 		const double lin = b + std::max(0.0, b - a), geo = b * std::min(1.35, std::max(1.0, b / std::max(1.0, a)));
-		predicted = (int)std::max(lin, geo) + 1;
-	}
-	else if (runIters.size() == 1) predicted = (int)(1.35 * runIters[0]) + 2;
-	else if (firstSolveIters > 0) predicted = firstSolveIters + 1;
+		predicted = (int)std::max(lin, geo) + margin;
+	}
+	else if (runIters.size() == 1) predicted = (int)(1.35 * runIters[0]) + 1 + margin;
+	else if (firstSolveIters > 0) predicted = firstSolveIters + margin;
 	{
 		const size_t k = runIters.size();
 		if (heuristics && k < prevRunIters.size() && std::equal(runIters.begin(), runIters.end(), prevRunIters.begin())) predicted = prevRunIters[k];
@@ -479,12 +484,16 @@
 	SolveCtx sc;
 	if (solveBegin(sc)) return sc.result;
 	const int maxIter = sc.maxIter; const Scalar tol2 = sc.tol2; const bool graphs = sc.graphs; const int predicted = sc.predicted;
+	const bool exact = !useGraph;
+	DeviceSystem sy = sys;
+	if (exact) sy.early = d_early.data();
 	bool converged = false;
 	int k0 = 0, looks = 0, eagerIters = 0;
-	int target = (predicted + 3) / 4 * 4;
+	const int first = pcgFirstBatch > 0 ? pcgFirstBatch : predicted;
+	int target = exact ? first : (first + 3) / 4 * 4;
 	while (k0 < sc.budget && !converged)
 	{
-		int todo = std::max(4, std::min(target, sc.budget) - k0);
+		int todo = std::max(exact ? 1 : 4, std::min(target, sc.budget) - k0);
 		while (todo > 0)
 		{
 			int c = graphs ? 256 : todo;
@@ -497,8 +506,8 @@
 			if (exec) { HIP_TRY(hipGraphLaunch(exec, stream)); noteReport(); }
 			else
 			{
-				for (int k = 0; k < c; k++) enqueuePcgIteration(k, maxIter, tol2, stream);
-				launch_pcg_advance(sys, c, stream, tol2); noteReport();
+				for (int k = 0; k < c; k++) enqueuePcgIteration(sy, exact ? k0 + k : k, maxIter, tol2, stream);
+				launch_pcg_advance(sy, exact ? 0 : c, stream, tol2, exact ? k0 + c : c); noteReport();
 				if (graphs) { eagerIters += c; cntPcgPlain += c; }
 			}
 			k0 += c; todo -= c;
@@ -506,7 +515,8 @@
 		waitReport();
 		if (sc.hInts[0] != 0) return solveBrokeDown(sc);
 		if (sc.hInts[2] != 0 || sc.hInts[1] < std::min(k0, maxIter)) converged = true;
-		target = k0 + ((looks == 0 && k0 <= 96) ? 4 : std::max(8, k0 / 8 / 4 * 4));
+		if (exact) target = k0 + ((looks == 0 && k0 <= 96) ? PCG_CONT_FIRST : std::max(8, k0 / 8));
+		else target = k0 + ((looks == 0 && k0 <= 96) ? 4 : std::max(8, k0 / 8 / 4 * 4));
 		looks++; cntPcgLooks++; cntHostLooks++;
 	}
 	sc.converged = converged; sc.k0 = k0; sc.looks = looks; sc.eagerIters = eagerIters;
@@ -576,7 +586,7 @@
 	return a + b;
 }
 
-void cuba_hip_solver::lmRunBegin(LmRun& r, int niter, double* chi2Out)
+void cuba_hip_solver::lmRunBegin(LmRun& r, int niter, double* chi2Out, bool deviceStart)
 {
 	const double tau = 1e-5;
 	if (!h_lmRing)
@@ -588,6 +598,19 @@
 	startRunHistory();
 	r = LmRun();
 	r.niter = niter; r.chi2Out = chi2Out; r.stop = niter <= 0;
+	r.lm.state = d_lmState.data(); r.lm.lam = d_lamS.data(); r.lm.ring = lmRingDev;
+	if (deviceStart && niter > 0)
+	{
+		need();
+		launch_residual_chi2(g, d_parts.data(), slotsDev, nullptr, stream, priors(), relPoses());
+		zeroReduced(true);
+		d_maxdiag.zero(stream);
+		linearize(0, 0.0);
+		launch_pose_maxdiag(g, st, sys, stream);
+		r.tagBase = 65536.0 * (double)(++lmRunNonce);
+		launch_lm_start(sys, slotsDev, r.lm, tau, LmRun::maxq, r.tagBase, stream);
+		return;
+	}
 	r.F = computeErrors();
 	r.lam = tau * maxDiagonal();
 	{
@@ -599,7 +622,6 @@
 		HIP_TRY(hipMemcpyAsync(d_lmState.data(), st8, sizeof(double) * 9, hipMemcpyHostToDevice, stream));
 		HIP_TRY(hipMemcpyAsync(d_lamS.data(), l1, sizeof(Scalar), hipMemcpyHostToDevice, stream));
 	}
-	r.lm.state = d_lmState.data(); r.lm.lam = d_lamS.data(); r.lm.ring = lmRingDev;
 }
 
 void cuba_hip_solver::lmAbsorb(LmRun& r, int upto)
@@ -671,7 +693,7 @@
 int cuba_hip_solver::optimizeDeviceDecision(int niter, double* chi2Out)
 {
 	LmRun r;
-	lmRunBegin(r, niter, chi2Out);
+	lmRunBegin(r, niter, chi2Out, true);
 	while (lmBeforeTrial(r))
 	{
 		schur(true);
diff --git a/cuda-bundle-adjustment_amd/csrc/ba_pcg.hip b/cuda-bundle-adjustment_amd/csrc/ba_pcg.hip
--- a/cuda-bundle-adjustment_amd/csrc/ba_pcg.hip
+++ b/cuda-bundle-adjustment_amd/csrc/ba_pcg.hip
@@ -86,7 +86,7 @@
 	rzk = wave_sum(load_parts(rz_slot(sys, k), rz_count(sys, k), lane));
 	const Scalar rz0 = wave_sum(load_parts(sys.rz, sys.nrz0, lane));
 	const bool on = k < maxIter && *sys.fail == 0 && rzk > tol2 * rz0 && rzk == rzk;
-	if (!on && blockIdx.x == 0 && threadIdx.x == 0) { *sys.done = 1; if (!(rzk == rzk)) *sys.fail = 3; }
+	if (!on && blockIdx.x == 0 && threadIdx.x == 0) pcg_raise_done(sys, rzk);
 	return on;
 }
 
@@ -258,7 +258,7 @@
 	const Scalar rzk = to_uniform(wave_sum(s_k)), rz0 = to_uniform(wave_sum(s_0)), rzm = to_uniform(wave_sum(s_m));
 	if (!(k < maxIter && failed == 0 && rzk > tol2 * rz0 && rzk == rzk))
 	{
-		if (blockIdx.x == 0 && threadIdx.x == 0) { *sys.done = 1; if (!(rzk == rzk)) *sys.fail = 3; }
+		if (blockIdx.x == 0 && threadIdx.x == 0) pcg_raise_done(sys, rzk);
 		return;
 	}
 	const Scalar beta = k > 0 ? rzk / rzm : Scalar(0);
@@ -398,7 +398,7 @@
 	const Scalar rzk = to_uniform(wave_sum(s_k)), rz0 = to_uniform(wave_sum(s_0)), rzm = to_uniform(wave_sum(s_m));
 	if (!(k < maxIter && failed == 0 && rzk > tol2 * rz0 && rzk == rzk))
 	{
-		if (blockIdx.x == 0 && threadIdx.x == 0) { *sys.done = 1; if (!(rzk == rzk)) *sys.fail = 3; }
+		if (blockIdx.x == 0 && threadIdx.x == 0) pcg_raise_done(sys, rzk);
 		return;
 	}
 	const Scalar beta = k > 0 ? rzk / rzm : Scalar(0);
@@ -685,7 +685,7 @@
 		for (int w = 0; w < PCG2_T / 64; w++) { rzk += wsum[w]; rz0 += wsum[8 + w]; pqk += wsum[16 + w]; }
 		if (!(kabs < maxIter && failed == 0 && rzk > tol2 * rz0 && rzk == rzk))
 		{
-			if (blockIdx.x == 0 && threadIdx.x == 0) { *sys.done = 1; if (!(rzk == rzk)) *sys.fail = 3; }
+			if (blockIdx.x == 0 && threadIdx.x == 0) pcg_raise_done(sys, rzk);
 			return;
 		}
 		if (!PRE)
@@ -919,7 +919,7 @@
 	const Scalar rzk = to_uniform(wave_sum(s_k)), rz0 = to_uniform(wave_sum(s_0)), rzm = to_uniform(wave_sum(s_m));
 	if (!(k < maxIter && failed == 0 && rzk > tol2 * rz0 && rzk == rzk))
 	{
-		if (blockIdx.x == 0 && threadIdx.x == 0) { *sys.done = 1; if (!(rzk == rzk)) *sys.fail = 3; }
+		if (blockIdx.x == 0 && threadIdx.x == 0) pcg_raise_done(sys, rzk);
 		return;
 	}
 	const Scalar beta = k > 0 ? rzk / rzm : Scalar(0);
@@ -1032,7 +1032,7 @@
 	for (int w = 0; w < ROWS_T / 64; w++) { rzk += wsum[w]; rz0 += wsum[8 + w]; pqk += wsum[16 + w]; }
 	if (!(kabs < maxIter && failed == 0 && rzk > tol2 * rz0 && rzk == rzk))
 	{
-		if (blockIdx.x == 0 && threadIdx.x == 0) { *sys.done = 1; if (!(rzk == rzk)) *sys.fail = 3; }
+		if (blockIdx.x == 0 && threadIdx.x == 0) pcg_raise_done(sys, rzk);
 		return;
 	}
 	if (!(pqk > 0))
@@ -1137,12 +1137,12 @@
 	hipLaunchKernelGGL(pcg_update_kernel, dim3((g.Pf + 39) / 40), dim3(256), 0, s, g, st, sys, k, maxIter, tol2);
 }
 
-__device__ __forceinline__ void pcg_advance_body(const DeviceSystem& sys, int n, int report, Scalar tol2)
-{
-	if (tol2 >= 0 && n > 0)
+__device__ __forceinline__ void pcg_advance_body(const DeviceSystem& sys, int n, int report, Scalar tol2, int kEnd)
+{
+	if (tol2 >= 0 && kEnd > 0)
 	{
 		const int lane = threadIdx.x;
-		const Scalar rzk = wave_sum(load_parts(rz_slot(sys, 0), sys.nrz, lane)), rz0 = wave_sum(load_parts(sys.rz, sys.nrz0, lane));
+		const Scalar rzk = wave_sum(load_parts(rz_slot(sys, kEnd), sys.nrz, lane)), rz0 = wave_sum(load_parts(sys.rz, sys.nrz0, lane));
 		if (lane == 0 && *sys.done == 0 && *sys.fail == 0 && !(rzk > tol2 * rz0))
 		{
 			*sys.done = 1;
@@ -1151,15 +1151,20 @@
 	}
 	if (threadIdx.x != 0) return;
 	*sys.kbase += n;
+	if (sys.early && *sys.early)
+	{
+		*sys.early = 0;
+		return;
+	}
 	if (report && sys.host_flags) publish_report(sys);
 }
 
-__global__ __launch_bounds__(64) void pcg_advance_kernel(DeviceSystem sys, int n, int report, Scalar tol2) { pcg_advance_body(sys, n, report, tol2); }
+__global__ __launch_bounds__(64) void pcg_advance_kernel(DeviceSystem sys, int n, int report, Scalar tol2, int kEnd) { pcg_advance_body(sys, n, report, tol2, kEnd); }
 
 __global__ __launch_bounds__(64) void pcg_advance_batch_kernel(const BatchEntry* __restrict__ tab, int n, int report, Scalar tol2)
 {
 	if (tab[blockIdx.x].gridSpmv == 0) return;
-	pcg_advance_body(tab[blockIdx.x].sys, n, report, tol2);
+	pcg_advance_body(tab[blockIdx.x].sys, n, report, tol2, n);
 }
 
 __global__ void collect_eval_kernel(const Scalar* slots, Scalar* out)
@@ -1174,12 +1179,12 @@
 
 void launch_pcg_report(const DeviceSystem& sys, hipStream_t s)
 {
-	hipLaunchKernelGGL(pcg_advance_kernel, dim3(1), dim3(64), 0, s, sys, 0, 1, Scalar(-1));
-}
-
-void launch_pcg_advance(const DeviceSystem& sys, int n, hipStream_t s, Scalar tol2)
-{
-	hipLaunchKernelGGL(pcg_advance_kernel, dim3(1), dim3(64), 0, s, sys, n, 1, tol2);
+	hipLaunchKernelGGL(pcg_advance_kernel, dim3(1), dim3(64), 0, s, sys, 0, 1, Scalar(-1), 0);
+}
+
+void launch_pcg_advance(const DeviceSystem& sys, int n, hipStream_t s, Scalar tol2, int kEnd)
+{
+	hipLaunchKernelGGL(pcg_advance_kernel, dim3(1), dim3(64), 0, s, sys, n, 1, tol2, kEnd);
 }
 
 template <int CL, int AC, int AC2, int W>
@@ -1264,7 +1269,7 @@
 		}
 		else e = add_kernel_node(graph, last, (void*)pcg_update_kernel, dim3((g.Pf + 39) / 40), dim3(256), 0, g, st, sys, k, maxIter, tol2);
 	}
-	if (e == hipSuccess) e = add_kernel_node(graph, last, (void*)pcg_advance_kernel, dim3(1), dim3(64), 0, sys, chunk, report, tol2);
+	if (e == hipSuccess) e = add_kernel_node(graph, last, (void*)pcg_advance_kernel, dim3(1), dim3(64), 0, sys, chunk, report, tol2, chunk);
 	return e;
 }
 
diff --git a/cuda-bundle-adjustment_amd/csrc/ba_setup.hip b/cuda-bundle-adjustment_amd/csrc/ba_setup.hip
--- a/cuda-bundle-adjustment_amd/csrc/ba_setup.hip
+++ b/cuda-bundle-adjustment_amd/csrc/ba_setup.hip
@@ -201,8 +201,8 @@
 		HIP_TRY(hipHostGetDevicePointer(&dev, h_pinned, 0));
 		slotsDev = (Scalar*)dev; flagsDev = (int*)((char*)dev + 1024);
 	}
-	d_parts.resize(8192 + (size_t)E + 64); d_maxdiag.resize(64); d_fail.resize(1); d_iters.resize(1); d_kbase.resize(1); d_done.resize(1); d_ticket.resize(1);
-	d_fail.zero(stream); d_iters.zero(stream); d_kbase.zero(stream); d_done.zero(stream); d_ticket.zero(stream);
+	d_parts.resize(8192 + (size_t)E + 64); d_maxdiag.resize(64); d_fail.resize(1); d_iters.resize(1); d_kbase.resize(1); d_done.resize(1); d_ticket.resize(1); d_early.resize(1);
+	d_fail.zero(stream); d_iters.zero(stream); d_kbase.zero(stream); d_done.zero(stream); d_ticket.zero(stream); d_early.zero(stream);
 	if (deferredUpload)
 	{
 		if (!upStream) { HIP_TRY(hipStreamCreateWithFlags(&upStream, hipStreamNonBlocking)); HIP_TRY(hipEventCreateWithFlags(&evValues, hipEventDisableTiming)); }
diff --git a/cuda-bundle-adjustment_amd/csrc/ba_solver.hip b/cuda-bundle-adjustment_amd/csrc/ba_solver.hip
--- a/cuda-bundle-adjustment_amd/csrc/ba_solver.hip
+++ b/cuda-bundle-adjustment_amd/csrc/ba_solver.hip
@@ -147,6 +147,7 @@
 		}
 		else if (k == "spmv_upper") { s->spmvUpper = (int)value; s->haveStructure = false; s->dropPcgGraph(); }
 		else if (k == "pcg_graph") { s->useGraph = value != 0; s->dropPcgGraph(); }
+		else if (k == "pcg_first_batch") s->pcgFirstBatch = std::max(0, (int)value);
 		else if (k == "profile") s->profile = value != 0;
 		else throw ArgError{ "unknown option: " + k };
 	});
@@ -379,6 +380,7 @@
 		else if (k == "structure_builds") *value = s->cntStructureBuilds;
 		else if (k == "value_bytes_uploaded") *value = s->cntValueBytes;
 		else if (k == "late_decision_records") *value = s->cntLateRecords;
+		else if (k == "report_wait_timeouts") *value = s->cntReportTimeouts;
 		else if (k == "covariance_ns") *value = (int64_t)(1e9 * s->covSeconds);
 		else if (k == "covariance_pairs_ns") *value = (int64_t)(1e9 * s->covPairsSeconds);
 		else if (k == "covariance_pairs_chunks") *value = s->covPairChunks;
diff --git a/cuda-bundle-adjustment_amd/csrc/ba_solver.hpp b/cuda-bundle-adjustment_amd/csrc/ba_solver.hpp
--- a/cuda-bundle-adjustment_amd/csrc/ba_solver.hpp
+++ b/cuda-bundle-adjustment_amd/csrc/ba_solver.hpp
@@ -115,6 +115,7 @@
 	int pcgAggregate = -1;
 	int spmvUpper = -1;
 	DevBuf<Scalar> d_tq; DevBuf<int> d_lowpos;
+	int pcgFirstBatch = 0;
 	bool deviceSetup = true;
 	bool devTopology = false;
 	bool hostTopoValid = false;
@@ -172,7 +173,7 @@
 	DevBuf<Scalar> d_red;
 	DevBuf<Scalar> d_parts, d_lmSys, d_lmInv, d_xp, d_xl, d_minv, d_r, d_z, d_p0, d_p1, d_ap, d_rz, d_pq;
 	DevBuf<unsigned long long> d_maxdiag;
-	DevBuf<int> d_fail, d_iters, d_kbase, d_done, d_ticket;
+	DevBuf<int> d_fail, d_iters, d_kbase, d_done, d_ticket, d_early;
 	DevBuf<Scalar> d_eval;
 	DevBuf<Scalar> d_coarse[3], d_gjPivots, d_rc, d_r2, d_qpart, d_hrow;
 	DevBuf<float> d_coarse32[2];
@@ -229,15 +230,15 @@
 	void dropPcgGraph();
 	std::map<int, int> batchRequests;
 
-	void enqueuePcgIteration(int k, int maxIter, Scalar tol2, hipStream_t s)
-	{
-		if (sys.agg > 0 && sys.upper) launch_pcg_upper_iteration(g, st, sys, k, maxIter, tol2, s);
-		else if (sys.agg > 0)
+	void enqueuePcgIteration(const DeviceSystem& sy, int k, int maxIter, Scalar tol2, hipStream_t s)
+	{
+		if (sy.agg > 0 && sy.upper) launch_pcg_upper_iteration(g, st, sy, k, maxIter, tol2, s);
+		else if (sy.agg > 0)
 		{
-			launch_pcg_spmv(g, st, sys, k, maxIter, tol2, s);
-			launch_pcg2_fused(g, sys, k, k + 1, maxIter, tol2, 1, s);
+			launch_pcg_spmv(g, st, sy, k, maxIter, tol2, s);
+			launch_pcg2_fused(g, sy, k, k + 1, maxIter, tol2, 1, s);
 		}
-		else launch_pcg_iteration(g, st, sys, k, maxIter, tol2, s);
+		else launch_pcg_iteration(g, st, sy, k, maxIter, tol2, s);
 	}
 
 	Scalar pcgGraphTol2 = 0; int pcgGraphMaxIter = 0;
@@ -310,6 +311,7 @@
 
 	bool failDirty = true;
 	int expectedTicket = 0;
+	int64_t cntReportTimeouts = 0;
 	bool hintSameEdges = false, hintSameValues = false;
 	void noteReport() { expectedTicket++; }
 	void waitReport();
@@ -587,7 +589,7 @@
 		double* chi2Out = nullptr;
 		LmDevice lm;
 	};
-	void lmRunBegin(LmRun& r, int niter, double* chi2Out);
+	void lmRunBegin(LmRun& r, int niter, double* chi2Out, bool deviceStart = false);
 	void lmAbsorb(LmRun& r, int upto);
 	bool lmBeforeTrial(LmRun& r);
 	bool lmAfterSolveHost(LmRun& r);
```

After: 817.5 million. No clear change (-0.1%).
